# AIR-DISCOVER/TOIST

Measured on AMD Instinct MI355X. Metric: train images/sec/node (640x640, bs=8/GPU) + matcher index bit-match, higher is better.
Workload: dtype bf16; 1 GPU; configs[1]: ResNet-101 + RoBERTa-base + 6+6 transformer, 100 queries, batch 8/GPU 640x640, 16-token captions, detection loss (labels+boxes+cardinality+contrastive_align, 5 aux layers), dropout 0.1, clip 0.1 + AdamW + EMA (fused HIP tail); random-init weights; every step a different batch (4 resident batches, 0..10 targets per image) through fixed-address inputs; global_batch=8, parallelism=dp1, launch=hipGraph replay, decoder=2 XCD-resident launches (toist_xdec_fwd / toist_xdec_bwd, one image per XCD)

## Files before the change

include/toist_hip.h:

```cpp
#ifndef TOIST_HIP_H
#define TOIST_HIP_H

#include <stddef.h>
#include <stdint.h>

#ifdef __cplusplus
extern "C" {
#endif

#define TOIST_OK 0
#define TOIST_EINVAL (-1)
#define TOIST_EHIP (-2)

#define TOIST_ABI_VERSION 1

#if defined(__GNUC__)
#define TOIST_API __attribute__((visibility("default")))
#else
#define TOIST_API
#endif

TOIST_API int toist_version(void);
TOIST_API int toist_last_error(char* buf, size_t cap);

TOIST_API int toist_matcher(const float* logits, const float* boxes, const float* tgt_boxes, const float* pos_map,
                  const int32_t* tgt_off, const int32_t* match_off, int L, int B, int Q, int K, int max_T,
                  float w_class, float w_bbox, float w_giou, int64_t* src_idx, int64_t* tgt_idx,
                  int32_t* status, float* cost_out, void* stream);

enum {
    TOIST_A_ROWK = 0,
    TOIST_A_KROW = 1,
    TOIST_A_CONV = 2,
    TOIST_A_CONVT = 3
};
enum {
    TOIST_B_ROWK = 0,
    TOIST_B_KROW = 1,
    TOIST_B_CONVX = 2
};
enum {
    TOIST_ACT_NONE = 0,
    TOIST_ACT_RELU = 1,
    TOIST_ACT_GELU = 2,
    TOIST_ACT_SIGMOID = 3,
    TOIST_ACT_MASK_POS = 4,
    TOIST_ACT_GELU_BWD = 5,
    TOIST_ACT_SIGMOID_BWD = 6
};

typedef struct toist_operand {
    const void* ptr;
    int64_t bs_outer;
    int64_t bs_inner;
    int32_t ld;
    int32_t kin;
    int64_t tap_stride;
    int32_t SH, SW, SC;
    int32_t PH, PW;
    int32_t R, S, stride, pad, dil;
} toist_operand;

typedef struct toist_epilogue {
    float alpha;
    const float* scale;
    const float* shift;
    const float* rscale;
    const void* res;
    int32_t ldr;
    const void* aux;
    int32_t ldaux;
    int32_t act;
    void* pre_out;
    int32_t out_f32;
    int32_t accumulate;
    int32_t cmap, cH, cW, cOH, cOW, cst;
    int32_t res_div, res_mod;
    int32_t drop_where;
    float drop_p;
    uint64_t drop_seed;
    const uint64_t* drop_seed_dev;
} toist_epilogue;

typedef struct toist_group {
    const void* a;
    const void* b;
    int64_t c_off;
    int64_t rscale_off;
    int64_t colsum_off;
    int64_t shift_off;
} toist_group;

typedef struct toist_gemm {
    int32_t M, N, K;
    int32_t a_kind, b_kind;
    toist_operand a, b;
    void* c;
    int32_t ldc;
    int64_t cs_outer, cs_inner;
    int32_t batch, batch_inner;
    int32_t split_k;
    int32_t tile;
    int32_t flags;
    toist_epilogue epi;
    float* workspace;
    float* a_colsum;
    const toist_group* group;
    const void* a2;
    int32_t a2_from;
} toist_gemm;

TOIST_API int toist_gemm_bf16(const toist_gemm* desc, void* stream);
TOIST_API int toist_group_fill(const toist_group* rows, int n, toist_group* table, void* stream);

TOIST_API int toist_layernorm_fwd(const void* x, const float* gamma, const float* beta, float eps, int rows, int D,
                        void* y, float* mean, float* rstd, const void* add, void* y2, void* stream);
TOIST_API int toist_layernorm_bwd(const void* dy, const void* x, const float* mean, const float* rstd, const float* gamma,
                        int rows, int D, void* dx, float* dgamma, float* dbeta, void* dx_drop, float drop_p,
                        uint64_t seed, const uint64_t* seed_dev, float* partials, int partial_blocks, void* stream);
TOIST_API int toist_layernorm_bwd_blocks(int rows);
TOIST_API int toist_softmax_fwd(const void* scores, const uint8_t* key_pad, int nbatch, int H, int Sq, int Sk, int ld,
                      void* p, void* p_drop, float drop_p, uint64_t seed, const uint64_t* seed_dev, void* stream);
TOIST_API int toist_softmax_bwd(const void* p, const void* dp, int rows, int Sk, int ld, void* ds, float drop_p,
                      uint64_t seed, const uint64_t* seed_dev, void* stream);
TOIST_API int toist_colsum(const void* g, int M, int N, int ld, float* out, void* stream);
TOIST_API int toist_add_bf16(const void* a, const void* b, int64_t n, int64_t b_period, void* out, void* stream);
TOIST_API int toist_dropout_bf16(const void* x, int64_t n, float p, uint64_t seed, const uint64_t* seed_dev, void* out, void* stream);

TOIST_API int toist_pack_image(const float* nchw, int N, int C, int H, int W, void* nhwc8, void* stream);
TOIST_API int toist_maxpool3x3s2(const void* in, int N, int H, int W, int C, void* out, void* stream);
TOIST_API int toist_unpack_nhwc(const void* nhwc, int N, int HW, int C, float* nchw, void* stream);
TOIST_API int toist_text_prep(const int64_t* ids, const int64_t* attention_mask, int B, int L, int64_t pad_id, int64_t* pos_ids, uint8_t* key_pad, void* stream);
TOIST_API int toist_stamp(uint64_t* slots, int idx, void* stream);

TOIST_API int toist_stem_fwd(const float* image, const void* weight, const float* shift, int N, int C, int H, int W, void* out, void* stream);

TOIST_API int toist_sine_position(const uint8_t* mask, int B, int H, int W, int num_pos_feats, float temperature, void* out_tok,
                        float* out_nchw, void* stream);
TOIST_API int toist_sine_position_seq(const uint8_t* mask, int B, int H, int W, int num_pos_feats, float temperature, void* out_tok, int rows_per_image,
                                      void* stream);

TOIST_API int toist_embed_fwd(const int64_t* ids, const int64_t* pos_ids, const float* word, const float* pos, const float* type0,
                    int n, int D, void* out, void* stream);
TOIST_API int toist_embed_bwd(const void* g, const int64_t* ids, const int64_t* pos_ids, int n, int D, int64_t pad_id, float* dword,
                    float* dpos, float* dtype0, void* stream);

TOIST_API int toist_criterion_fwd(const float* logits, const float* boxes, const float* tgt_boxes, const float* pos_map,
                        const int32_t* tgt_off, const int32_t* match_off, const int64_t* src_idx, const int64_t* tgt_idx,
                        const float* num_boxes, int L, int B, int Q, int K, float eos_coef, float* losses,
                        const int32_t* match_status, void* stream);
TOIST_API int toist_criterion_bwd(const float* logits, const float* boxes, const float* tgt_boxes, const float* pos_map,
                        const int32_t* tgt_off, const int32_t* match_off, const int64_t* src_idx, const int64_t* tgt_idx,
                        const float* num_boxes, int L, int B, int Q, int K, float eos_coef, const float* upstream,
                        float* dlogits, float* dboxes, void* stream);

TOIST_API int toist_contrastive_fwd(const float* proj_queries, const float* proj_tokens, const uint64_t* tok_mask, const int32_t* tgt_off,
                          const int32_t* match_off, const int64_t* src_idx, const int64_t* tgt_idx, const float* num_boxes, int L,
                          int B, int Q, int T, int D, float temperature, float* losses, void* stream);
TOIST_API int toist_contrastive_bwd(const float* proj_queries, const float* proj_tokens, const uint64_t* tok_mask, const int32_t* tgt_off,
                          const int32_t* match_off, const int64_t* src_idx, const int64_t* tgt_idx, const float* num_boxes, int L,
                          int B, int Q, int T, int D, float temperature, const float* upstream, float* dproj_queries,
                          float* dproj_tokens, void* stream);
TOIST_API int toist_contrastive_bwd_ws(const float* proj_queries, const float* proj_tokens, const uint64_t* tok_mask, const int32_t* tgt_off,
                          const int32_t* match_off, const int64_t* src_idx, const int64_t* tgt_idx, const float* num_boxes, int L,
                          int B, int Q, int T, int D, float temperature, const float* upstream, float* dproj_queries,
                          float* dproj_tokens, float* workspace, void* stream);
TOIST_API int toist_contrastive_fwd_live(const float* proj_queries, const float* proj_tokens, const uint64_t* tok_mask, const int32_t* tgt_off,
                          const int32_t* match_off, const int64_t* src_idx, const int64_t* tgt_idx, const float* num_boxes, int L,
                          int B, int Q, int T, int D, float temperature, const int32_t* live_tokens, float* losses, void* stream);
TOIST_API int toist_contrastive_bwd_ws_live(const float* proj_queries, const float* proj_tokens, const uint64_t* tok_mask, const int32_t* tgt_off,
                          const int32_t* match_off, const int64_t* src_idx, const int64_t* tgt_idx, const float* num_boxes, int L,
                          int B, int Q, int T, int D, float temperature, const int32_t* live_tokens, const float* upstream,
                          float* dproj_queries, float* dproj_tokens, float* workspace, void* stream);
TOIST_API int toist_l2norm_fwd(const float* x, int rows, int D, float* y, void* stream);
TOIST_API int toist_l2norm_bwd(const float* x, const float* dy, int rows, int D, float* dx, void* stream);

TOIST_API int toist_attnmap_softmax_fwd(const void* scores, const uint8_t* key_pad, int B, int Q, int H, int HW, int ld, void* out, void* stream);
TOIST_API int toist_attnmap_softmax_bwd(const void* prob, const void* dprob, int BQ, int H, int HW, int ld, void* dscores, void* stream);
TOIST_API int toist_groupnorm_fwd(const void* x, const float* gamma, const float* beta, int N, int HW, int C, int G, float eps, int relu,
                        void* y, float* stats, void* stream);
TOIST_API int toist_groupnorm_apply(const void* x, const float* stats, const float* gamma, const float* beta, int N, int HW, int C, int G, float eps, int relu,
                        void* y, void* stream);
TOIST_API int toist_groupnorm_bwd(const void* dy, const void* y, const void* x, const float* stats, const float* gamma, const float* beta, int N, int HW,
                        int C, int G, float eps, int relu, void* dx, float* dgamma, float* dbeta, float* bstats, void* stream);
TOIST_API int toist_upsample_add(const void* in, const void* fpn, int BQ, int Q, int H, int W, int C, void* out, void* stream);
TOIST_API int toist_upsample_add_rows(const void* in, const void* fpn, const int64_t* rows, int n, int Q, int H, int W, int C, void* out, void* stream);
TOIST_API int toist_upsample_add_bwd(const void* dout, int BQ, int H, int W, int C, void* din, void* stream);
TOIST_API int toist_resize_add(const void* in, const void* fpn, const int64_t* rows, int n, int Q, int H, int W, int OH, int OW, int C, void* out, void* stream);
TOIST_API int toist_resize_add_bwd(const void* dout, int BQ, int H, int W, int OH, int OW, int C, void* din, void* stream);
TOIST_API int toist_sum_queries(const void* in, int B, int Q, int64_t per, void* out, void* stream);
TOIST_API int toist_mask_stage_fwd(const void* src, const float* src_stats, const float* gamma, const float* beta, const void* fpn_conv, const void* w,
                        const float* bias, void* out, float* out_stats, int N, int Q, int H, int W, int c_in, int c_out, int w_rows, int gn_in, int up,
                        float eps, void* stream);
TOIST_API int toist_mask_stage_fwd_pairs(const void* src, const float* src_stats, const float* gamma, const float* beta, const void* fpn_conv, const void* w,
                        const float* bias, void* out, float* out_stats, int N, int Q, int H, int W, int c_in, int c_out, int w_rows, int gn_in, int up,
                        float eps, const int32_t* pair_image, int n_images, int32_t* status, void* stream);
TOIST_API int toist_resize_add_pairs(const void* in, const void* fpn, const int32_t* pair_image, int n_images, int n, int Q, int H, int W, int OH, int OW,
                        int C, void* out, int32_t* status, void* stream);
TOIST_API int toist_sum_segments(const void* in, const int32_t* seg, int B, int rows, int64_t per, void* out, void* stream);
TOIST_API int toist_resize_add_rows_pairs(const void* in, const void* fpn, const int64_t* rows, const int32_t* pair_image, int n_images, int P, int n, int Q,
                        int H, int W, int OH, int OW, int C, void* out, int32_t* status, void* stream);
TOIST_API int toist_sum_maps_by_image(const void* in, const int32_t* seg, const int32_t* pair_image, int P, int Q, int n_images, int rows, int64_t per,
                        void* out, int32_t* status, void* stream);
TOIST_API int toist_mask_loss_fwd(const float* pred, const int32_t* pred_row, const uint8_t* gt, const int32_t* gt_row, int T, int h, int w,
                        int TH, int TW, float alpha, float* sums, const int32_t* valid_hw, void* stream);
TOIST_API int toist_mask_loss_bwd(const float* pred, const int32_t* pred_row, const uint8_t* gt, const int32_t* gt_row, int T, int h, int w,
                        int TH, int TW, float alpha, const float* sums, const float* coef, float* dpred, const int32_t* valid_hw, void* stream);
TOIST_API int toist_mask_loss_bwd_compact(const float* pred, const int32_t* pred_row, const uint8_t* gt, const int32_t* gt_row, int T, int h, int w,
                        int TH, int TW, float alpha, const float* sums, const float* coef, float* dpred_rows, const int32_t* valid_hw, void* stream);

typedef struct toist_opt_tensor {
    float* p;
    float* m;
    float* v;
    float* ema;
    uint16_t* w;
    const float* row_scale;
    int64_t numel;
    int32_t row_len;
    int32_t group;
} toist_opt_tensor;

typedef struct toist_opt_group {
    float lr;
    float weight_decay;
} toist_opt_group;

typedef struct toist_opt_state {
    float clip_coef;
    float grad_norm;
    float bias1;
    float bias2_sqrt;
    int32_t step;
    int32_t skipped;
    int32_t skipped_total;
    int32_t veto_mask;
} toist_opt_state;
#define TOIST_OPT_MAX_VETO 8

TOIST_API int toist_attn2_splits(int Sk);
TOIST_API int toist_attn2_fwd(const void* q, int ldq, const void* kmat, int ldk, const void* v, int ldv, const uint8_t* key_pad, int B, int H, int Sq,
                    int Sk, int dh, float scale, float drop_p, uint64_t seed, const uint64_t* seed_dev, void* ctx, int ldo, float* lse,
                    void* stream);
TOIST_API int toist_attn2_bwd(const void* q, int ldq, const void* kmat, int ldk, const void* v, int ldv, const void* ctx, int ldo, const void* dctx, int lddo,
                    const float* lse, const uint8_t* key_pad, int B, int H, int Sq, int Sk, int dh, float scale, float drop_p, uint64_t seed,
                    const uint64_t* seed_dev, void* dq, int lddq, void* dk, int lddk, void* dv, int lddv, void* dq_part, void* stream);

enum { TOIST_ROW_PLAIN = 0, TOIST_ROW_LN_FWD = 1, TOIST_ROW_LN_BWD = 2 };

typedef struct toist_rowgemm_desc {
    int32_t M, K;
    int32_t b_kind;
    int32_t epi;
    const void* a;
    const void* w;
    int32_t lda, ldw;
    const void* fold;
    int64_t fold_stride;
    int32_t fold_parts, fold_cols;
    const float* bias;
    const void* res;
    const void* res2;
    int32_t ldr, ldr2;
    float drop_p;
    float eps;
    uint64_t drop_seed;
    const uint64_t* drop_seed_dev;
    const float* gamma;
    const float* beta;
    void* z;
    float* mean;
    float* rstd;
    void* out;
    int32_t ldo, reserved;
    const void* add;
    void* out2;
    float* partials;
} toist_rowgemm_desc;

TOIST_API int toist_rowgemm_blocks(int M);
TOIST_API int toist_rowgemm(const toist_rowgemm_desc* d, void* stream);

enum { TOIST_XDEC_MAX_LAYERS = 8, TOIST_XDEC_CTL_WORDS = 1024 };

typedef struct toist_xdec_layer {
    const void* w_in;  const float* b_in;
    const void* w_os;  const float* b_os;
    const float* g1;   const float* be1;
    const void* w_q;   const float* b_q;
    const void* w_oc;  const float* b_oc;
    const float* g3;   const float* be3;
    const void* w1;    const float* b1;
    const void* w2;    const float* b2;
    const float* g4;   const float* be4;
    uint64_t seed[6];
} toist_xdec_layer;

typedef struct toist_xdec_desc {
// ... 4 lines not shown
    const void* kv;
    int32_t ldkv;
    int32_t ff;
    int32_t test_absent;
    int32_t reserved;
    const uint8_t* key_pad;
    float drop_p, eps;
    const uint64_t* seed_dev;
    void* qkv;
    void* ctx_s;
    float* lse_s;
    void* z1; void* y1; void* y1e; float* mean1; float* rstd1;
    void* qc;
    void* ctx_c;
    float* lse_c;
    void* z3; void* y3; float* mean3; float* rstd3;
    void* h;
    void* z4; void* y4; void* y4e; float* mean4; float* rstd4;
    void* part;
    uint32_t* ctl;
    uint64_t* prof;
    toist_xdec_layer layer[TOIST_XDEC_MAX_LAYERS];
} toist_xdec_desc;

TOIST_API int toist_xdec_supported(int B, int Q, int S, int L);
TOIST_API int toist_xdec_fwd(const toist_xdec_desc* d, void* stream);

typedef struct toist_xdec_bwd_layer {
    const void* w_in;
    const void* w_os;
    const void* w_q;
    const void* w_oc;
    const void* w1;
    const void* w2;
    const float* g1;
    const float* g3;
    const float* g4;
    uint64_t seed[6];
} toist_xdec_bwd_layer;

typedef struct toist_xdec_bwd_desc {
    int32_t B, Q, S, L;
    const void* kv;
    int32_t ldkv, ldsink, lddkv;
    int32_t ff;
    int32_t test_absent;
    int32_t reserved;
    const uint8_t* key_pad;
    float drop_p, reserved2;
    const uint64_t* seed_dev;
    const void* qkv; const void* ctx_s; const float* lse_s; const void* z1; const float* mean1; const float* rstd1;
    const void* qc; const void* ctx_c; const float* lse_c; const void* z3; const float* mean3; const float* rstd3;
    const void* h; const void* z4; const float* mean4; const float* rstd4;
    const void* g_out;
    void* gb4;
    void* dh;
    void* go3;
    void* go1;
    void* sink;
    void* dkv;
    float* ln_part;
    void* dctx;
    void* part;
    void* dq_part;
    uint32_t* ctl;
    uint64_t* prof;
    toist_xdec_bwd_layer layer[TOIST_XDEC_MAX_LAYERS];
} toist_xdec_bwd_desc;

TOIST_API int toist_xdec_bwd(const toist_xdec_bwd_desc* d, void* stream);

TOIST_API int toist_scatter_rows_f32(const float* src, const int64_t* src_row, float* dst, const int64_t* dst_row, int m, int d, void* stream);

TOIST_API int toist_kmeans(const float* banks, int64_t bank_stride, float* centers, int64_t centers_stride, const int32_t* group_task,
                 const int32_t* group_off, const int32_t* members, int n_groups, const float* features, int N, int D, int K, float tol,
                 int max_iter, int32_t* pick, float* chosen_center, int32_t* iters, void* stream);

TOIST_API int toist_kmeans_init(const float* banks, int64_t bank_stride, float* centers, int64_t centers_stride, const int32_t* group_task,
                 const int32_t* group_off, const int32_t* members, int n_groups, const float* features, int N, int D, int K, float tol,
                 int max_iter, int32_t* pick, float* chosen_center, int32_t* iters, const float* full_label, const int32_t* init_rows,
                 int32_t* status, void* stream);

TOIST_API int toist_sweep_prototypes(const void* memory, void* memory_mod, const int32_t* pair_caption, const int32_t* live, const float* W_sth,
                 const uint8_t* sub_sth, const int32_t* cap_task, const int32_t* group_task, const float* banks, int64_t bank_stride,
                 float* centers, int64_t centers_stride, int P, int HW, int L, int T, int n_tasks, int N, int D, int K, float tol, int max_iter,
                 int32_t* status, int32_t* pick, float* features, int32_t* iters, void* stream);

TOIST_API int toist_bank_fifo(float* banks, int64_t bank_stride, float* update_count, float* full_label, const int32_t* group_task,
                 const int32_t* group_off, const int32_t* members, int n_groups, const float* rows, int T, int B, int N, int D,
                 int fifo_when_full, int32_t* lsap_rows, void* stream);

TOIST_API int toist_attn_small_fwd(const void* q, int ldq, const void* kmat, int ldk, const void* v, int ldv, const uint8_t* key_pad, int B, int H, int S,
                         int dh, float scale, float drop_p, uint64_t seed, const uint64_t* seed_dev, void* ctx, int ldo, float* stats,
                         const float* bq, const float* bk, const float* bv, void* stream);
TOIST_API int toist_attn_small_bwd(const void* q, int ldq, const void* kmat, int ldk, const void* v, int ldv, const uint8_t* key_pad, int B, int H, int S,
                         int dh, float scale, float drop_p, uint64_t seed, const uint64_t* seed_dev, const float* stats, const void* dctx,
                         int lddo, void* dq, int lddq, void* dk, int lddk, void* dv, int lddv, const float* bq, const float* bk,
                         const float* bv, void* stream);

TOIST_API int toist_conv3x3_small(int dgrad, const void* src, const void* w, const float* shift, const void* res, void* out, int n_img, int H, int W,
                        int c_src, int c_out, int w_co, int w_ci, void* stream);

TOIST_API int toist_wgrad3x3_small_blocks(void);
TOIST_API int toist_wgrad3x3_small(const void* dy, const void* x, float* ws, int n_img, int H, int W, int c_in, int c_out, void* stream);

TOIST_API int toist_lsap(const float* cost, const int64_t* offset, const int32_t* rows, const int32_t* cols, int ld ,
               int n, int max_rows, int max_cols,
               int64_t max_cells , const int64_t* out_off, int64_t* row_idx, int64_t* col_idx, int32_t* status, void* stream);

#define TOIST_GEMM_DEFER_REDUCE 2
#define TOIST_GEMM_SPLIT_EPILOGUE 4
#define TOIST_GEMM_COLSUM_SLICES 32768
TOIST_API int toist_gemm_pick_tile(const toist_gemm* desc);
typedef struct toist_reduce_desc {
    const float* ws;
    float* out;
    const float* rscale;
    int32_t splits, M, N, ldc;
    float alpha;
    int32_t accumulate;
} toist_reduce_desc;
TOIST_API int toist_gemm_effective_split(const toist_gemm* desc);
TOIST_API int toist_splitk_reduce_batch(const toist_reduce_desc* descs, int n, void* stream);

typedef struct toist_conv_pair {
    int32_t M, C;
    int32_t dgrad;
    int32_t lda;
    const void* a;
    const void* w_first;
    const void* w_second;
    const float* shift_mid;
    const float* shift_out;
    const void* res;
    const void* aux_mid;
    const void* aux_out;
    void* mid;
    void* out;
    int32_t ldr, ldaux_mid, ldaux_out, ldmid, ldout, reserved;
} toist_conv_pair;
TOIST_API int toist_conv_pair_bf16(const toist_conv_pair* desc, void* stream);

TOIST_API int toist_opt_chunk_elems(void);
TOIST_API int toist_opt_sqnorm(const toist_opt_tensor* table, const int64_t* grads, const int32_t* chunks, int n_chunks, float* partial, void* stream);
TOIST_API int toist_opt_finish_norm(const float* partial, int n_chunks, float max_norm, float beta1, float beta2, toist_opt_state* state, void* stream);
TOIST_API int toist_opt_finish_norm_guarded(const float* partial, int n_chunks, float max_norm, float beta1, float beta2, toist_opt_state* state,
                        const int32_t* const* veto_i32, int n_veto_i32, const float* const* veto_f32, int n_veto_f32, void* stream);
TOIST_API int toist_opt_adamw_ema(const toist_opt_tensor* table, const int64_t* grads, const int32_t* chunks, int n_chunks,
                        const toist_opt_group* groups, const toist_opt_state* state, float beta1, float beta2, float eps,
                        float ema_decay, void* stream);
TOIST_API int toist_opt_adamw_ema_blocks(const toist_opt_tensor* table, const int64_t* grads, const int32_t* chunks, int n_chunks,
                               const toist_opt_group* groups, const toist_opt_state* state, float beta1, float beta2, float eps,
                               float ema_decay, int max_blocks, void* stream);

TOIST_API int toist_mask_resize_pack(const float* src, int n, int h0, int w0, int max_h, int max_w, int crop_h, int crop_w, int h, int w,
                           float threshold, uint64_t* bits, void* stream);
TOIST_API int toist_mask_resize_pack_batch(const float* src, int batch, int queries, int h0, int w0, int max_h, int max_w, const int64_t* table,
                                 int cap_h, int cap_w, long long capacity_words, float threshold, uint64_t* bits, void* stream);
TOIST_API int toist_mask_pack(const uint8_t* dense, int n, int h, int w, uint64_t* bits, void* stream);
TOIST_API int toist_mask_unpack(const uint64_t* bits, int n, int h, int w, uint8_t* dense, void* stream);
TOIST_API int toist_mask_area(const uint64_t* bits, int n, int h, int w, uint32_t* area, void* stream);
TOIST_API int toist_mask_iou(const uint64_t* dt, int n_dt, const uint64_t* gt, int n_gt, const uint8_t* iscrowd, const uint32_t* area_dt,
                   const uint32_t* area_gt, int h, int w, double* iou, void* stream);
TOIST_API int toist_mask_rle_count(const uint64_t* bits, int n, int h, int w, int32_t* column_transitions, void* stream);
TOIST_API int toist_mask_rle_emit(const uint64_t* bits, int n, int h, int w, const int64_t* column_offset, uint32_t* positions, void* stream);
TOIST_API int toist_mask_rle_counts(const uint32_t* positions, const int64_t* first_position, const int64_t* first_run, int n, int h, int w,
                          uint32_t* counts, void* stream);

TOIST_API int toist_postprocess(const void* pred_logits, int logits_bf16, const void* pred_boxes, int boxes_bf16, const void* pred_isfinal, int isfinal_bf16,
                      const int64_t* orig_sizes, int B, int Q, int C, float* scores, float* boxes, float* scores_refexp, void* stream);

TOIST_API int toist_coco_match(const double* iou, const int64_t* iou_offset, const double* dt_area, const int64_t* dt_offset, const double* gt_area,
                     const uint8_t* gt_ignore, const uint8_t* gt_crowd, const int64_t* gt_offset, int n_images, const double* area_ranges,
                     int n_ranges, const double* iou_thresholds, int n_thresholds, int32_t* dt_match, uint8_t* dt_ignore,
                     uint8_t* gt_range_ignore, uint8_t* gt_taken, void* stream);

#define TOIST_COCO_BOXES_MAX_Q 1024
TOIST_API int toist_coco_boxes(const float* scores, const float* boxes, int R, int Q, int max_det, const int32_t* row_slot, const int64_t* slot_off,
                     int n_slots, const double* gt_xywh, const double* gt_area, const uint8_t* gt_crowd, long long n_gt, const int64_t* iou_off,
                     const int64_t* gt_off, long long iou_cap, long long gt_cap, int32_t* order, double* dt_score, double* dt_area, double* iou,
                     double* out_gt_area, uint8_t* out_gt_crowd, void* stream);

#define TOIST_COCO_MASKS_CHUNK_WORDS 4096
TOIST_API int toist_coco_masks(const uint64_t* bits, long long capacity_words, const int64_t* row_hw, int R, int Q, int D, const int32_t* order,
                     const int32_t* row_slot, const int64_t* slot_off, int n_slots, const uint64_t* gt_bits, long long gt_words,
                     const int64_t* gt_plane_off, const int32_t* slot_hw, const uint32_t* gt_parea, const uint8_t* gt_crowd, long long n_gt,
                     const int64_t* iou_off, long long iou_cap, double* dt_area, double* iou, void* stream);

#define TOIST_PREP_DESC_WORDS 20
TOIST_API int toist_image_prep(const uint8_t* src, long long src_bytes, const int32_t* desc, const int32_t* arena, long long arena_words, const float* lut,
                     int batch_cap, int cap_h, int cap_w, float* out, uint8_t* mask, uint8_t* dst_u8, long long dst_bytes, void* stream);

#define TOIST_TMASK_DESC_WORDS 8
TOIST_API int toist_target_masks(const uint8_t* src, long long src_bytes, const int32_t* desc, const int32_t* arena, long long arena_words, int slots,
                     int cap_h, int cap_w, uint8_t* dst, void* stream);

#define TOIST_POLY_DESC_WORDS 8
#define TOIST_POLY_REC_WORDS 2
#define TOIST_POLY_STRIP 64
#define TOIST_POLY_MAX_ROWS 2048
#define TOIST_POLY_PACKED 0
#define TOIST_POLY_DENSE 1
TOIST_API int toist_polygon_masks(const int32_t* desc, int slots, const int32_t* polys, int poly_cap, const int32_t* verts, int vert_cap, int cap_h,
                     int cap_w, uint8_t* dst, long long dst_bytes, int mode, void* stream);

TOIST_API int toist_sweep_assemble(const void* img_tok, const void* img_pos, const uint8_t* img_pad, int B, int HW, const void* txt_tok,
                     const uint8_t* txt_pad, int T, int L, const int32_t* pair_image, const int32_t* pair_caption, int P, int D, void* tokens,
                     void* pos, uint8_t* key_pad, int32_t* status, void* stream);

TOIST_API int toist_sweep_assemble_bwd(const void* d_seq, const int32_t* pair_image, const int32_t* pair_caption, int P, int B, int HW, int T, int L,
                     int D, void* d_img, void* d_txt, void* stream);

TOIST_API int toist_sweep_gather(const void* src, const int32_t* pair_image, int n_images, int P, long long row_bytes, void* dst, int32_t* status,
                     void* stream);

#ifdef __cplusplus
}
#endif
#endif
```

toist_amd/csrc/optim.hip:

```cpp
#include "common.h"

namespace toist {

constexpr int OPT_CHUNK = 8192;

__device__ __forceinline__ float block_sum_256(float v, float* red) {
    v = wave_sum(v);
    const int lane = threadIdx.x & 63, wave = threadIdx.x >> 6;
    if (lane == 0) red[wave] = v;
    __syncthreads();
    return red[0] + red[1] + red[2] + red[3];
}

__global__ __launch_bounds__(256) void sqnorm_kernel(const toist_opt_tensor* __restrict__ T, const int64_t* __restrict__ G,
                                                     const int2* __restrict__ chunks, float* __restrict__ partial) {
    __shared__ float red[4];
    const int2 ch = chunks[blockIdx.x];
    const float* g = reinterpret_cast<const float*>(G[ch.x]);
    float acc = 0.f;
    if (g != nullptr) {
        const long long beg = (long long)ch.y * OPT_CHUNK;
        long long end = beg + OPT_CHUNK;
        if (end > T[ch.x].numel) end = T[ch.x].numel;
        const float* gp = g + beg;
        const int n = (int)(end - beg);
        if (((size_t)gp & 15) == 0) {
            const int n4 = n >> 2;
            for (int i = threadIdx.x; i < n4; i += 256) {
                const float4 x = reinterpret_cast<const float4*>(gp)[i];
                acc += x.x * x.x + x.y * x.y + x.z * x.z + x.w * x.w;
            }
            for (int i = (n4 << 2) + threadIdx.x; i < n; i += 256) acc += gp[i] * gp[i];
        } else {
            for (int i = threadIdx.x; i < n; i += 256) acc += gp[i] * gp[i];
        }
    }
    const float s = block_sum_256(acc, red);
    if (threadIdx.x == 0) partial[blockIdx.x] = s;
}

__device__ __forceinline__ double sum_partials_1024(const float* __restrict__ partial, int n, double* red) {
    double acc = 0.0;
    int i = threadIdx.x;
    for (; i + 3 * 1024 < n; i += 4 * 1024) {
        const float a = partial[i], b = partial[i + 1024], c = partial[i + 2 * 1024], d = partial[i + 3 * 1024];
        acc += ((double)a + (double)b) + ((double)c + (double)d);
    }
    for (; i < n; i += 1024) acc += (double)partial[i];
    red[threadIdx.x] = acc;
    __syncthreads();
    for (int s = 512; s > 0; s >>= 1) {
        if (threadIdx.x < s) red[threadIdx.x] += red[threadIdx.x + s];
        __syncthreads();
    }
    return red[0];
}

__device__ __forceinline__ void take_step(toist_opt_state* __restrict__ st, float norm, float max_norm, float beta1, float beta2) {
    float coef = 1.f;
    if (max_norm > 0.f) {
        coef = max_norm / (norm + 1e-6f);
        if (coef > 1.f) coef = 1.f;
    }
    const int step = st->step + 1;
    st->step = step;
    st->grad_norm = norm;
    st->clip_coef = coef;
    st->bias1 = 1.f - powf(beta1, (float)step);
    st->bias2_sqrt = sqrtf(1.f - powf(beta2, (float)step));
    st->skipped = 0;
}

__device__ __forceinline__ bool nonfinite(float x) { return (__float_as_uint(x) & 0x7f800000u) == 0x7f800000u; }

__global__ __launch_bounds__(1024) void finish_norm_kernel(const float* __restrict__ partial, int n, float max_norm, float beta1,
                                                           float beta2, toist_opt_state* __restrict__ st) {
    __shared__ double red[1024];
    const double sq = sum_partials_1024(partial, n, red);
    if (threadIdx.x == 0) take_step(st, (float)sqrt(sq), max_norm, beta1, beta2);
}

__global__ __launch_bounds__(1024) void finish_norm_guarded_kernel(const float* __restrict__ partial, int n, float max_norm, float beta1,
                                                                   float beta2, toist_opt_state* __restrict__ st,
                                                                   const int32_t* const* __restrict__ veto_i32, int n_i32,
                                                                   const float* const* __restrict__ veto_f32, int n_f32) {
    __shared__ double red[1024];
    __shared__ int veto[2 * TOIST_OPT_MAX_VETO];
    const int t = threadIdx.x;
    if (t < 2 * TOIST_OPT_MAX_VETO) {
        int bit = 0;
        if (t < TOIST_OPT_MAX_VETO) {
            if (t < n_i32 && *veto_i32[t] != 0) bit = 1 << (1 + t);
        } else if (t - TOIST_OPT_MAX_VETO < n_f32 && nonfinite(*veto_f32[t - TOIST_OPT_MAX_VETO])) {
            bit = 1 << (1 + t);
        }
        veto[t] = bit;
    }
    const double sq = sum_partials_1024(partial, n, red);
    if (t == 0) {
        const float norm = (float)sqrt(sq);
        int mask = nonfinite(norm) ? 1 : 0;
        for (int i = 0; i < 2 * TOIST_OPT_MAX_VETO; ++i) mask |= veto[i];
        st->veto_mask = mask;
        if (mask == 0) {
            take_step(st, norm, max_norm, beta1, beta2);
        } else {
            st->skipped = 1;
            st->skipped_total = st->skipped_total + 1;
            st->grad_norm = norm;
            st->clip_coef = 0.f;
        }
    }
}

__device__ __forceinline__ void adamw_one(float& p, float g, float& m, float& v, float lr, float wd, float b1, float b2, float eps,
                                          float step_size, float bias2_sqrt) {
    p -= lr * wd * p;
    m += (g - m) * (1.f - b1);
    v = b2 * v + (1.f - b2) * g * g;
    const float denom = sqrtf(v) / bias2_sqrt + eps;
    p -= step_size * (m / denom);
}

__global__ __launch_bounds__(256) void adamw_ema_kernel(const toist_opt_tensor* __restrict__ T, const int64_t* __restrict__ G,
                                                        const int2* __restrict__ chunks, const toist_opt_group* __restrict__ groups,
                                                        const toist_opt_state* __restrict__ st, float b1, float b2, float eps,
                                                        float decay, int n_chunks) {
  if (st->skipped != 0) return;
  for (int cb = blockIdx.x; cb < n_chunks; cb += gridDim.x) {
    const int2 ch = chunks[cb];
    const toist_opt_tensor t = T[ch.x];
    const float* g = reinterpret_cast<const float*>(G[ch.x]);
    const long long beg = (long long)ch.y * OPT_CHUNK;
    long long end = beg + OPT_CHUNK;
    if (end > t.numel) end = t.numel;
    const int n = (int)(end - beg);
    const float coef = st->clip_coef, bias2_sqrt = st->bias2_sqrt;
    const toist_opt_group gr = groups[t.group];
    const float lr = gr.lr, wd = gr.weight_decay, step_size = lr / st->bias1;
    float* p = t.p + beg;
    const bool upd = g != nullptr && t.m != nullptr;
    const bool vec = (((size_t)p | (size_t)(g ? g + beg : nullptr) | (size_t)(t.m ? t.m + beg : nullptr) | (size_t)(t.v ? t.v + beg : nullptr) |
                       (size_t)(t.ema ? t.ema + beg : nullptr)) & 15) == 0 &&
                     (t.w == nullptr || (((size_t)(t.w + beg)) & 7) == 0);
    const int n4 = vec ? (n >> 2) : 0;
    for (int i = threadIdx.x; i < n4; i += 256) {
        float4 pv = reinterpret_cast<float4*>(p)[i];
        if (upd) {
            float4 gv = reinterpret_cast<const float4*>(g + beg)[i];
            float4 mv = reinterpret_cast<float4*>(t.m + beg)[i];
            float4 vv = reinterpret_cast<float4*>(t.v + beg)[i];
            adamw_one(pv.x, gv.x * coef, mv.x, vv.x, lr, wd, b1, b2, eps, step_size, bias2_sqrt);
            adamw_one(pv.y, gv.y * coef, mv.y, vv.y, lr, wd, b1, b2, eps, step_size, bias2_sqrt);
            adamw_one(pv.z, gv.z * coef, mv.z, vv.z, lr, wd, b1, b2, eps, step_size, bias2_sqrt);
            adamw_one(pv.w, gv.w * coef, mv.w, vv.w, lr, wd, b1, b2, eps, step_size, bias2_sqrt);
            reinterpret_cast<float4*>(p)[i] = pv;
            reinterpret_cast<float4*>(t.m + beg)[i] = mv;
            reinterpret_cast<float4*>(t.v + beg)[i] = vv;
        }
        if (t.ema != nullptr) {
            float4 ev = reinterpret_cast<float4*>(t.ema + beg)[i];
            ev.x = ev.x * decay + (1.f - decay) * pv.x;
            ev.y = ev.y * decay + (1.f - decay) * pv.y;
            ev.z = ev.z * decay + (1.f - decay) * pv.z;
            ev.w = ev.w * decay + (1.f - decay) * pv.w;
            reinterpret_cast<float4*>(t.ema + beg)[i] = ev;
        }
        if (upd && t.w != nullptr) {
            float s = 1.f;
            const long long e0 = beg + ((long long)i << 2);
            if (t.row_scale != nullptr) {
                const long long r0 = e0 / t.row_len;
                if ((e0 + 3) / t.row_len == r0) s = t.row_scale[r0];
                else {
                    pv.x *= t.row_scale[e0 / t.row_len];
                    pv.y *= t.row_scale[(e0 + 1) / t.row_len];
                    pv.z *= t.row_scale[(e0 + 2) / t.row_len];
                    pv.w *= t.row_scale[(e0 + 3) / t.row_len];
                }
            }
            reinterpret_cast<uint2*>(t.w + beg)[i] = make_uint2(pack2bf(pv.x * s, pv.y * s), pack2bf(pv.z * s, pv.w * s));
        }
    }
    for (int i = (n4 << 2) + threadIdx.x; i < n; i += 256) {
        float pv = p[i];
        if (upd) {
            float mv = t.m[beg + i], vv = t.v[beg + i];
            adamw_one(pv, g[beg + i] * coef, mv, vv, lr, wd, b1, b2, eps, step_size, bias2_sqrt);
            p[i] = pv;
            t.m[beg + i] = mv;
            t.v[beg + i] = vv;
        }
        if (t.ema != nullptr) t.ema[beg + i] = t.ema[beg + i] * decay + (1.f - decay) * pv;
        if (upd && t.w != nullptr) {
            const float s = t.row_scale ? t.row_scale[(beg + i) / t.row_len] : 1.f;
            t.w[beg + i] = f2bf(pv * s);
        }
    }
  }
}

}

using namespace toist;

extern "C" int toist_opt_chunk_elems(void) { return OPT_CHUNK; }

extern "C" int toist_opt_sqnorm(const toist_opt_tensor* table, const int64_t* grads, const int32_t* chunks, int n_chunks, float* partial,
                                void* stream) {
    TOIST_REQUIRE(table && grads && chunks && partial && n_chunks > 0, "toist_opt_sqnorm: bad args");
    hipLaunchKernelGGL(sqnorm_kernel, dim3(n_chunks), dim3(256), 0, (hipStream_t)stream, table, grads, (const int2*)chunks, partial);
    return check_launch("toist_opt_sqnorm");
}

extern "C" int toist_opt_finish_norm(const float* partial, int n_chunks, float max_norm, float beta1, float beta2, toist_opt_state* state,
                                     void* stream) {
    TOIST_REQUIRE(partial && state && n_chunks > 0, "toist_opt_finish_norm: bad args");
    TOIST_REQUIRE(beta1 >= 0.f && beta1 < 1.f && beta2 >= 0.f && beta2 < 1.f, "toist_opt_finish_norm: betas must be in [0, 1)");
    hipLaunchKernelGGL(finish_norm_kernel, dim3(1), dim3(1024), 0, (hipStream_t)stream, partial, n_chunks, max_norm, beta1, beta2, state);
    return check_launch("toist_opt_finish_norm");
}

extern "C" int toist_opt_finish_norm_guarded(const float* partial, int n_chunks, float max_norm, float beta1, float beta2, toist_opt_state* state,
                                             const int32_t* const* veto_i32, int n_veto_i32, const float* const* veto_f32, int n_veto_f32,
                                             void* stream) {
    TOIST_REQUIRE(partial && state && n_chunks > 0, "toist_opt_finish_norm_guarded: bad args");
    TOIST_REQUIRE(beta1 >= 0.f && beta1 < 1.f && beta2 >= 0.f && beta2 < 1.f, "toist_opt_finish_norm_guarded: betas must be in [0, 1)");
    TOIST_REQUIRE(n_veto_i32 >= 0 && n_veto_i32 <= TOIST_OPT_MAX_VETO && n_veto_f32 >= 0 && n_veto_f32 <= TOIST_OPT_MAX_VETO,
                  "toist_opt_finish_norm_guarded: at most 8 veto words of each kind");
    TOIST_REQUIRE((veto_i32 || n_veto_i32 == 0) && (veto_f32 || n_veto_f32 == 0), "toist_opt_finish_norm_guarded: NULL veto table with a positive count");
    hipLaunchKernelGGL(finish_norm_guarded_kernel, dim3(1), dim3(1024), 0, (hipStream_t)stream, partial, n_chunks, max_norm, beta1, beta2, state,
                       veto_i32, n_veto_i32, veto_f32, n_veto_f32);
    return check_launch("toist_opt_finish_norm_guarded");
}

extern "C" int toist_opt_adamw_ema_blocks(const toist_opt_tensor* table, const int64_t* grads, const int32_t* chunks, int n_chunks,
                                          const toist_opt_group* groups, const toist_opt_state* state, float beta1, float beta2, float eps,
                                          float ema_decay, int max_blocks, void* stream) {
    TOIST_REQUIRE(table && grads && chunks && groups && state && n_chunks > 0, "toist_opt_adamw_ema: bad args");
    TOIST_REQUIRE(eps > 0.f && ema_decay >= 0.f && ema_decay <= 1.f, "toist_opt_adamw_ema: bad eps / ema_decay");
    const int blocks = (max_blocks > 0 && max_blocks < n_chunks) ? max_blocks : n_chunks;
    hipLaunchKernelGGL(adamw_ema_kernel, dim3(blocks), dim3(256), 0, (hipStream_t)stream, table, grads, (const int2*)chunks, groups, state,
                       beta1, beta2, eps, ema_decay, n_chunks);
    return check_launch("toist_opt_adamw_ema");
}

extern "C" int toist_opt_adamw_ema(const toist_opt_tensor* table, const int64_t* grads, const int32_t* chunks, int n_chunks,
                                   const toist_opt_group* groups, const toist_opt_state* state, float beta1, float beta2, float eps,
                                   float ema_decay, void* stream) {
    return toist_opt_adamw_ema_blocks(table, grads, chunks, n_chunks, groups, state, beta1, beta2, eps, ema_decay, 0, stream);
}
```

toist_amd/csrc/rows.hip:

```cpp
#include "common.h"
#include <cstdlib>

namespace toist {

constexpr int LN_MAXCH = 2;

__global__ __launch_bounds__(256) void layernorm_fwd_kernel(const bf16_t* __restrict__ x, const float* __restrict__ gamma,
                                                             const float* __restrict__ beta, float eps, int rows, int D,
                                                             bf16_t* __restrict__ y, float* __restrict__ mean_out,
                                                             float* __restrict__ rstd_out, const bf16_t* __restrict__ add,
                                                             bf16_t* __restrict__ y2) {
    const int lane = threadIdx.x & 63;
    const int row = blockIdx.x * 4 + (threadIdx.x >> 6);
    if (row >= rows) return;
    const int nch = D >> 3;
    float v[LN_MAXCH][8];
    float s = 0.f;
#pragma unroll
    for (int i = 0; i < LN_MAXCH; ++i) {
        const int ch = lane + 64 * i;
        if (ch < nch) {
            unpack8(*reinterpret_cast<const uint4*>(x + (size_t)row * D + ch * 8), v[i]);
#pragma unroll
            for (int j = 0; j < 8; ++j) s += v[i][j];
// ... 214 lines not shown
                }
                *reinterpret_cast<uint4*>(p_drop + (size_t)row * ld + ch * 8) = pack8(o);
            }
        }
    }
}

__global__ __launch_bounds__(256) void softmax_bwd_kernel(const bf16_t* __restrict__ p, const bf16_t* __restrict__ dp, int rows,
                                                           int Sk, int ld, bf16_t* __restrict__ ds, float drop_p,
                                                           unsigned long long seed, const unsigned long long* __restrict__ seed_dev) {
    if (seed_dev) seed += *seed_dev;
    const int lane = threadIdx.x & 63;
    const int row = blockIdx.x * 4 + (threadIdx.x >> 6);
    if (row >= rows) return;
    const int nch = ld >> 3;
    const bool drop = drop_p > 0.f;
    const unsigned thresh = drop ? (unsigned)(drop_p * 4294967296.0) : 0u;
    const float dscale = drop ? 1.f / (1.f - drop_p) : 1.f;
    float pv[SM_MAXCH][8], gv[SM_MAXCH][8];
    float dot = 0.f;
#pragma unroll
    for (int i = 0; i < SM_MAXCH; ++i) {
        const int ch = lane + 64 * i;
        if (ch < nch) {
            unpack8(*reinterpret_cast<const uint4*>(p + (size_t)row * ld + ch * 8), pv[i]);
            unpack8(*reinterpret_cast<const uint4*>(dp + (size_t)row * ld + ch * 8), gv[i]);
#pragma unroll
            for (int j = 0; j < 8; ++j) {
                const int k = ch * 8 + j;
                if (k >= Sk) { pv[i][j] = 0.f; gv[i][j] = 0.f; }
                if (drop) {
                    const unsigned long long idx = (unsigned long long)row * ld + k;
                    gv[i][j] = dropout_keep(seed, idx, thresh) ? gv[i][j] * dscale : 0.f;
                }
                dot += pv[i][j] * gv[i][j];
            }
        }
    }
    dot = wave_sum(dot);
#pragma unroll
    for (int i = 0; i < SM_MAXCH; ++i) {
        const int ch = lane + 64 * i;
        if (ch < nch) {
            float o[8];
#pragma unroll
            for (int j = 0; j < 8; ++j) o[j] = pv[i][j] * (gv[i][j] - dot);
            *reinterpret_cast<uint4*>(ds + (size_t)row * ld + ch * 8) = pack8(o);
        }
    }
}

constexpr int CS_ROWS = 8192;
__global__ __launch_bounds__(256) void colsum_narrow_kernel(const bf16_t* __restrict__ g, long long M, int N, float* __restrict__ out) {
    __shared__ float red[256][9];
    const int cpr = N >> 3;
    const int rpp = 256 / cpr;
    const int cx = threadIdx.x % cpr, ry = threadIdx.x / cpr;
    const long long m_beg = (long long)blockIdx.x * CS_ROWS;
    const long long m_end = (m_beg + CS_ROWS < M) ? m_beg + CS_ROWS : M;
    float a[8] = {0.f, 0.f, 0.f, 0.f, 0.f, 0.f, 0.f, 0.f};
    for (long long m = m_beg + ry; m < m_end; m += rpp) {
        float v[8];
        unpack8(*reinterpret_cast<const uint4*>(g + m * N + cx * 8), v);
#pragma unroll
        for (int j = 0; j < 8; ++j) a[j] += v[j];
    }
#pragma unroll
    for (int j = 0; j < 8; ++j) red[threadIdx.x][j] = a[j];
    __syncthreads();
    if ((int)threadIdx.x < N) {
        const int c = threadIdx.x, cc = c >> 3, j = c & 7;
        float t = 0.f;
        for (int r = 0; r < rpp; ++r) t += red[r * cpr + cc][j];
        atomicAdd(out + c, t);
    }
}

__global__ __launch_bounds__(256) void colsum_kernel(const bf16_t* __restrict__ g, int M, int N, int ld, float* __restrict__ out) {
    __shared__ float red[8][256];
    const int cx = threadIdx.x & 31, ry = threadIdx.x >> 5;
    const int n = blockIdx.x * 256 + cx * 8;
    const int m_beg = blockIdx.y * 256;
    const int m_end = (m_beg + 256 < M) ? m_beg + 256 : M;
    float a[8] = {0.f, 0.f, 0.f, 0.f, 0.f, 0.f, 0.f, 0.f};
    if (n < N) {
        const bool vec = (n + 8 <= N) && ((ld & 7) == 0) && ((((size_t)g) & 15) == 0);
        for (int m = m_beg + ry; m < m_end; m += 8) {
            if (vec) {
                float v[8];
                unpack8(*reinterpret_cast<const uint4*>(g + (size_t)m * ld + n), v);
#pragma unroll
                for (int j = 0; j < 8; ++j) a[j] += v[j];
            } else {
#pragma unroll
                for (int j = 0; j < 8; ++j) if (n + j < N) a[j] += bf2f(g[(size_t)m * ld + n + j]);
            }
        }
    }
#pragma unroll
    for (int j = 0; j < 8; ++j) red[ry][cx * 8 + j] = a[j];
    __syncthreads();
    const int c = threadIdx.x;
    if (blockIdx.x * 256 + c < N) {
        float t = 0.f;
#pragma unroll
        for (int r = 0; r < 8; ++r) t += red[r][c];
        atomicAdd(out + blockIdx.x * 256 + c, t);
    }
}

__global__ __launch_bounds__(256) void add_kernel(const bf16_t* __restrict__ a, const bf16_t* __restrict__ b, long long n8,
                                                   long long bperiod8, bf16_t* __restrict__ out) {
    for (long long i = (long long)blockIdx.x * 256 + threadIdx.x; i < n8; i += (long long)gridDim.x * 256) {
        float x[8], y[8];
        unpack8(reinterpret_cast<const uint4*>(a)[i], x);
        unpack8(reinterpret_cast<const uint4*>(b)[i % bperiod8], y);
#pragma unroll
        for (int j = 0; j < 8; ++j) x[j] += y[j];
        reinterpret_cast<uint4*>(out)[i] = pack8(x);
    }
}

__global__ __launch_bounds__(256) void dropout_kernel(const bf16_t* __restrict__ x, long long n8, float p, unsigned long long seed,
                                                       const unsigned long long* __restrict__ seed_dev, bf16_t* __restrict__ out) {
    if (seed_dev) seed += *seed_dev;
    const unsigned thresh = (unsigned)(p * 4294967296.0);
    const float sc = 1.f / (1.f - p);
    for (long long i = (long long)blockIdx.x * 256 + threadIdx.x; i < n8; i += (long long)gridDim.x * 256) {
        float v[8];
        unpack8(reinterpret_cast<const uint4*>(x)[i], v);
#pragma unroll
        for (int j = 0; j < 8; ++j) v[j] = dropout_keep(seed, (unsigned long long)i * 8 + j, thresh) ? v[j] * sc : 0.f;
        reinterpret_cast<uint4*>(out)[i] = pack8(v);
    }
}


__global__ __launch_bounds__(256) void embed_fwd_kernel(const long long* __restrict__ ids, const long long* __restrict__ pos_ids,
                                                         const float* __restrict__ word, const float* __restrict__ pos,
                                                         const float* __restrict__ type0, int n, int D, bf16_t* __restrict__ out) {
    const int lane = threadIdx.x & 63;
    const int t = blockIdx.x * 4 + (threadIdx.x >> 6);
    if (t >= n) return;
    const float* w = word + ids[t] * (long long)D;
    const float* p = pos + pos_ids[t] * (long long)D;
    for (int c = lane * 2; c < D; c += 128) {
        const float a = (w[c] + type0[c]) + p[c];
        const float b = (w[c + 1] + type0[c + 1]) + p[c + 1];
        *reinterpret_cast<unsigned*>(out + (size_t)t * D + c) = pack2bf(a, b);
    }
}
__global__ __launch_bounds__(256) void embed_bwd_kernel(const bf16_t* __restrict__ g, const long long* __restrict__ ids,
                                                         const long long* __restrict__ pos_ids, int n, int D, long long pad_id,
                                                         float* __restrict__ dword, float* __restrict__ dpos) {
    const int lane = threadIdx.x & 63;
    const int t = blockIdx.x * 4 + (threadIdx.x >> 6);
    if (t >= n) return;
    for (int which = 0; which < 2; ++which) {
        const long long* key = which ? pos_ids : ids;
        float* table = which ? dpos : dword;
        if (table == nullptr) continue;
        const long long id = key[t];
        if (id == pad_id) continue;
        bool dup = false;
        for (int u = lane; u < t; u += 64) dup |= (key[u] == id);
        if (__any(dup)) continue;
        float* row = table + id * (long long)D;
        for (int c0 = 0; c0 < D; c0 += 64) {
            const int c = c0 + lane;
            float s = 0.f;
            for (int base = t; base < n; base += 64) {
                const int u = base + lane;
                unsigned long long m = __ballot(u < n && key[u] == id);
                while (m) {
                    const int b = __ffsll((long long)m) - 1;
                    m &= m - 1;
                    if (c < D) s += bf2f(g[(size_t)(base + b) * D + c]);
                }
            }
            if (c < D) row[c] += s;
        }
    }
}
__global__ __launch_bounds__(256) void embed_type_bwd_kernel(const bf16_t* __restrict__ g, int n, int D, float* __restrict__ dtype0) {
    __shared__ float red[8][32];
    const int cx = threadIdx.x & 31, ry = threadIdx.x >> 5;
    const int c = blockIdx.x * 32 + cx;
    float a = 0.f;
    if (c < D)
        for (int t = ry; t < n; t += 8) a += bf2f(g[(size_t)t * D + c]);
    red[ry][cx] = a;
    __syncthreads();
    if (ry == 0 && c < D) {
        float s = 0.f;
#pragma unroll
        for (int r = 0; r < 8; ++r) s += red[r][cx];
        dtype0[c] += s;
    }
}

static inline int grid_for(long long n, int cap = 2048) {
    long long g = (n + 255) / 256;
    if (g < 1) g = 1;
    return (int)(g > cap ? cap : g);
}

}

using namespace toist;

extern "C" int toist_layernorm_fwd(const void* x, const float* gamma, const float* beta, float eps, int rows, int D,
                                   void* y, float* mean, float* rstd, const void* add, void* y2, void* stream) {
    TOIST_REQUIRE(rows > 0 && D > 0 && (D % 8) == 0 && D <= 1024, "toist_layernorm_fwd: rows=%d D=%d (D%%8==0, D<=1024)", rows, D);
    TOIST_REQUIRE((add == nullptr) == (y2 == nullptr), "toist_layernorm_fwd: add and y2 come together");
    hipLaunchKernelGGL(layernorm_fwd_kernel, dim3((rows + 3) / 4), dim3(256), 0, (hipStream_t)stream, (const bf16_t*)x, gamma,
                       beta, eps, rows, D, (bf16_t*)y, mean, rstd, (const bf16_t*)add, (bf16_t*)y2);
    return check_launch("toist_layernorm_fwd");
}

extern "C" int toist_layernorm_bwd_blocks(int rows) {
    int blocks = (rows + 7) / 8;
    if (blocks > 512) blocks = 512;
    return blocks < 1 ? 1 : blocks;
}

extern "C" int toist_layernorm_bwd(const void* dy, const void* x, const float* mean, const float* rstd, const float* gamma,
                                   int rows, int D, void* dx, float* dgamma, float* dbeta, void* dx_drop, float drop_p,
                                   uint64_t seed, const uint64_t* seed_dev, float* partials, int partial_blocks, void* stream) {
    TOIST_REQUIRE(rows > 0 && D > 0 && (D % 8) == 0 && D <= 1024, "toist_layernorm_bwd: rows=%d D=%d", rows, D);
    TOIST_REQUIRE((dgamma == nullptr) == (dbeta == nullptr), "toist_layernorm_bwd: dgamma/dbeta must both be set or null");
    TOIST_REQUIRE(partials == nullptr || (dgamma == nullptr && partial_blocks > 0), "toist_layernorm_bwd: partials replace dgamma / dbeta and need a block count");
    int blocks = (rows + 15) / 16;
    if (blocks > 128) blocks = 128;
    if (blocks < 1) blocks = 1;
    if (partials) blocks = partial_blocks;
    hipLaunchKernelGGL(layernorm_bwd_kernel, dim3(blocks), dim3(256), 0, (hipStream_t)stream, (const bf16_t*)dy,
                       (const bf16_t*)x, mean, rstd, gamma, rows, D, (bf16_t*)dx, dgamma, dbeta, (bf16_t*)dx_drop, drop_p,
                       (unsigned long long)seed, (const unsigned long long*)seed_dev, partials);
    return check_launch("toist_layernorm_bwd");
}

extern "C" int toist_softmax_fwd(const void* scores, const uint8_t* key_pad, int nbatch, int H, int Sq, int Sk, int ld,
                                 void* p, void* p_drop, float drop_p, uint64_t seed, const uint64_t* seed_dev, void* stream) {
    TOIST_REQUIRE(nbatch > 0 && H > 0 && Sq > 0 && Sk > 0, "toist_softmax_fwd: bad shape");
    TOIST_REQUIRE((ld % 8) == 0 && ld >= Sk && ld <= 2048, "toist_softmax_fwd: ld=%d Sk=%d (ld%%8==0, Sk<=ld<=2048)", ld, Sk);
    const int rows = nbatch * H * Sq;
    hipLaunchKernelGGL(softmax_fwd_kernel, dim3((rows + 3) / 4), dim3(256), 0, (hipStream_t)stream, (const bf16_t*)scores, key_pad,
                       rows, H, Sq, Sk, ld, (bf16_t*)p, (bf16_t*)p_drop, drop_p, (unsigned long long)seed, (const unsigned long long*)seed_dev);
    return check_launch("toist_softmax_fwd");
}

extern "C" int toist_softmax_bwd(const void* p, const void* dp, int rows, int Sk, int ld, void* ds, float drop_p, uint64_t seed,
                                 const uint64_t* seed_dev, void* stream) {
    TOIST_REQUIRE(rows > 0 && Sk > 0 && (ld % 8) == 0 && ld >= Sk && ld <= 2048, "toist_softmax_bwd: bad shape");
    hipLaunchKernelGGL(softmax_bwd_kernel, dim3((rows + 3) / 4), dim3(256), 0, (hipStream_t)stream, (const bf16_t*)p,
                       (const bf16_t*)dp, rows, Sk, ld, (bf16_t*)ds, drop_p, (unsigned long long)seed, (const unsigned long long*)seed_dev);
    return check_launch("toist_softmax_bwd");
}

extern "C" int toist_colsum(const void* g, int M, int N, int ld, float* out, void* stream) {
    TOIST_REQUIRE(M > 0 && N > 0 && ld >= N, "toist_colsum: bad shape");
    if (ld == N && N <= 128 && (N & 7) == 0 && (256 % (N >> 3)) == 0 && M >= 4 * CS_ROWS && ((((size_t)g) & 15) == 0)) {
        hipLaunchKernelGGL(colsum_narrow_kernel, dim3((unsigned)((M + CS_ROWS - 1) / CS_ROWS)), dim3(256), 0, (hipStream_t)stream, (const bf16_t*)g,
                           (long long)M, N, out);
        return check_launch("toist_colsum(narrow)");
    }
    hipLaunchKernelGGL(colsum_kernel, dim3((N + 255) / 256, (M + 255) / 256), dim3(256), 0, (hipStream_t)stream, (const bf16_t*)g, M,
                       N, ld, out);
    return check_launch("toist_colsum");
}

extern "C" int toist_add_bf16(const void* a, const void* b, int64_t n, int64_t b_period, void* out, void* stream) {
    TOIST_REQUIRE(n > 0 && (n % 8) == 0 && b_period > 0 && (b_period % 8) == 0 && (n % b_period) == 0,
                  "toist_add_bf16: n and b_period must be multiples of 8 and n %% b_period == 0");
    hipLaunchKernelGGL(add_kernel, dim3(grid_for(n / 8)), dim3(256), 0, (hipStream_t)stream, (const bf16_t*)a, (const bf16_t*)b,
                       (long long)(n / 8), (long long)(b_period / 8), (bf16_t*)out);
    return check_launch("toist_add_bf16");
}

extern "C" int toist_dropout_bf16(const void* x, int64_t n, float p, uint64_t seed, const uint64_t* seed_dev, void* out, void* stream) {
    TOIST_REQUIRE(n > 0 && (n % 8) == 0 && p >= 0.f && p < 1.f, "toist_dropout_bf16: bad args");
    hipLaunchKernelGGL(dropout_kernel, dim3(grid_for(n / 8)), dim3(256), 0, (hipStream_t)stream, (const bf16_t*)x, (long long)(n / 8),
                       p, (unsigned long long)seed, (const unsigned long long*)seed_dev, (bf16_t*)out);
    return check_launch("toist_dropout_bf16");
}

extern "C" int toist_embed_fwd(const int64_t* ids, const int64_t* pos_ids, const float* word, const float* pos, const float* type0,
                               int n, int D, void* out, void* stream) {
    TOIST_REQUIRE(n > 0 && D > 0 && (D % 2) == 0, "toist_embed_fwd: bad shape");
    hipLaunchKernelGGL(embed_fwd_kernel, dim3((n + 3) / 4), dim3(256), 0, (hipStream_t)stream, (const long long*)ids,
                       (const long long*)pos_ids, word, pos, type0, n, D, (bf16_t*)out);
    return check_launch("toist_embed_fwd");
}

extern "C" int toist_embed_bwd(const void* g, const int64_t* ids, const int64_t* pos_ids, int n, int D, int64_t pad_id, float* dword,
                               float* dpos, float* dtype0, void* stream) {
    TOIST_REQUIRE(n > 0 && D > 0, "toist_embed_bwd: bad shape");
    if (dword != nullptr || dpos != nullptr)
        hipLaunchKernelGGL(embed_bwd_kernel, dim3((n + 3) / 4), dim3(256), 0, (hipStream_t)stream, (const bf16_t*)g, (const long long*)ids,
                           (const long long*)pos_ids, n, D, (long long)pad_id, dword, dpos);
    if (dtype0 != nullptr)
        hipLaunchKernelGGL(embed_type_bwd_kernel, dim3((D + 31) / 32), dim3(256), 0, (hipStream_t)stream, (const bf16_t*)g, n, D, dtype0);
    return check_launch("toist_embed_bwd");
}
```

toist_amd/engine.py:

```python
import math

import weakref

import torch

from . import kernels as k
from . import ops
from .knobs import knob

BF16 = torch.bfloat16


class Var:

    __slots__ = ("data", "grad", "needs_grad", "drop", "gdrop", "raw_grad")

    def __init__(self, data, needs_grad=True):
        self.data = data
        self.grad = None
        self.needs_grad = needs_grad
        self.raw_grad = False
        self.drop = None
        self.gdrop = None

    def take_branch_grad(self, g):
        gd, self.gdrop = self.gdrop, None
        if gd is None:
            gd = torch.empty_like(g)
            k.dropout(g, self.drop[0], self.drop[1], gd)
        return gd

    def take_grad(self):
        g, self.grad = self.grad, None
        return g


OVERLAP = knob("TOIST_OVERLAP", "capture")
FUSED_ATTENTION = True
FUSED_BLOCKS = True
_SIDE = {}
SIDE_PRIORITY = knob("TOIST_SIDE_PRIORITY", 0)


_TEXT_PRELUDE = []


def register_text_prelude(opt, late_params):
    _TEXT_PRELUDE[:] = [(r, ids) for r, ids in _TEXT_PRELUDE if r() is not None]
    _TEXT_PRELUDE.append((weakref.ref(opt), frozenset(id(p) for p in late_params)))


def run_text_prelude(param):
    for r, ids in _TEXT_PRELUDE:
        opt = r()
        if opt is not None and id(param) in ids:
            opt.flush_late()


def side_stream(device, name):
    key = (device.index, name)
    s = _SIDE.get(key)
    if s is None:
        s = _SIDE[key] = torch.cuda.Stream(device=device, priority=SIDE_PRIORITY)
    return s


def overlap_enabled():
    if OVERLAP == "on":
        return True
    return OVERLAP == "capture" and torch.cuda.is_current_stream_capturing()


GROUP_WGRADS = knob("TOIST_GROUP_WGRADS", True)


class Tape:
    def __init__(self, training, drop_p=0.0, seed=0, group_wgrads=False):
        self.groups = {} if (group_wgrads and GROUP_WGRADS) else None
        self.steps = []
        self.training = training
        self.drop_p = drop_p if training else 0.0
        self._seed = seed * 1000003 + 12345
        self.keep = []
        self.fresh_views = []

    def next_seed(self):
        self._seed += 7919
        return self._seed & 0x7FFFFFFFFFFF

    def record(self, fn):
        self.steps.append(fn)

    def conv_wgrad(self, dy, x, w_shape, out, rscale, stride=1, pad=0, view=None):
        store = view is not None and view.fresh and not view.written
        if view is not None:
            view.mark_written()
        if self.groups is None:
            ops.conv2d_wgrad(dy, x, w_shape, stride=stride, pad=pad, out=out, rscale=rscale, defer=True, accumulate=not store)
        else:
            self.groups.setdefault((tuple(dy.shape), tuple(x.shape), tuple(w_shape), stride, pad, store), []).append((dy, x, out, rscale))

    def linear_wgrad(self, dy, x, W, b, owned=True):
        bias_out = b.g if b is not None else None
        store = W.fresh and not W.written
        W.mark_written()
        if self.groups is None or not owned:
            ops.linear_wgrad(dy, x, out=W.g, bias_out=bias_out, defer=True, accumulate=not store)
        else:
            key = ("linear", tuple(dy.shape), dy.stride(0), tuple(x.shape), x.stride(0), W.g.stride(0), bias_out is None, store)
            self.groups.setdefault(key, []).append((dy, x, W.g, bias_out))

    def backward(self):
        for fn in reversed(self.steps):
            fn()
        self.steps = []
        if self.groups:
            for key, items in self.groups.items():
                if key[0] == "linear":
                    ops.linear_wgrad_group(items, accumulate=not key[-1])
                else:
                    ops.conv2d_wgrad_group(items, key[2], stride=key[3], pad=key[4], accumulate=not key[5])
            self.groups = {}
        k.flush_reductions()
        for v in self.fresh_views:
            for a, b in v.unwritten_rows():
                if v.g.dim() == 0:
                    v.g.zero_()
                else:
                    v.g[a:b].zero_()


WEIGHT_EPOCH = 0
COPY_GEN = 0
COPIES = {}


def bump_weight_epoch():
    global WEIGHT_EPOCH
    WEIGHT_EPOCH += 1


try:
    from torch.optim.optimizer import register_optimizer_step_post_hook as _reg_post_hook
    _reg_post_hook(lambda *a, **k: bump_weight_epoch())
except Exception:
    _reg_post_hook = None


class ComputeCopy:
    __slots__ = ("version", "ptr", "epoch", "w", "row_scale", "elementwise", "master")


def prune_copies():
    for ptr in [ptr for ptr, ent in COPIES.items() if ent.master() is None]:
        del COPIES[ptr]


def copy_of(t):
    ent = COPIES.get(t.data_ptr())
    return ent if ent is not None and ent.master() is t and ent.ptr == t.data_ptr() else None


def _cast_bf16(m):
    return m.detach().to(BF16)


_cast_bf16.elementwise = True


def compute_copy(t, make, cache, name):
    global COPY_GEN
    ent = cache.get(name) if cache is not None else None
    if ent is not None and ent.version == t._version and ent.ptr == t.data_ptr() and (ent.epoch == WEIGHT_EPOCH or not t.requires_grad) \
            and _reg_post_hook is not None:
        return ent.w
    w = make(t)
    pinned = bool(getattr(make, "pinned", False))
    if ent is not None and pinned and ent.w.data_ptr() != w.data_ptr():
        ent = None
    if ent is not None and pinned:
        pass
    elif ent is not None and ent.w.shape == w.shape and ent.w.stride() == w.stride():
        ent.w.copy_(w)
    else:
        ent = ComputeCopy()
        ent.w = w
        ent.elementwise = bool(getattr(make, "elementwise", False)) and w.shape == t.shape and w.stride() == t.stride()
        ent.row_scale = getattr(make, "row_scale", None)
        COPY_GEN += 1
        if cache is not None:
            cache[name] = ent
    ent.version, ent.ptr, ent.epoch, ent.master = t._version, t.data_ptr(), WEIGHT_EPOCH, weakref.ref(t)
    if cache is not None:
        COPIES[t.data_ptr()] = ent
    return ent.w


def named_cache(owner, key, build):
    memo = owner.__dict__.setdefault("_named_memo", {})
    ent = memo.get(key)
    if ent is None:
        ent = memo[key] = build()
    return ent


class ParamView:

    __slots__ = ("w", "g", "f32", "fresh", "parent", "_lo", "_hi", "_ranges")

    def __init__(self, w_bf16, grad_f32, f32=None, fresh=False, parent=None, lo=None, hi=None):
        self.w = w_bf16
        self.g = grad_f32
        self.f32 = f32
        self.fresh = fresh
        self.parent = parent
        self._lo, self._hi = lo, hi
        self._ranges = []

    def _root(self):
        v = self
        while v.parent is not None:
            v = v.parent
        return v

    def _span(self):
        lo, hi, v = 0, None, self
        chain = []
        while v is not None:
            chain.append(v)
            v = v.parent
        for v in reversed(chain):
            if v._lo is not None:
                lo, hi = lo + v._lo, lo + v._hi
        return lo, hi

    @property
    def written(self):
        root = self._root()
        if any(a is None for a, _ in root._ranges):
            return True
        lo, hi = self._span()
        if hi is None:
            n = root.g.shape[0] if root.g is not None and root.g.dim() > 0 else 1
            lo, hi = 0, n
        pos = lo
        for a, b in sorted(root._ranges):
            if a > pos:
                break
            pos = max(pos, b)
        return pos >= hi

    @written.setter
    def written(self, value):
        if value:
            self.mark_written()
        else:
            self._root()._ranges = []

    def rows(self, a, b):
        return ParamView(None if self.w is None else self.w[a:b], None if self.g is None else self.g[a:b],
                         None if self.f32 is None else self.f32[a:b], fresh=self.fresh, parent=self, lo=a, hi=b)

    def mark_written(self):
        root = self._root()
        lo, hi = self._span()
        root._ranges.append((None, None) if hi is None else (lo, hi))

    def unwritten_rows(self):
        if any(a is None for a, _ in self._ranges):
            return []
        n = self.g.shape[0] if self.g.dim() > 0 else 1
        gaps, pos = [], 0
        for a, b in sorted(self._ranges):
            if a > pos:
                gaps.append((pos, a))
            pos = max(pos, b)
        if pos < n:
            gaps.append((pos, n))
        return gaps


REUSE_GRAD_BUFFERS = False
STORE_ONCE = knob("TOIST_STORE_ONCE", True)
POISON_FRESH = False


class ParamSet:

    def __init__(self, named, trainable, need_grads, bf16_cache=None, transforms=None, store_once=None):
        self.names = list(named.keys())
        self.views = {}
        self.zero_elems = 0
        memo = bf16_cache.get("__layout__") if bf16_cache is not None else None
        params = list(named.values())
        sig = (need_grads, len(params), tuple(trainable.get(n, False) for n in self.names), id(params[0]) if params else 0,
               params[0].data_ptr() if params else 0, id(params[-1]) if params else 0, params[-1].data_ptr() if params else 0,
               STORE_ONCE and store_once is not None)
        if REUSE_GRAD_BUFFERS and memo is not None and memo["sig"] == sig and need_grads and memo["flat"] is not None:
            lo, hi = memo["flat"].data_ptr(), memo["flat"].data_ptr() + memo["flat"].numel() * 4
            if not any(p.grad is not None and lo <= p.grad.data_ptr() < hi for p in params):
                self.flat = memo["flat"]
                self.zero_elems = memo["zero_elems"]
                self._clear()
                for n, t in named.items():
                    pv = memo["views"][n]
                    pv.written = False
                    if t.dim() >= 2:
                        pv.w = compute_copy(t, (transforms or {}).get(n) or _cast_bf16, bf16_cache, n)
                    self.views[n] = pv
                return
        fresh_names = set()
        if need_grads and STORE_ONCE and store_once is not None:
            fresh_names = {n for n in self.names if trainable.get(n, False) and store_once(n, named[n])}
        pad = lambda t: (t.numel() + 63) // 64 * 64
        total = 0
        if need_grads:
            self.zero_elems = sum(pad(named[n]) for n in self.names if trainable.get(n, False) and n not in fresh_names)
            total = self.zero_elems + sum(pad(named[n]) for n in fresh_names)
        dev = next(iter(named.values())).device if named else None
        self.flat = torch.empty(total, dtype=torch.float32, device=dev) if total else None
        self._clear()
        off_zero, off_fresh = 0, self.zero_elems
        for n in self.names:
            t = named[n]
            g = None
            if need_grads and trainable.get(n, False):
                off = off_fresh if n in fresh_names else off_zero
                g = self.flat[off:off + t.numel()].view(t.shape)
                if t.dim() == 4 and not t.is_contiguous() and t.is_contiguous(memory_format=torch.channels_last):
                    O, I, R, S = t.shape
                    g = self.flat[off:off + t.numel()].view(O, R, S, I).permute(0, 3, 1, 2)
                if n in fresh_names:
                    off_fresh += pad(t)
                else:
                    off_zero += pad(t)
            wb = None
            if t.dim() >= 2:
                make = (transforms or {}).get(n) or _cast_bf16
                wb = compute_copy(t, make, bf16_cache, n)
            self.views[n] = ParamView(wb, g, t.detach(), fresh=n in fresh_names)
        if REUSE_GRAD_BUFFERS and bf16_cache is not None and need_grads and (memo is None or memo["sig"] != sig):
            bf16_cache["__layout__"] = {"sig": sig, "flat": self.flat, "views": dict(self.views), "zero_elems": self.zero_elems}

    def _clear(self):
        if self.flat is None:
            return
        if self.zero_elems:
            self.flat[:self.zero_elems].zero_()
        if POISON_FRESH and self.zero_elems < self.flat.numel():
            self.flat[self.zero_elems:].fill_(float("nan"))

    def fresh_views(self):
        return [v for v in self.views.values() if v.fresh and v.g is not None]

    def __getitem__(self, name):
        return self.views[name]

    def grads(self):
        return [self.views[n].g for n in self.names]


def krsc(w):
    v = w.permute(0, 2, 3, 1)
    assert v.is_contiguous(), "conv weights must be channels_last"
    return v


def accumulate(var, g):
    if var.grad is None:
        var.grad = g
    else:
        k.add(var.grad, g, var.grad)


def linear_chain(tape, x, layers, res=None, final_drop=False, out_dtype=BF16, last_act_external=False, in_relu_mask=False):
    acts = []
    cur = x.data
    p = tape.drop_p
    seeds = []
    n = len(layers)
    for i, (W, b, act, drop_after) in enumerate(layers):
        last = i == n - 1
        kw = {}
        seed = 0
        if drop_after and p > 0:
            seed = tape.next_seed()
            kw = dict(drop_where=2, drop_p=p, drop_seed=seed)
        if last and final_drop and p > 0:
            seed = tape.next_seed()
            kw = dict(drop_where=1, drop_p=p, drop_seed=seed)
        pre = None
        if act == k.ACT_GELU:
            pre = torch.empty(cur.shape[0], W.w.shape[0], dtype=BF16, device=cur.device)
        y = ops.linear(cur, W.w, b.f32 if b is not None else None, act=act, res=res.data if (last and res is not None) else None,
                       pre_out=pre, out_dtype=out_dtype if last else BF16, **kw)
        acts.append((cur, y, pre))
        seeds.append(seed)
        cur = y
    out = Var(cur)
    if final_drop and p > 0:
        out.drop = (p, seeds[-1])

    def bwd():
        g = out.take_grad()
        if g is None:
            return
        if res is not None and res.needs_grad:
            accumulate(res, g)
        for i in range(n - 1, -1, -1):
            W, b, act, drop_after = layers[i]
            xin, y, pre = acts[i]
            last = i == n - 1
            if last:
                if final_drop and p > 0:
                    g = out.take_branch_grad(g)
                if act != k.ACT_NONE and not last_act_external:
                    raise NotImplementedError("activation on the last layer of a chain needs last_act_external")
            if W.g is not None:
                tape.linear_wgrad(g, xin, W, b, owned=not (last and res is not None and res.needs_grad and not (final_drop and p > 0)))
            if i == 0:
                if x.needs_grad:
                    if in_relu_mask:
                        x.grad = ops.linear_dgrad(g, W.w, res=x.grad, act=k.ACT_MASK_POS, aux=x.data)
                    else:
                        x.grad = ops.linear_dgrad(g, W.w, res=x.grad)
            else:
                pW, pb, pact, pdrop = layers[i - 1]
                _, py, ppre = acts[i - 1]
                alpha = 1.0 / (1.0 - p) if (pdrop and p > 0) else 1.0
                if pact == k.ACT_RELU:
                    g = ops.linear_dgrad(g, W.w, act=k.ACT_MASK_POS, aux=py, alpha=alpha)
                elif pact == k.ACT_GELU:
                    if pdrop and p > 0:
                        raise NotImplementedError("dropout after GELU")
                    g = ops.linear_dgrad(g, W.w, act=k.ACT_GELU_BWD, aux=ppre)
                elif pact == k.ACT_NONE:
                    g = ops.linear_dgrad(g, W.w)
                else:
                    raise NotImplementedError

    tape.record(bwd)
    return out


def layernorm(tape, x, gamma, beta, eps, y=None):
    rows, D = x.data.shape
    if y is None:
        y = torch.empty_like(x.data)
    mean = torch.empty(rows, dtype=torch.float32, device=y.device)
    rstd = torch.empty(rows, dtype=torch.float32, device=y.device)
    k.layernorm_fwd(x.data, gamma.f32, beta.f32, eps, y, mean, rstd)
    out = Var(y)

    def bwd():
        g = out.take_grad()
        if g is None:
            return
        dx = torch.empty_like(g)
        if x.drop is not None and x.grad is None and x.needs_grad:
            x.gdrop = torch.empty_like(g)
            k.layernorm_bwd(g, x.data, mean, rstd, gamma.f32, dx, gamma.g, beta.g if gamma.g is not None else None, dx_drop=x.gdrop,
                            drop_p=x.drop[0], seed=x.drop[1], defer=True)
        else:
            k.layernorm_bwd(g, x.data, mean, rstd, gamma.f32, dx, gamma.g, beta.g if gamma.g is not None else None, defer=True)
        if x.needs_grad:
            accumulate(x, dx)

    tape.record(bwd)
    return out


def add_const(tape, x, c):
    y = torch.empty_like(x.data)
    k.add(x.data, c, y, b_period=c.numel())
    out = Var(y)

    def bwd():
        g = out.take_grad()
        if g is not None and x.needs_grad:
            accumulate(x, g)

    tape.record(bwd)
    return out


def add_vars(tape, a, b):
    y = torch.empty_like(a.data)
    k.add(a.data, b.data, y, b_period=b.data.numel())
    out = Var(y)
    rep = a.data.numel() // b.data.numel()

    def bwd():
        g = out.take_grad()
        if g is None:
            return
        if b.needs_grad:
            if rep == 1:
                accumulate(b, g)
            else:
                gb = g.view(rep, -1).float().sum(0).to(BF16).view(b.data.shape)
                accumulate(b, gb)
        if a.needs_grad:
            accumulate(a, g)
# ... 317 lines not shown
```

toist_amd/functions.py:

```python
import torch

from . import engine, kernels

GRAD_SYNC = None

AFTER_BACKWARD = []

REJOIN = None

PARAM_GRADS = "auto"


def _via_autograd():
    if PARAM_GRADS != "auto":
        return PARAM_GRADS == "autograd"
    try:
        from torch.nn.parallel import DistributedDataParallel as _DDP
        return getattr(_DDP, "_active_ddp_module", None) is not None
    except Exception:
        return False


class _TapeFn(torch.autograd.Function):
    @staticmethod
    def forward(ctx, body, names, cache, n_in, tape_kw, *tensors):
        inputs = tensors[:n_in]
        params = tensors[n_in:]
        tape_kw = dict(tape_kw)
        ctx.rejoin = tape_kw.pop('rejoin')
        ctx.via_autograd = tape_kw.pop('via_autograd')
        need = tape_kw.pop('need_grads')
        transforms = tape_kw.pop('transforms')
        store_once = tape_kw.pop('store_once')
        named = dict(zip(names, params))
        trainable = {n: p.requires_grad for n, p in named.items()}
        ps = engine.ParamSet(named, trainable, need_grads=need, bf16_cache=cache, transforms=transforms, store_once=store_once)
        tape = engine.Tape(**tape_kw)
        tape.fresh_views = ps.fresh_views() if need else []
        in_vars = [None if t is None else engine.Var(t, needs_grad=(need and t.requires_grad and t.is_floating_point()))
                   for t in inputs]
        out_vars, extra = body(tape, ps, *in_vars)
        if need:
            ctx.tape, ctx.ps, ctx.in_vars, ctx.out_vars = tape, ps, in_vars, out_vars
            ctx.params = params
        else:
            tape.steps = []
        ctx.n_in = n_in
        ctx.label = names[0].split(".")[0] if names else "program"
        ctx.n_par = len(params)
        ctx.extra = extra
        non_diff = [v.data for v in out_vars if not v.needs_grad]
        if non_diff:
            ctx.mark_non_differentiable(*non_diff)
        return tuple(v.data for v in out_vars)

    @staticmethod
    def backward(ctx, *grads):
        tape, ps = ctx.tape, ctx.ps
        if kernels.STAMPS is not None:
            kernels.stamp("bwd." + ctx.label + ".start")
        for v, g in zip(ctx.out_vars, grads):
            if g is not None and v.needs_grad:
                if v.raw_grad:
                    v.grad = g
                    continue
                if g.dtype != v.data.dtype:
                    g = g.to(v.data.dtype)
                v.grad = g.contiguous()
        tape.backward()
        if kernels.STAMPS is not None:
            kernels.stamp("bwd." + ctx.label + ".end")
        in_grads = []
        for v in ctx.in_vars:
            if v is None or not v.needs_grad:
                in_grads.append(None)
            else:
                in_grads.append(v.take_grad())
        n_par = len(ctx.params)
        if ctx.via_autograd:
            par_grads = [g if (g is not None and p.requires_grad) else None for p, g in zip(ctx.params, ps.grads())]
            if ctx.rejoin is not None:
                ctx.rejoin.wait_stream(torch.cuda.current_stream())
            ctx.tape = ctx.ps = ctx.in_vars = ctx.out_vars = ctx.params = None
            del tape, ps
            return (None, None, None, None, None, *in_grads, *par_grads)
        for p, g in zip(ctx.params, ps.grads()):
            if g is None:
                continue
            if p.grad is None:
                p.grad = g
            else:
                p.grad.add_(g)
                ps.flat = None
        if GRAD_SYNC is not None:
            GRAD_SYNC(ps.flat)
        elif AFTER_BACKWARD:
            for hook in AFTER_BACKWARD:
                hook(ctx.params)
        if ctx.rejoin is not None:
            ctx.rejoin.wait_stream(torch.cuda.current_stream())
        ctx.tape = ctx.ps = ctx.in_vars = ctx.out_vars = ctx.params = None
        return (None, None, None, None, None, *in_grads, *([None] * n_par))


def run_program(body, named_params, inputs, cache=None, training=False, drop_p=0.0, seed=0, transforms=None, group_wgrads=False, store_once=None):
    names = tuple(named_params.keys())
    params = tuple(named_params.values())
    need = torch.is_grad_enabled() and any(t is not None and t.requires_grad for t in (*inputs, *params))
    tape_kw = dict(training=training, drop_p=drop_p, seed=seed, need_grads=need, transforms=transforms, rejoin=REJOIN, group_wgrads=group_wgrads,
                   via_autograd=need and _via_autograd(), store_once=store_once)
    return _TapeFn.apply(body, names, cache, len(inputs), tape_kw, *inputs, *params)
```

toist_amd/kernels.py:

```python
import ctypes
import os

import torch

from . import _lib
from .devcache import DeviceCache, keep
from .folds import FOLDS, _raw_stream
from .knobs import knob
from ._lib import (A_CONV, A_CONVT, A_KROW, A_ROWK, ACT_GELU, ACT_GELU_BWD, ACT_MASK_POS, ACT_NONE, ACT_RELU,
                   ACT_SIGMOID, ACT_SIGMOID_BWD, B_CONVX, B_KROW, B_ROWK, Epilogue, Gemm, Operand)

__all__ = [
    "A_ROWK", "A_KROW", "A_CONV", "A_CONVT", "B_ROWK", "B_KROW", "B_CONVX", "ACT_NONE", "ACT_RELU", "ACT_GELU",
    "ACT_SIGMOID", "ACT_MASK_POS", "ACT_GELU_BWD", "ACT_SIGMOID_BWD", "ConvGeom", "operand", "gemm", "matcher",
    "layernorm_fwd", "layernorm_bwd", "softmax_fwd", "softmax_bwd", "colsum", "add", "dropout", "pack_image", "maxpool3x3s2", "stem_fwd",
    "unpack_nhwc", "sine_position", "embed_fwd", "embed_bwd", "criterion_fwd", "criterion_bwd", "attnmap_softmax_fwd", "attnmap_softmax_bwd",
    "groupnorm_fwd", "groupnorm_apply", "groupnorm_bwd", "upsample_add", "upsample_add_bwd", "sum_queries", "sum_segments", "upsample_add_rows", "mask_stage_fwd", "mask_loss_fwd", "mask_loss_bwd",
]


PROFILE = None
SEED_DEV = None
FORCE_TILE = 0
FORCE_SPLIT = 0
# ... 249 lines not shown
    d.aux_mid, d.ldaux_mid = _p(aux_mid, torch.bfloat16), aux_mid.stride(0) if aux_mid is not None else 0
    d.aux_out, d.ldaux_out = _p(aux_out, torch.bfloat16), aux_out.stride(0) if aux_out is not None else 0
    d.mid, d.ldmid, d.out, d.ldout = _p(mid, torch.bfloat16), mid.stride(0), _p(out, torch.bfloat16), out.stride(0)
    CONV_PAIR_CALLS[1 if dgrad else 0] += 1
    _lib.check(_lib.lib().toist_conv_pair_bf16(ctypes.cast(ctypes.pointer(d), ctypes.c_void_p), _stream()), "toist_conv_pair_bf16")


def matcher(logits, boxes, tgt_boxes, pos_map, tgt_off, match_off, max_T, w_class, w_bbox, w_giou, src_idx, tgt_idx,
            status, cost_out=None):
    L, B, Q, K = logits.shape
    _lib.check(
        _lib.lib().toist_matcher(_p(logits, torch.float32), _p(boxes, torch.float32), _p(tgt_boxes, torch.float32),
                                 _p(pos_map, torch.float32), _p(tgt_off, torch.int32), _p(match_off, torch.int32), L, B, Q,
                                 K, max_T, w_class, w_bbox, w_giou, _p(src_idx, torch.int64), _p(tgt_idx, torch.int64),
                                 _p(status, torch.int32), _p(cost_out, torch.float32), _stream()), "toist_matcher")


def layernorm_fwd(x, gamma, beta, eps, y, mean=None, rstd=None, add=None, y2=None):
    rows, D = x.shape
    _lib.check(
        _lib.lib().toist_layernorm_fwd(_p(x, torch.bfloat16), _p(gamma, torch.float32), _p(beta, torch.float32), eps, rows, D,
                                       _p(y, torch.bfloat16), _p(mean, torch.float32), _p(rstd, torch.float32), _p(add, torch.bfloat16),
                                       _p(y2, torch.bfloat16), _stream()),
        "toist_layernorm_fwd")


LN_DEFER = knob("TOIST_LN_DEFER", True)


def _queue_ln_param_grads(blocks, D, dgamma, dbeta):
    partials = FOLDS.acquire(2 * blocks * D, dgamma.device, (dgamma, dbeta))
    for i, out in enumerate((dgamma, dbeta)):
        FOLDS.queue(partials.data_ptr() + 4 * i * blocks * D, out, blocks, 1, D, D)
    return partials


def layernorm_bwd(dy, x, mean, rstd, gamma, dx, dgamma=None, dbeta=None, dx_drop=None, drop_p=0.0, seed=0, defer=False):
    rows, D = x.shape
    partials, blocks = None, 0
    if defer and LN_DEFER and dgamma is not None:
        blocks = int(_lib.lib().toist_layernorm_bwd_blocks(rows))
        partials = _queue_ln_param_grads(blocks, D, dgamma, dbeta)
    _lib.check(
        _lib.lib().toist_layernorm_bwd(_p(dy, torch.bfloat16), _p(x, torch.bfloat16), _p(mean, torch.float32),
                                       _p(rstd, torch.float32), _p(gamma, torch.float32), rows, D, _p(dx, torch.bfloat16),
                                       None if partials is not None else _p(dgamma, torch.float32),
                                       None if partials is not None else _p(dbeta, torch.float32), _p(dx_drop, torch.bfloat16),
                                       drop_p, seed, _p(SEED_DEV), _p(partials, torch.float32), blocks, _stream()), "toist_layernorm_bwd")


def softmax_fwd(scores, key_pad, nbatch, H, Sq, Sk, ld, p, p_drop=None, drop_p=0.0, seed=0):
    _lib.check(
        _lib.lib().toist_softmax_fwd(_p(scores, torch.bfloat16), _p(key_pad, torch.uint8), nbatch, H, Sq, Sk, ld,
                                     _p(p, torch.bfloat16), _p(p_drop, torch.bfloat16), drop_p, seed, _p(SEED_DEV), _stream()),
        "toist_softmax_fwd")


def softmax_bwd(p, dp, rows, Sk, ld, ds, drop_p=0.0, seed=0):
    _lib.check(
        _lib.lib().toist_softmax_bwd(_p(p, torch.bfloat16), _p(dp, torch.bfloat16), rows, Sk, ld, _p(ds, torch.bfloat16),
                                     drop_p, seed, _p(SEED_DEV), _stream()), "toist_softmax_bwd")


def colsum(g, M, N, ld, out):
    _lib.check(_lib.lib().toist_colsum(_p(g, torch.bfloat16), M, N, ld, _p(out, torch.float32), _stream()), "toist_colsum")


def add(a, b, out, b_period=None):
    n = a.numel()
    _lib.check(
        _lib.lib().toist_add_bf16(_p(a, torch.bfloat16), _p(b, torch.bfloat16), n, n if b_period is None else b_period,
                                  _p(out, torch.bfloat16), _stream()), "toist_add_bf16")


STAMPS = None


def stamp(name):
    st = STAMPS
    if st is None:
        return
    names = st["names"]
    if name in names:
        idx = names.index(name)
    else:
        idx = len(names)
        if idx >= st["buf"].numel():
            return
        names.append(name)
    _lib.check(_lib.lib().toist_stamp(_p(st["buf"], torch.int64), idx, _stream()), "toist_stamp")


def dropout(x, p, seed, out):
    _lib.check(_lib.lib().toist_dropout_bf16(_p(x, torch.bfloat16), x.numel(), p, seed, _p(SEED_DEV), _p(out, torch.bfloat16), _stream()),
               "toist_dropout_bf16")


def pack_image(nchw, out):
    N, C, H, W = nchw.shape
    _lib.check(_lib.lib().toist_pack_image(_p(nchw, torch.float32), N, C, H, W, _p(out, torch.bfloat16), _stream()), "toist_pack_image")


def stem_fwd(images, w, shift, out):
    N, C, H, W = images.shape
    assert tuple(w.shape) == (64, 7, 7, 8) and w.is_contiguous() and images.is_contiguous() and out.is_contiguous()
    _lib.check(_lib.lib().toist_stem_fwd(_p(images, torch.float32), _p(w, torch.bfloat16), _p(shift, torch.float32), N, C, H, W,
                                         _p(out, torch.bfloat16), _stream()), "toist_stem_fwd")


def maxpool3x3s2(x, out):
    N, H, W, C = x.shape
    _lib.check(_lib.lib().toist_maxpool3x3s2(_p(x, torch.bfloat16), N, H, W, C, _p(out, torch.bfloat16), _stream()), "toist_maxpool3x3s2")


def unpack_nhwc(x, out):
    N, HW, C = x.shape
    _lib.check(_lib.lib().toist_unpack_nhwc(_p(x, torch.bfloat16), N, HW, C, _p(out, torch.float32), _stream()), "toist_unpack_nhwc")


def sine_position(mask_u8, num_pos_feats, temperature, out_tok=None, out_nchw=None):
    B, H, W = mask_u8.shape
    _lib.check(_lib.lib().toist_sine_position(_p(mask_u8, torch.uint8), B, H, W, num_pos_feats, temperature, _p(out_tok, torch.bfloat16),
                                              _p(out_nchw, torch.float32), _stream()), "toist_sine_position")


def text_prep(ids, attention_mask, pad_id):
    B, L = ids.shape
    pos_ids = torch.empty(B, L, dtype=torch.int64, device=ids.device)
    key_pad = torch.empty(B, L, dtype=torch.uint8, device=ids.device)
    _lib.check(_lib.lib().toist_text_prep(_p(ids, torch.int64), _p(attention_mask, torch.int64), B, L, pad_id, _p(pos_ids), _p(key_pad), _stream()),
               "toist_text_prep")
    return pos_ids, key_pad


def sine_position_seq(mask_u8, num_pos_feats, temperature, out_tok):
    B, H, W = mask_u8.shape
    _lib.check(_lib.lib().toist_sine_position_seq(_p(mask_u8, torch.uint8), B, H, W, num_pos_feats, temperature, _p(out_tok, torch.bfloat16),
                                                  out_tok.shape[1], _stream()), "toist_sine_position_seq")


def embed_fwd(ids, pos_ids, word, pos, type0, out):
    n, D = out.shape
    _lib.check(_lib.lib().toist_embed_fwd(_p(ids, torch.int64), _p(pos_ids, torch.int64), _p(word, torch.float32), _p(pos, torch.float32),
                                          _p(type0, torch.float32), n, D, _p(out, torch.bfloat16), _stream()), "toist_embed_fwd")


def embed_bwd(g, ids, pos_ids, pad_id, dword, dpos, dtype0):
    n, D = g.shape
    _lib.check(_lib.lib().toist_embed_bwd(_p(g, torch.bfloat16), _p(ids, torch.int64), _p(pos_ids, torch.int64), n, D, pad_id,
                                          _p(dword, torch.float32), _p(dpos, torch.float32), _p(dtype0, torch.float32), _stream()),
               "toist_embed_bwd")


def criterion_fwd(logits, boxes, tgt_boxes, pos_map, tgt_off, match_off, src_idx, tgt_idx, num_boxes, eos_coef, losses, status=None):
    L, B, Q, K = logits.shape
    _lib.check(_lib.lib().toist_criterion_fwd(_p(logits, torch.float32), _p(boxes, torch.float32), _p(tgt_boxes, torch.float32),
                                              _p(pos_map, torch.float32), _p(tgt_off, torch.int32), _p(match_off, torch.int32),
                                              _p(src_idx, torch.int64), _p(tgt_idx, torch.int64), _p(num_boxes, torch.float32), L, B, Q, K,
                                              eos_coef, _p(losses, torch.float32), _p(status, torch.int32), _stream()), "toist_criterion_fwd")


def criterion_bwd(logits, boxes, tgt_boxes, pos_map, tgt_off, match_off, src_idx, tgt_idx, num_boxes, eos_coef, upstream, dlogits, dboxes):
    L, B, Q, K = logits.shape
    _lib.check(_lib.lib().toist_criterion_bwd(_p(logits, torch.float32), _p(boxes, torch.float32), _p(tgt_boxes, torch.float32),
                                              _p(pos_map, torch.float32), _p(tgt_off, torch.int32), _p(match_off, torch.int32),
                                              _p(src_idx, torch.int64), _p(tgt_idx, torch.int64), _p(num_boxes, torch.float32), L, B, Q, K,
                                              eos_coef, _p(upstream, torch.float32), _p(dlogits, torch.float32), _p(dboxes, torch.float32),
                                              _stream()), "toist_criterion_bwd")


def contrastive_fwd(pq, pt, tok_mask, tgt_off, match_off, src_idx, tgt_idx, num_boxes, temperature, losses, live_tokens=None):
    L, B, Q, D = pq.shape
    if live_tokens is None:
        _lib.check(_lib.lib().toist_contrastive_fwd(_p(pq, torch.float32), _p(pt, torch.float32), _p(tok_mask, torch.int64), _p(tgt_off, torch.int32),
                                                    _p(match_off, torch.int32), _p(src_idx, torch.int64), _p(tgt_idx, torch.int64),
                                                    _p(num_boxes, torch.float32), L, B, Q, pt.shape[1], D, temperature, _p(losses, torch.float32),
                                                    _stream()), "toist_contrastive_fwd")
        return
    _lib.check(_lib.lib().toist_contrastive_fwd_live(_p(pq, torch.float32), _p(pt, torch.float32), _p(tok_mask, torch.int64), _p(tgt_off, torch.int32),
                                                     _p(match_off, torch.int32), _p(src_idx, torch.int64), _p(tgt_idx, torch.int64),
                                                     _p(num_boxes, torch.float32), L, B, Q, pt.shape[1], D, temperature, _p(live_tokens, torch.int32),
                                                     _p(losses, torch.float32), _stream()), "toist_contrastive_fwd_live")


def contrastive_bwd(pq, pt, tok_mask, tgt_off, match_off, src_idx, tgt_idx, num_boxes, temperature, upstream, dpq, dpt, live_tokens=None, workspace=None):
    L, B, Q, D = pq.shape
    ws = workspace if workspace is not None else \
        torch.empty(L * B * pt.shape[1] * D, dtype=torch.float32, device=pq.device)
    if ws.numel() < L * B * pt.shape[1] * D:
        raise ValueError(f"contrastive_bwd: the workspace holds {ws.numel()} floats, L * B * T * D = {L * B * pt.shape[1] * D}")
    if live_tokens is None:
        _lib.check(_lib.lib().toist_contrastive_bwd_ws(_p(pq, torch.float32), _p(pt, torch.float32), _p(tok_mask, torch.int64), _p(tgt_off, torch.int32),
                                                       _p(match_off, torch.int32), _p(src_idx, torch.int64), _p(tgt_idx, torch.int64),
                                                       _p(num_boxes, torch.float32), L, B, Q, pt.shape[1], D, temperature, _p(upstream, torch.float32),
                                                       _p(dpq, torch.float32), _p(dpt, torch.float32), _p(ws, torch.float32), _stream()), "toist_contrastive_bwd_ws")
        return
    _lib.check(_lib.lib().toist_contrastive_bwd_ws_live(_p(pq, torch.float32), _p(pt, torch.float32), _p(tok_mask, torch.int64), _p(tgt_off, torch.int32),
                                                        _p(match_off, torch.int32), _p(src_idx, torch.int64), _p(tgt_idx, torch.int64),
                                                        _p(num_boxes, torch.float32), L, B, Q, pt.shape[1], D, temperature,
                                                        _p(live_tokens, torch.int32), _p(upstream, torch.float32), _p(dpq, torch.float32),
                                                        _p(dpt, torch.float32), _p(ws, torch.float32), _stream()), "toist_contrastive_bwd_ws_live")


def l2norm_fwd(x, y):
    rows, D = x.numel() // x.shape[-1], x.shape[-1]
    _lib.check(_lib.lib().toist_l2norm_fwd(_p(x, torch.float32), rows, D, _p(y, torch.float32), _stream()), "toist_l2norm_fwd")


def l2norm_bwd(x, dy, dx):
    rows, D = x.numel() // x.shape[-1], x.shape[-1]
    _lib.check(_lib.lib().toist_l2norm_bwd(_p(x, torch.float32), _p(dy, torch.float32), rows, D, _p(dx, torch.float32), _stream()), "toist_l2norm_bwd")


BF16, F32 = torch.bfloat16, torch.float32


def attnmap_softmax_fwd(scores, key_pad, B, Q, H, HW, ld, out):
    _lib.check(_lib.lib().toist_attnmap_softmax_fwd(_p(scores, BF16), _p(key_pad, torch.uint8), B, Q, H, HW, ld, _p(out, BF16), _stream()),
               "toist_attnmap_softmax_fwd")


def attnmap_softmax_bwd(prob, dprob, BQ, H, HW, ld, dscores):
    _lib.check(_lib.lib().toist_attnmap_softmax_bwd(_p(prob, BF16), _p(dprob, BF16), BQ, H, HW, ld, _p(dscores, BF16), _stream()),
               "toist_attnmap_softmax_bwd")


def groupnorm_fwd(x, gamma, beta, N, HW, C, G, eps, relu, y, stats):
    _lib.check(_lib.lib().toist_groupnorm_fwd(_p(x, BF16), _p(gamma, F32), _p(beta, F32), N, HW, C, G, eps, 1 if relu else 0, _p(y, BF16),
                                              _p(stats, F32), _stream()), "toist_groupnorm_fwd")


def groupnorm_apply(x, stats, gamma, beta, N, HW, C, G, eps, relu, y):
    _lib.check(_lib.lib().toist_groupnorm_apply(_p(x, BF16), _p(stats, F32), _p(gamma, F32), _p(beta, F32), N, HW, C, G, eps, 1 if relu else 0, _p(y, BF16),
                                                _stream()), "toist_groupnorm_apply")


def groupnorm_bwd(dy, y, x, stats, gamma, N, HW, C, G, eps, relu, dx, dgamma, dbeta, bstats, beta=None):
    _lib.check(_lib.lib().toist_groupnorm_bwd(_p(dy, BF16), _p(y, BF16), _p(x, BF16), _p(stats, F32), _p(gamma, F32), _p(beta, F32), N, HW, C, G, eps,
                                              1 if relu else 0, _p(dx, BF16), _p(dgamma, F32), _p(dbeta, F32), _p(bstats, F32), _stream()),
               "toist_groupnorm_bwd")


def upsample_add(inp, fpn, BQ, Q, H, W, C, out):
    _lib.check(_lib.lib().toist_upsample_add(_p(inp, BF16), _p(fpn, BF16), BQ, Q, H, W, C, _p(out, BF16), _stream()), "toist_upsample_add")


def resize_add(inp, fpn, rows, n, Q, H, W, OH, OW, C, out):
    _lib.check(_lib.lib().toist_resize_add(_p(inp, BF16), _p(fpn, BF16), _p(rows, torch.int64), n, Q, H, W, OH, OW, C, _p(out, BF16), _stream()), "toist_resize_add")


def resize_add_bwd(dout, BQ, H, W, OH, OW, C, din):
    _lib.check(_lib.lib().toist_resize_add_bwd(_p(dout, BF16), BQ, H, W, OH, OW, C, _p(din, BF16), _stream()), "toist_resize_add_bwd")


def upsample_add_rows(inp, fpn, rows, n, Q, H, W, C, out):
    _lib.check(_lib.lib().toist_upsample_add_rows(_p(inp, BF16), _p(fpn, BF16), _p(rows, torch.int64), n, Q, H, W, C, _p(out, BF16), _stream()),
               "toist_upsample_add_rows")


def mask_stage_fwd(src, src_stats, gamma, beta, fpn_conv, w, bias, out, out_stats, N, Q, H, W, c_in, c_out, w_rows, gn_in, up, eps=1e-5):
    _lib.check(_lib.lib().toist_mask_stage_fwd(_p(src, BF16), _p(src_stats, F32), _p(gamma, F32), _p(beta, F32), _p(fpn_conv, BF16), _p(w, BF16), _p(bias, F32),
                                               _p(out, F32 if c_out == 1 else BF16), _p(out_stats, F32), N, Q, H, W, c_in, c_out, w_rows,
                                               1 if gn_in else 0, 1 if up else 0, eps, _stream()), "toist_mask_stage_fwd")


def upsample_add_bwd(dout, BQ, H, W, C, din):
    _lib.check(_lib.lib().toist_upsample_add_bwd(_p(dout, BF16), BQ, H, W, C, _p(din, BF16), _stream()), "toist_upsample_add_bwd")


def sum_queries(inp, B, Q, per, out):
    _lib.check(_lib.lib().toist_sum_queries(_p(inp, BF16), B, Q, per, _p(out, BF16), _stream()), "toist_sum_queries")


def mask_loss_fwd(pred, pred_row, gt, gt_row, T, h, w, TH, TW, alpha, sums, valid_hw=None):
    _lib.check(_lib.lib().toist_mask_loss_fwd(_p(pred, F32), _p(pred_row, torch.int32), _p(gt, torch.uint8), _p(gt_row, torch.int32), T, h, w, TH,
                                              TW, alpha, _p(sums, F32), _p(valid_hw, torch.int32), _stream()), "toist_mask_loss_fwd")


def sum_segments(inp, seg, B, rows, per, out):
    _lib.check(_lib.lib().toist_sum_segments(_p(inp, BF16), _p(seg, torch.int32), B, rows, per, _p(out, BF16), _stream()), "toist_sum_segments")


def mask_loss_bwd(pred, pred_row, gt, gt_row, T, h, w, TH, TW, alpha, sums, coef, dpred, compact=False, valid_hw=None):
    if compact:
        _lib.check(_lib.lib().toist_mask_loss_bwd_compact(_p(pred, F32), _p(pred_row, torch.int32), _p(gt, torch.uint8), _p(gt_row, torch.int32), T, h, w,
                                                          TH, TW, alpha, _p(sums, F32), _p(coef, F32), _p(dpred, F32), _p(valid_hw, torch.int32), _stream()), "toist_mask_loss_bwd_compact")
        return
    _lib.check(_lib.lib().toist_mask_loss_bwd(_p(pred, F32), _p(pred_row, torch.int32), _p(gt, torch.uint8), _p(gt_row, torch.int32), T, h, w, TH,
                                              TW, alpha, _p(sums, F32), _p(coef, F32), _p(dpred, F32), _p(valid_hw, torch.int32), _stream()), "toist_mask_loss_bwd")


def opt_chunk_elems():
    return int(_lib.lib().toist_opt_chunk_elems())


def opt_sqnorm(table, grads, chunks, n_chunks, partial):
    _lib.check(_lib.lib().toist_opt_sqnorm(_p(table, torch.uint8), _p(grads, torch.int64), _p(chunks, torch.int32), n_chunks,
                                           _p(partial, torch.float32), _stream()), "toist_opt_sqnorm")


def opt_finish_norm(partial, n_chunks, max_norm, beta1, beta2, state):
    _lib.check(_lib.lib().toist_opt_finish_norm(_p(partial, torch.float32), n_chunks, max_norm, beta1, beta2, _p(state, torch.uint8),
                                                _stream()), "toist_opt_finish_norm")


def opt_finish_norm_guarded(partial, n_chunks, max_norm, beta1, beta2, state, veto_i32, n_veto_i32, veto_f32, n_veto_f32):
    _lib.check(_lib.lib().toist_opt_finish_norm_guarded(_p(partial, torch.float32), n_chunks, max_norm, beta1, beta2, _p(state, torch.uint8),
                                                        _p(veto_i32, torch.int64), n_veto_i32, _p(veto_f32, torch.int64), n_veto_f32, _stream()),
               "toist_opt_finish_norm_guarded")


def opt_adamw_ema(table, grads, chunks, n_chunks, groups, state, beta1, beta2, eps, ema_decay, max_blocks=0):
    _lib.check(_lib.lib().toist_opt_adamw_ema_blocks(_p(table, torch.uint8), _p(grads, torch.int64), _p(chunks, torch.int32), n_chunks,
                                                     _p(groups, torch.float32), _p(state, torch.uint8), beta1, beta2, eps, ema_decay, max_blocks, _stream()),
               "toist_opt_adamw_ema")


def lsap(cost, offset, rows, cols, n, max_rows, max_cols, max_cells, out_off, row_idx, col_idx, status, ld=0):
    _lib.check(_lib.lib().toist_lsap(_p(cost, torch.float32), _p(offset, torch.int64), _p(rows, torch.int32), _p(cols, torch.int32), ld, n, max_rows,
                                     max_cols, max_cells, _p(out_off, torch.int64), _p(row_idx, torch.int64), _p(col_idx, torch.int64),
                                     _p(status, torch.int32), _stream()), "toist_lsap")


def conv3x3_small(dgrad, src, w, shift, res, out, n_img, H, W, c_src, c_out):
    w_co, w_ci = int(w.shape[0]), int(w.shape[3])
    _lib.check(_lib.lib().toist_conv3x3_small(1 if dgrad else 0, _p(src, torch.bfloat16), _p(w, torch.bfloat16), _p(shift, torch.float32),
                                              _p(res, torch.bfloat16), _p(out, torch.bfloat16), n_img, H, W, c_src, c_out, w_co, w_ci, _stream()),
               "toist_conv3x3_small")


def wgrad3x3_small(dy, x, out, defer=False, accumulate=True):
    n_img, H, W, C = x.shape
    Co = dy.shape[-1]
    blocks = int(_lib.lib().toist_wgrad3x3_small_blocks())
    ws = FOLDS.acquire(blocks * Co * 9 * C, x.device, (out,))
    _lib.check(_lib.lib().toist_wgrad3x3_small(_p(dy, torch.bfloat16), _p(x, torch.bfloat16), _p(ws, torch.float32), n_img, H, W, C, Co, _stream()),
               "toist_wgrad3x3_small")
    FOLDS.queue(ws.data_ptr(), out, blocks, Co, 9 * C, 9 * C, accumulate=accumulate)
    if not defer:
        flush_reductions()


def attn2_splits(Sk):
    return int(_lib.lib().toist_attn2_splits(Sk))


def attn2_fwd(q, kmat, v, key_pad, B, H, Sq, Sk, dh, scale, drop_p, seed, ctx, lse):
    _lib.check(_lib.lib().toist_attn2_fwd(_p(q, torch.bfloat16), q.stride(0), _p(kmat, torch.bfloat16), kmat.stride(0), _p(v, torch.bfloat16), v.stride(0),
                                          _p(key_pad, torch.uint8), B, H, Sq, Sk, dh, scale, drop_p, seed, _p(SEED_DEV) if drop_p > 0 else None,
                                          _p(ctx, torch.bfloat16), ctx.stride(0), _p(lse, torch.float32), _stream()), "toist_attn2_fwd")


def attn2_bwd(q, kmat, v, ctx, dctx, lse, key_pad, B, H, Sq, Sk, dh, scale, drop_p, seed, dq, dk, dv, dq_part=None):
    _lib.check(_lib.lib().toist_attn2_bwd(_p(q, torch.bfloat16), q.stride(0), _p(kmat, torch.bfloat16), kmat.stride(0), _p(v, torch.bfloat16), v.stride(0),
                                          _p(ctx, torch.bfloat16), ctx.stride(0), _p(dctx, torch.bfloat16), dctx.stride(0), _p(lse, torch.float32),
                                          _p(key_pad, torch.uint8), B, H, Sq, Sk, dh, scale, drop_p, seed, _p(SEED_DEV) if drop_p > 0 else None,
                                          _p(dq, torch.bfloat16), dq.stride(0) if dq is not None else 0, _p(dk, torch.bfloat16), dk.stride(0),
                                          _p(dv, torch.bfloat16), dv.stride(0), _p(dq_part, torch.bfloat16), _stream()), "toist_attn2_bwd")


def rowgemm(a, w, out, *, b_kind, epi, K=None, bias=None, res=None, res2=None, drop_p=0.0, drop_seed=0, gamma=None, beta=None, eps=1e-5,
            z=None, mean=None, rstd=None, add=None, out2=None, fold=None, fold_cols=0, dgamma=None, dbeta=None):
    M = a.shape[0]
    d = _lib.RowGemm()
    d.M, d.K, d.b_kind, d.epi = M, (a.shape[1] if K is None else K), b_kind, epi
    d.a, d.lda, d.w, d.ldw = _p(a, torch.bfloat16), a.stride(0), _p(w, torch.bfloat16), w.stride(0)
    if fold is not None:
        d.fold, d.fold_parts, d.fold_cols, d.fold_stride = _p(fold, torch.bfloat16), fold.shape[0], fold_cols, fold.stride(0)
        assert fold.shape[1] == M and fold.shape[2] == fold_cols and fold.stride(1) == fold_cols
    d.bias = _p(bias, torch.float32)
    if res is not None:
        d.res, d.ldr = _p(res, torch.bfloat16), res.stride(0)
    if res2 is not None:
        d.res2, d.ldr2 = _p(res2, torch.bfloat16), res2.stride(0)
    d.drop_p, d.eps, d.drop_seed = drop_p, eps, drop_seed
    d.drop_seed_dev = _p(SEED_DEV) if drop_p > 0 else None
    d.gamma, d.beta = _p(gamma, torch.float32), _p(beta, torch.float32)
    for name, t in (("z", z), ("add", add), ("out2", out2)):
        if t is not None:
            assert t.is_contiguous() and t.shape[-1] == 256
            setattr(d, name, _p(t, torch.bfloat16))
    d.mean, d.rstd = _p(mean, torch.float32), _p(rstd, torch.float32)
    d.out, d.ldo = _p(out, torch.bfloat16), out.stride(0)
    keep = None
    if epi == _lib.ROW_LN_BWD and dgamma is not None:
        keep = _queue_ln_param_grads(int(_lib.lib().toist_rowgemm_blocks(M)), 256, dgamma, dbeta)
        d.partials = _p(keep, torch.float32)
    _lib.check(_lib.lib().toist_rowgemm(ctypes.byref(d), _stream()), "toist_rowgemm")
    return keep


ROW_PLAIN, ROW_LN_FWD, ROW_LN_BWD = _lib.ROW_PLAIN, _lib.ROW_LN_FWD, _lib.ROW_LN_BWD


XDEC_PROF = None
XDEC_TEST_ABSENT = 0
XDEC_LAUNCHES = 0
XDEC_FAILED = False
_XDEC_CTL = {}


def _xdec_ctl(device, create=True):
    ctl = _XDEC_CTL.get(device)
    if ctl is None and create:
        if torch.cuda.is_current_stream_capturing():
            return None
        ctl = _XDEC_CTL[device] = torch.zeros(_lib.XDEC_CTL_WORDS, dtype=torch.int32, device=device)
    return ctl


def _ranks_share_a_device():
    import torch.distributed as dist
    if not (dist.is_available() and dist.is_initialized()):
        return False
    local = os.environ.get("LOCAL_WORLD_SIZE")
    local = int(local) if local and local.isdigit() else dist.get_world_size()
    return local > torch.cuda.device_count()


def xdec_supported(B, Q, S, L, ff=2048):
    if XDEC_FAILED or ff != 2048 or _ranks_share_a_device():
        return False
    if not _lib.lib().toist_xdec_supported(B, Q, S, L):
        return False
    return _xdec_ctl(torch.device("cuda", torch.cuda.current_device())) is not None


def xdec_fwd(B, Q, S, x0, qpos, kv, key_pad, drop_p, eps, out, layers, part, *, xe0):
    d = _lib.Xdec()
    d.B, d.Q, d.S, d.L = B, Q, S, len(layers)
    d.ff, d.test_absent = int(layers[0]["w1"].shape[0]), XDEC_TEST_ABSENT
    assert all(tuple(ly["w1"].shape) == (d.ff, 256) and tuple(ly["w2"].shape) == (256, d.ff) for ly in layers)
    d.x0, d.qpos, d.kv, d.ldkv = _p(x0, torch.bfloat16), _p(qpos, torch.bfloat16), _p(kv, torch.bfloat16), kv.stride(0)
    assert xe0.is_contiguous() and xe0.shape == qpos.shape
    d.xe0 = _p(xe0, torch.bfloat16)
    d.key_pad = _p(key_pad, torch.uint8) if key_pad is not None else None
    d.drop_p, d.eps = drop_p, eps
    d.seed_dev = _p(SEED_DEV) if drop_p > 0 else None
    for name in ("qkv", "ctx_s", "z1", "y1", "y1e", "qc", "ctx_c", "z3", "y3", "h", "z4", "y4", "y4e"):
        t = out[name]
        assert t.is_contiguous()
        setattr(d, name, _p(t, torch.bfloat16))
    for name in ("lse_s", "mean1", "rstd1", "lse_c", "mean3", "rstd3", "mean4", "rstd4"):
        t = out[name]
        assert t.is_contiguous()
        setattr(d, name, _p(t, torch.float32))
    assert part.is_contiguous() and part.numel() >= B * 32 * 128 * 256
    d.part = _p(part, torch.bfloat16)
    d.ctl = _xdec_ctl(x0.device).data_ptr()
    d.prof = XDEC_PROF.data_ptr() if XDEC_PROF is not None else None
    for i, ly in enumerate(layers):
        e = d.layer[i]
        for name in ("w_in", "w_os", "w_q", "w_oc", "w1", "w2"):
            t = ly[name]
            assert t.is_contiguous()
            setattr(e, name, _p(t, torch.bfloat16))
        for name in ("b_in", "b_os", "g1", "be1", "b_q", "b_oc", "g3", "be3", "b1", "b2", "g4", "be4"):
            t = ly[name]
            assert t.is_contiguous()
            setattr(e, name, _p(t, torch.float32))
        for j in range(6):
            e.seed[j] = ly["seed"][j]
    global XDEC_LAUNCHES
    XDEC_LAUNCHES += 1
    _lib.check(_lib.lib().toist_xdec_fwd(ctypes.byref(d), _stream()), "toist_xdec_fwd")
# ... 598 lines not shown
```

toist_amd/optim.py:

```python
import numpy as np
import torch

from . import _lib, engine
from . import kernels as k
from .knobs import knob

LATE_BLOCKS = knob("TOIST_LATE_BLOCKS", 0)

_TENSOR_DT = np.dtype([("p", "<i8"), ("m", "<i8"), ("v", "<i8"), ("ema", "<i8"), ("w", "<i8"), ("row_scale", "<i8"),
                       ("numel", "<i8"), ("row_len", "<i4"), ("group", "<i4")])
assert _TENSOR_DT.itemsize == 64
_GROUP_DT = np.dtype([("lr", "<f4"), ("weight_decay", "<f4")])
_STATE_DT = np.dtype([("clip_coef", "<f4"), ("grad_norm", "<f4"), ("bias1", "<f4"), ("bias2_sqrt", "<f4"),
                      ("step", "<i4"), ("skipped", "<i4"), ("skipped_total", "<i4"), ("veto_mask", "<i4")])


def ema_pairs(model, model_ema):
    if hasattr(model, "module"):
        model = model.module
    msd = model.state_dict()
    return [(msd[name], ev) for name, ev in model_ema.state_dict().items() if ev.is_floating_point()]


def _dense(t):
    return t.is_contiguous() or (t.dim() == 4 and t.is_contiguous(memory_format=torch.channels_last))


import weakref as _weakref

_LIVE_TAILS = _weakref.WeakSet()
CARRY_OTHER_TAILS = True


class FusedClipAdamWEMA:

    MAX_VETO = _lib.CONSTANTS["TOIST_OPT_MAX_VETO"]

    def __init__(self, param_groups, lr=1e-4, betas=(0.9, 0.999), eps=1e-8, weight_decay=1e-4, max_norm=0.1, ema=None, ema_decay=0.9998,
                 defer_ema=False, skip_nonfinite=False):
        if isinstance(param_groups, (list, tuple)) and param_groups and torch.is_tensor(param_groups[0]):
            param_groups = [{"params": list(param_groups)}]
        self.param_groups = []
        for g in param_groups:
            g = dict(g)
            g["params"] = [p for p in g["params"]]
            g.setdefault("lr", lr)
            g.setdefault("weight_decay", weight_decay)
            self.param_groups.append(g)
        self.betas, self.eps, self.max_norm, self.ema_decay = (float(betas[0]), float(betas[1])), float(eps), float(max_norm), float(ema_decay)
        params = [p for g in self.param_groups for p in g["params"]]
        if not params:
            raise ValueError("FusedClipAdamWEMA: no parameters")
        self.device = params[0].device
        if self.device.type != "cuda":
            raise RuntimeError("FusedClipAdamWEMA needs GPU tensors: toist_amd has no CPU fallback")
        self.params = params
        self.exp_avg = [torch.zeros_like(p) for p in params]
        self.exp_avg_sq = [torch.zeros_like(p) for p in params]
        ema = list(ema or [])
        by_ptr = {src.data_ptr(): e for src, e in ema}
        self._ema_of = [by_ptr.pop(p.data_ptr(), None) for p in params]
        self._ema_only = [(src, e) for src, e in ema if src.data_ptr() in by_ptr]
        self._group_of = [gi for gi, g in enumerate(self.param_groups) for _ in g["params"]]
        self._late = [bool(g.get("late", False)) for g in self.param_groups for _ in g["params"]]
        self._early = [bool(g.get("early_norm", False)) and not bool(g.get("late", False)) for g in self.param_groups for _ in g["params"]]
        self._param_ids = frozenset(id(p) for p in params)
        _LIVE_TAILS.add(self)
        self._early_ids = frozenset(id(p) for p, e in zip(params, self._early) if e)
        self._early_idx = [i for i, e in enumerate(self._early) if e]
        self._early_done = False
        self._e_lo = self._e_hi = 0
        if self._early_ids:
            import weakref
            from . import functions
            ref = weakref.ref(self)

            def hook(prog_params, _ref=ref):
                o = _ref()
                if o is not None:
                    o._maybe_norm_early(prog_params)

            functions.AFTER_BACKWARD[:] = [h for h in functions.AFTER_BACKWARD if getattr(h, "_owner", lambda: None)() is not None]
            hook._owner = ref
            functions.AFTER_BACKWARD.append(hook)
        self._late_pending = False
        self._late_captured = False
        self._late_grads = None
        self._n_now = self._n_late = 0
        if any(self._late):
            if defer_ema:
                raise ValueError("FusedClipAdamWEMA: late groups and defer_ema are alternatives")
            engine.register_text_prelude(self, [p for p, l in zip(params, self._late) if l])
        for t in params + self.exp_avg + [e for e in self._ema_of if e is not None] + [x for pr in self._ema_only for x in pr]:
            if t.dtype != torch.float32 or not _dense(t) or t.device != self.device:
                raise TypeError("FusedClipAdamWEMA: tensors must be dense fp32 tensors on one GPU")
        for p, e in zip(params, self._ema_of):
            if e is not None and (e.shape != p.shape or e.stride() != p.stride()):
                raise ValueError("FusedClipAdamWEMA: an EMA tensor must share its source's shape and strides")
        self.state = torch.zeros(_STATE_DT.itemsize, dtype=torch.uint8, device=self.device)
        self.skip_nonfinite = bool(skip_nonfinite)
        self._veto_words = ([], [])
        self._veto_dev = tuple(torch.zeros(self.MAX_VETO, dtype=torch.int64, device=self.device) for _ in range(2)) if self.skip_nonfinite else None
        self._groups_host = None
        self._groups_dev = torch.zeros(len(self.param_groups), len(_GROUP_DT.names), dtype=torch.float32, device=self.device)
        self._chunk = k.opt_chunk_elems()
        n_t = len(params) + len(self._ema_only)
        self._grads_host = [torch.zeros(n_t, dtype=torch.int64).pin_memory() for _ in range(2)]
        self._grads_event = [None, None]
        self._grads_turn = 0
        self._grads_last = None
        self._grads_dev = torch.zeros(n_t, dtype=torch.int64, device=self.device)
        self._table = None
        self._chunks = self._partial = self._ema_table = self._ema_chunks = self._ema_grads = None
        self._retired = []
        self.defer_ema = bool(defer_ema) and (any(e is not None for e in self._ema_of) or bool(self._ema_only))
        self._ema_pending = False
        self._copy_gen = -1
        self._copies = []
        self.sync_hyperparams()

    def sync_hyperparams(self):
        cur = [(float(g["lr"]), float(g["weight_decay"])) for g in self.param_groups]
        if cur != self._groups_host:
            self._groups_host = cur
            rows = np.array(cur, dtype=_GROUP_DT)
            self._groups_dev.copy_(torch.from_numpy(rows.view(np.float32).reshape(len(rows), -1)), non_blocking=False)

    def _build_table(self):
        rows = np.zeros(len(self.params) + len(self._ema_only), dtype=_TENSOR_DT)
        engine.prune_copies()
        self._copies = []
        for i, p in enumerate(self.params):
            r = rows[i]
            r["p"], r["m"], r["v"] = p.data_ptr(), self.exp_avg[i].data_ptr(), self.exp_avg_sq[i].data_ptr()
            r["ema"] = self._ema_of[i].data_ptr() if self._ema_of[i] is not None else 0
            r["numel"], r["group"], r["row_len"] = p.numel(), self._group_of[i], 1
            ent = engine.copy_of(p)
            if ent is not None and ent.elementwise and ent.w.numel() == p.numel():
                r["w"] = ent.w.data_ptr()
                if ent.row_scale is not None:
                    r["row_scale"] = ent.row_scale.data_ptr()
                    r["row_len"] = p.numel() // p.shape[0]
                self._copies.append((ent, p))
        for j, (src, e) in enumerate(self._ema_only):
            r = rows[len(self.params) + j]
            r["p"], r["ema"], r["numel"], r["row_len"] = src.data_ptr(), e.data_ptr(), src.numel(), 1

        def chunked(rr):
            numels = rr["numel"]
            nch = (numels + self._chunk - 1) // self._chunk
            tens = np.repeat(np.arange(len(rr), dtype=np.int32), nch)
            first = np.repeat(np.cumsum(nch) - nch, nch)
            idx = (np.arange(int(nch.sum()), dtype=np.int64) - first).astype(np.int32)
            ch = np.ascontiguousarray(np.stack([tens, idx], axis=1).astype(np.int32))
            return torch.from_numpy(rr.view(np.uint8).copy()).to(self.device), torch.from_numpy(ch).to(self.device), int(ch.shape[0])

        def keep(name, new):
            cur = getattr(self, name, None)
            if cur is not None and cur.shape == new.shape and cur.dtype == new.dtype:
                cur.copy_(new)
                return
            if cur is not None:
                self._retired.append(cur)
            setattr(self, name, new)

        if self.defer_ema:
            erows = rows[rows["ema"] != 0].copy()
            erows["m"], erows["v"], erows["w"], erows["row_scale"] = 0, 0, 0, 0
            et, ec, self._n_ema_chunks = chunked(erows)
            keep("_ema_table", et)
            keep("_ema_chunks", ec)
            keep("_ema_grads", torch.zeros(len(erows), dtype=torch.int64, device=self.device))
            rows = rows[:len(self.params)].copy()
            rows["ema"] = 0
        table, chunks, self._n_chunks = chunked(rows)
        keep("_table", table)
        late_rows = torch.tensor(self._late + [False] * len(self._ema_only), dtype=torch.bool, device=self.device)
        early_rows = torch.tensor(self._early + [False] * len(self._ema_only), dtype=torch.bool, device=self.device)
        is_late = late_rows[chunks[:, 0].long()]
        is_early = early_rows[chunks[:, 0].long()]
        keep("_chunks", torch.cat([chunks[~is_late & ~is_early], chunks[is_early], chunks[is_late]], dim=0).contiguous())
        self._n_late = int(is_late.sum())
        self._n_now = self._n_chunks - self._n_late
        self._e_hi = self._n_now
        self._e_lo = self._n_now - int(is_early.sum())
        self._late_copies = [(ent, p_) for ent, p_ in self._copies if any(p_ is q for q, l in zip(self.params, self._late) if l)]
        keep("_partial", torch.empty(self._n_chunks, dtype=torch.float32, device=self.device))
        self._copy_gen = engine.COPY_GEN

    def add_veto(self, word):
        if not self.skip_nonfinite:
            raise ValueError("FusedClipAdamWEMA.add_veto needs skip_nonfinite=True")
        if not torch.is_tensor(word) or word.numel() != 1 or word.device != self.device or word.dtype not in (torch.int32, torch.float32):
            raise TypeError("FusedClipAdamWEMA.add_veto: a one-element int32 or fp32 tensor on the optimizer's device")
        kind = 0 if word.dtype == torch.int32 else 1
        words = self._veto_words[kind]
        for j, w in enumerate(words):
            if w.data_ptr() == word.data_ptr():
                return 1 << (1 + self.MAX_VETO * kind + j)
        if len(words) >= self.MAX_VETO:
            raise ValueError(f"FusedClipAdamWEMA.add_veto: at most {self.MAX_VETO} {'fp32' if kind else 'int32'} veto words")
        words.append(word)
        self._veto_dev[kind].copy_(torch.tensor([w.data_ptr() for w in words] + [0] * (self.MAX_VETO - len(words)), dtype=torch.int64))
        return 1 << (1 + self.MAX_VETO * kind + len(words) - 1)

    def zero_grad(self, set_to_none=True):
        if not set_to_none:
            self.flush_late()
        self._early_done = False
        for p in self.params:
            if set_to_none:
                p.grad = None
            elif p.grad is not None:
                p.grad.zero_()

    @torch.no_grad()
    def step(self):
        capturing = torch.cuda.is_current_stream_capturing()
        if self._late_pending and not self._late_captured:
            self.flush_late()
        self._late_captured = False
        if self._table is None or (self._copy_gen != engine.COPY_GEN and not capturing):
            self._build_table()
        if not capturing:
            self.sync_hyperparams()
        if self._ema_pending:
            self.ema_update()
        turn = self._grads_turn
        if self._grads_event[turn] is not None and not capturing:
            self._grads_event[turn].synchronize()
        gh = self._grads_host[turn].numpy()
        for i, p in enumerate(self.params):
            g = p.grad
            if g is None:
                gh[i] = 0
                continue
            if g.dtype != torch.float32 or g.shape != p.shape or g.stride() != p.stride():
                raise TypeError("FusedClipAdamWEMA: every gradient must be fp32 with its parameter's shape and strides")
            gh[i] = g.data_ptr()
        if self._grads_last is None or capturing or not np.array_equal(gh, self._grads_last):
            self._grads_dev.copy_(self._grads_host[turn], non_blocking=True)
            if not capturing:
                ev = self._grads_event[turn] or torch.cuda.Event()
                ev.record()
                self._grads_event[turn] = ev
            self._grads_last = gh.copy()
            self._grads_turn = turn ^ 1
        if self._early_done and self._e_hi > self._e_lo:
            if self._e_lo:
                k.opt_sqnorm(self._table, self._grads_dev, self._chunks, self._e_lo, self._partial)
            if self._n_chunks > self._e_hi:
                k.opt_sqnorm(self._table, self._grads_dev, self._chunks[self._e_hi:], self._n_chunks - self._e_hi, self._partial[self._e_hi:])
        else:
            k.opt_sqnorm(self._table, self._grads_dev, self._chunks, self._n_chunks, self._partial)
        self._early_done = False
        if self.skip_nonfinite:
            k.opt_finish_norm_guarded(self._partial, self._n_chunks, self.max_norm, self.betas[0], self.betas[1], self.state,
                                      self._veto_dev[0], len(self._veto_words[0]), self._veto_dev[1], len(self._veto_words[1]))
        else:
            k.opt_finish_norm(self._partial, self._n_chunks, self.max_norm, self.betas[0], self.betas[1], self.state)
        if self._n_now:
            k.opt_adamw_ema(self._table, self._grads_dev, self._chunks, self._n_now, self._groups_dev, self.state, self.betas[0],
                            self.betas[1], self.eps, self.ema_decay)
        self._ema_pending = self.defer_ema
        self._bump_epoch()
        if self._n_late:
            self._late_pending = True
            self._late_grads = [p.grad for p, l in zip(self.params, self._late) if l]

    def note_replayed_step(self):
        self._bump_epoch()

    def _bump_epoch(self):
        old = engine.WEIGHT_EPOCH
        engine.bump_weight_epoch()
        late_ids = {id(p_) for _, p_ in self._late_copies} if self._n_late else ()
        for ent, p in self._copies:
            if p.grad is not None and id(p) not in late_ids:
                ent.epoch = engine.WEIGHT_EPOCH
        for other in list(_LIVE_TAILS) if CARRY_OTHER_TAILS else ():
            if other is self:
                continue
            for ent, p in getattr(other, "_copies", ()):
                if ent.epoch == old and id(p) not in self._param_ids:
                    ent.epoch = engine.WEIGHT_EPOCH

    @torch.no_grad()
    def _maybe_norm_early(self, prog_params):
        if not self._early_ids or self._table is None or self._grads_last is None or self._e_hi <= self._e_lo:
            return
        if not any(id(p) in self._early_ids for p in prog_params):
            return
        self._early_done = False
        if self._copy_gen != engine.COPY_GEN and not torch.cuda.is_current_stream_capturing():
            return
        last = self._grads_last
        for i in self._early_idx:
            g = self.params[i].grad
            if (0 if g is None else g.data_ptr()) != int(last[i]):
                return
        k.opt_sqnorm(self._table, self._grads_dev, self._chunks[self._e_lo:], self._e_hi - self._e_lo, self._partial[self._e_lo:])
        self._early_done = True

    @torch.no_grad()
    def flush_late(self):
        capturing = torch.cuda.is_current_stream_capturing()
        if not self._n_late or not (self._late_pending or capturing) or (capturing and self._late_captured):
            return
        k.opt_adamw_ema(self._table, self._grads_dev, self._chunks[self._n_now:], self._n_late, self._groups_dev, self.state, self.betas[0],
                        self.betas[1], self.eps, self.ema_decay, max_blocks=LATE_BLOCKS)
        for ent, p in self._late_copies:
            ent.epoch = engine.WEIGHT_EPOCH
        if not capturing:
            self._late_pending = False
            self._late_grads = None
        else:
            self._late_captured = True

    def finish(self):
        self.flush_late()
        if self._ema_pending:
            self.ema_update()

    @torch.no_grad()
    def ema_update(self):
        if not self._ema_pending:
            return
        if self._table is None:
            self._build_table()
        k.opt_adamw_ema(self._ema_table, self._ema_grads, self._ema_chunks, self._n_ema_chunks, self._groups_dev, self.state, self.betas[0],
                        self.betas[1], self.eps, self.ema_decay)
        self._ema_pending = False

    def device_state(self):
        s = self.state.cpu().numpy().view(_STATE_DT)[0]
        return {n: bool(s[n]) if n == "skipped" else s[n].item() for n in _STATE_DT.names}

    def state_dict(self):
        self.finish()
        step = self.device_state()["step"]
        state = {i: {"step": torch.tensor(float(step)), "exp_avg": self.exp_avg[i].clone(), "exp_avg_sq": self.exp_avg_sq[i].clone()}
                 for i in range(len(self.params))} if step > 0 else {}
        groups, base = [], 0
        for g in self.param_groups:
            d = {kk: vv for kk, vv in g.items() if kk != "params"}
            d.update(betas=self.betas, eps=self.eps, amsgrad=False, maximize=False)
            d["params"] = list(range(base, base + len(g["params"])))
            base += len(g["params"])
            groups.append(d)
        return {"state": state, "param_groups": groups}

    def load_state_dict(self, sd):
        self.finish()
        if "state" not in sd and "exp_avg" in sd:
            sd = {"state": {i: {"step": sd["step"], "exp_avg": a, "exp_avg_sq": b} for i, (a, b) in enumerate(zip(sd["exp_avg"], sd["exp_avg_sq"]))},
                  "param_groups": sd.get("param_groups", [])}
        steps = []
        for i, st in sd["state"].items():
            i = int(i)
            self.exp_avg[i].copy_(st["exp_avg"].reshape(self.exp_avg[i].shape) if st["exp_avg"].shape != self.exp_avg[i].shape else st["exp_avg"])
            self.exp_avg_sq[i].copy_(st["exp_avg_sq"].reshape(self.exp_avg_sq[i].shape) if st["exp_avg_sq"].shape != self.exp_avg_sq[i].shape else st["exp_avg_sq"])
            steps.append(int(float(st["step"])))
        if steps and min(steps) != max(steps):
            raise ValueError("FusedClipAdamWEMA.load_state_dict: parameters with different step counts (the fused tail keeps one counter)")
        raw = np.zeros(1, dtype=_STATE_DT)
        raw["step"] = steps[0] if steps else 0
        self.state.copy_(torch.from_numpy(raw.view(np.uint8)))
        for g, src in zip(self.param_groups, sd.get("param_groups", [])):
            g.update({kk: vv for kk, vv in src.items() if kk in ("lr", "weight_decay", "initial_lr")})
        self.sync_hyperparams()
```

toist_amd/parallel.py:

```python
import torch
import torch.distributed as dist

from . import functions


class GradSync:

    def __init__(self, model=None, process_group=None, static_set=False):
        if model is not None and not isinstance(model, (torch.nn.Module, list, tuple)):
            model, process_group = None, model
        self.models = [] if model is None else (list(model) if isinstance(model, (list, tuple)) else [model])
        self.group = process_group
        self.pending = []
        self.ranges = []
        self.world = dist.get_world_size(process_group) if dist.is_available() and dist.is_initialized() else 1
        self.static_set = static_set
        self._agreed = None

    def __enter__(self):
        if self.world > 1:
            functions.GRAD_SYNC = self._launch
        return self

    def __exit__(self, *exc):
        functions.GRAD_SYNC = None
        return False

    def _launch(self, flat):
        if flat is None:
            return
        op = _mean_op(self.group)
        work = dist.all_reduce(flat, op=op, group=self.group, async_op=True)
        self.pending.append((work, flat, op))
        self.ranges.append((flat.data_ptr(), flat.data_ptr() + flat.numel() * flat.element_size()))

    def _local_states(self, params):
        state = []
        for p in params:
            g = p.grad
            if g is None:
                state.append(0)
            else:
                a = g.data_ptr()
                state.append(1 if any(lo <= a < hi for lo, hi in self.ranges) else 2)
        return state

    def _agree(self, params, state):
        if self.static_set and self._agreed is not None:
            if self._agreed[0] != state:
                raise RuntimeError("GradSync(static_set=True): this rank's gradient states changed since the first step; use the default (agreement every step)")
            return self._agreed[1]
        dev = next((p.grad.device for p in params if p.grad is not None), params[0].device)
        onehot = torch.zeros(len(params), 3, dtype=torch.int32)
        onehot[torch.arange(len(params)), torch.tensor(state, dtype=torch.int64)] = 1
        counts = onehot.to(dev)
        dist.all_reduce(counts, op=dist.ReduceOp.SUM, group=self.group)
        counts = counts.cpu()
        conflict = ((counts[:, 1] > 0) & (counts[:, 2] > 0)).nonzero().flatten().tolist()
        if conflict:
            raise RuntimeError("GradSync: %d parameter gradient(s) travelled in a flat program buffer on some ranks and stand-alone on others "
                               "(first index %d): the ranks ran different backward schedules; zero the gradients on every rank before the step "
                               "or accumulate on all of them" % (len(conflict), conflict[0]))
        alone = (counts[:, 2] > 0).nonzero().flatten().tolist()
        if self.static_set:
            self._agreed = (list(state), alone)
        return alone

    def finish(self):
        for work, flat, op in self.pending:
            work.wait()
            if op == dist.ReduceOp.SUM:
                flat.div_(self.world)
        rest = []
        if self.world > 1 and self.models:
            params = [q for m in self.models for q in m.parameters() if q.requires_grad]
            if params:
                try:
                    for i in self._agree(params, self._local_states(params)):
                        p = params[i]
                        if p.grad is None:
                            p.grad = torch.zeros_like(p)
                        rest.append(p.grad)
                finally:
                    self.pending, self.ranges = [], []
        if rest:
            all_reduce_mean(rest, self.group)
        self.pending, self.ranges = [], []


def _mean_op(group=None):
    return dist.ReduceOp.AVG if dist.get_backend(group) == "nccl" else dist.ReduceOp.SUM


class _MeanHandle:
    def __init__(self, works, flats, op, world, wire=None):
        self.works, self.flats, self.op, self.world, self.wire = works, flats, op, world, wire

    def wait(self):
        for w in self.works:
            w.wait()
        if self.wire is not None:
            for f, t in zip(self.flats, self.wire):
                f.copy_(t)
        if self.op == dist.ReduceOp.SUM:
            for f in self.flats:
                f.div_(self.world)


def all_reduce_mean_async(flats, group=None, bf16=False):
    op = _mean_op(group)
    wire = [f.to(torch.bfloat16) for f in flats] if bf16 else None
    works = [dist.all_reduce(t, op=op, group=group, async_op=True) for t in (wire if bf16 else flats)]
    return _MeanHandle(works, list(flats), op, dist.get_world_size(group), wire)


def measure_all_reduce(flats, group=None, iters=5, bf16=False):
    import time
    world = dist.get_world_size(group)
    nbytes = sum(f.numel() * (2 if bf16 else f.element_size()) for f in flats)
    scratch = [torch.zeros_like(f) for f in flats]
    all_reduce_mean_async(scratch, group, bf16).wait()
    torch.cuda.synchronize()
    dist.barrier(group)
    t0 = time.perf_counter()
    for _ in range(iters):
        all_reduce_mean_async(scratch, group, bf16).wait()
    torch.cuda.synchronize()
    dt = (time.perf_counter() - t0) / iters
    alg = nbytes / dt / 1e9
    return {"bytes": nbytes, "ms": round(1000 * dt, 3), "algbw_GBps": round(alg, 1), "busbw_GBps": round(alg * 2 * (world - 1) / world, 1)}


def all_reduce_mean(flats, group=None):
    all_reduce_mean_async(flats, group).wait()


def enable_backward_cuts(model, on=True):
    getattr(model, "detr", model).split_backward = bool(on)


BACKWARD_CUTS = ("text", "backbone", "backbone.layer3", "backbone.layer2")


def backward_cut(memory_cache, name):
    cut = memory_cache.get("_native", {}).get("cuts", {}).get(name)
    if not cut:
        return
    pairs = [(src, leaf.grad) for src, leaf in zip(*cut) if leaf.grad is not None and src.requires_grad]
    if pairs:
        torch.autograd.backward([s for s, _ in pairs], [g for _, g in pairs])


def broadcast_parameters(module, src=0, group=None):
    if not (dist.is_available() and dist.is_initialized()) or dist.get_world_size(group) < 2:
        return
    with torch.no_grad():
        for t in list(module.parameters()) + list(module.buffers()):
            dist.broadcast(t.data, src=src, group=group)


class DistributedDataParallel(torch.nn.Module):

    def __init__(self, module, device_ids=None, output_device=None, find_unused_parameters=False, process_group=None, broadcast_buffers=True,
                 **unused):
        super().__init__()
        self.module = module
        self.process_group = process_group
        self.require_backward_grad_sync = True
        self._sync = GradSync(module, process_group)
        self._queued = False
        broadcast_parameters(module, 0, process_group)

    def forward(self, *args, **kwargs):
        functions.GRAD_SYNC = None
        if self.require_backward_grad_sync and self._sync.world > 1 and torch.is_grad_enabled():
            functions.GRAD_SYNC = self._on_flat
        return self.module(*args, **kwargs)

    def _on_flat(self, flat):
        if not self._queued:
            self._queued = True
            torch.autograd.Variable._execution_engine.queue_callback(self._finish)
        self._sync._launch(flat)

    def _finish(self):
        functions.GRAD_SYNC = None
        self._queued = False
        self._sync.finish()

    class _NoSync:
        def __init__(self, ddp):
            self.ddp = ddp

        def __enter__(self):
            self.old, self.ddp.require_backward_grad_sync = self.ddp.require_backward_grad_sync, False

        def __exit__(self, *exc):
            self.ddp.require_backward_grad_sync = self.old
            return False

    def no_sync(self):
        return DistributedDataParallel._NoSync(self)
```

toist_amd/transformer.py:

```python
from collections import OrderedDict
from types import SimpleNamespace

import torch
from torch import nn

from . import engine, functions, tlayer
from . import kernels as k

BF16 = torch.bfloat16


class MHAParams(nn.Module):

    def __init__(self, d_model, nhead, dropout=0.0):
        super().__init__()
        self.embed_dim, self.num_heads, self.dropout = d_model, nhead, dropout
        self.in_proj_weight = nn.Parameter(torch.empty(3 * d_model, d_model))
        self.in_proj_bias = nn.Parameter(torch.zeros(3 * d_model))
        self.out_proj = nn.Linear(d_model, d_model)
        nn.init.xavier_uniform_(self.in_proj_weight)
        nn.init.zeros_(self.out_proj.bias)


class TransformerEncoderLayer(nn.Module):
# ... 218 lines not shown
    tgt = engine.Var(torch.zeros(B * Q, d, dtype=BF16, device=dev), needs_grad=False)
    stack = torch.empty(n_layers, B * Q, d, dtype=BF16, device=dev)
    inter = []
    for i in range(n_layers):
        lp = f"layers.{i}."
        Ws, bs = ps[lp + "self_attn.in_proj_weight"], ps[lp + "self_attn.in_proj_bias"]
        Wc, bc = ps[lp + "cross_attn_image.in_proj_weight"], ps[lp + "cross_attn_image.in_proj_bias"]
        qk = engine.add_vars(tape, tgt, qpos)
        z1 = engine.attention(tape, qk, qk, tgt, None, None, (Ws.rows(2 * d, 3 * d), bs.rows(2 * d, 3 * d)),
                              ps[lp + "self_attn.out_proj.weight"], ps[lp + "self_attn.out_proj.bias"], tgt, None, B, Q, Q, H,
                              packed_qk=(Ws.rows(0, 2 * d), bs.rows(0, 2 * d)))
        t1 = engine.layernorm(tape, z1, ps[lp + "norm1.weight"], ps[lp + "norm1.bias"], 1e-5)
        q2 = engine.add_vars(tape, t1, qpos)
        z3 = engine.attention(tape, q2, mem_pos, mem, (Wc.rows(0, d), bc.rows(0, d)), (Wc.rows(d, 2 * d), bc.rows(d, 2 * d)),
                              (Wc.rows(2 * d, 3 * d), bc.rows(2 * d, 3 * d)), ps[lp + "cross_attn_image.out_proj.weight"],
                              ps[lp + "cross_attn_image.out_proj.bias"], t1, key_pad, B, Q, S, H)
        t3 = engine.layernorm(tape, z3, ps[lp + "norm3.weight"], ps[lp + "norm3.bias"], 1e-5)
        z4 = engine.linear_chain(tape, t3, [(ps[lp + "linear1.weight"], ps[lp + "linear1.bias"], k.ACT_RELU, True),
                                            (ps[lp + "linear2.weight"], ps[lp + "linear2.bias"], k.ACT_NONE, False)],
                                 res=t3, final_drop=True)
        tgt = engine.layernorm(tape, z4, ps[lp + "norm4.weight"], ps[lp + "norm4.bias"], 1e-5)
        inter.append(engine.layernorm(tape, tgt, ps["norm.weight"], ps["norm.bias"], 1e-5, y=stack[i]))
    hs = engine.Var(stack)

    def split_bwd():
        g = hs.take_grad()
        if g is None:
            return
        for i, v in enumerate(inter):
            v.grad = g[i]

    tape.record(split_bwd)
    return [hs], None


class Transformer(nn.Module):
    def __init__(self, args=None, d_model=512, nhead=8, num_encoder_layers=6, num_decoder_layers=6, dim_feedforward=2048,
                 dropout=0.1, activation="relu", normalize_before=False, return_intermediate_dec=False, pass_pos_and_query=True,
                 text_encoder_type="roberta-base", freeze_text_encoder=False, contrastive_loss=False):
        super().__init__()
        if normalize_before:
            raise NotImplementedError("pre-norm is not on the hot path (the reference decoder asserts False)")
        if activation != "relu":
            raise NotImplementedError("only relu FFNs are on the hot path")
        if not pass_pos_and_query:
            raise NotImplementedError("pass_pos_and_query=False is not on the hot path")
        self.args = args
        self.pass_pos_and_query = True
        self.encoder = TransformerEncoder([TransformerEncoderLayer(d_model, nhead, dim_feedforward, dropout) for _ in range(num_encoder_layers)])
        self.decoder = TransformerDecoder([TransformerDecoderLayer(d_model, nhead, dim_feedforward, dropout) for _ in range(num_decoder_layers)], d_model)
        self.CLS = nn.Embedding(1, d_model) if contrastive_loss else None
        if contrastive_loss:
            raise NotImplementedError("--contrastive_loss (CLS token) is off in every TOIST recipe; not on the hot path")
        for p in self.parameters():
            if p.dim() > 1:
                nn.init.xavier_uniform_(p)
        self._tokenizer = None
        self.text_encoder_type = text_encoder_type
        without_pretrain = bool(getattr(args, "without_pretrain", False)) if args is not None else True
        if without_pretrain:
            self.text_encoder = RobertaTextEncoder(roberta_config())
        else:
            self.text_encoder = self._from_pretrained(text_encoder_type)
        if freeze_text_encoder:
            for p in self.text_encoder.parameters():
                p.requires_grad_(False)
        self.expander_dropout = 0.1
        self.resizer = FeatureResizer(self.text_encoder.config.hidden_size, d_model, self.expander_dropout)
        self.d_model, self.nhead, self.dropout = d_model, nhead, dropout
        self._cache_text, self._cache_enc, self._cache_dec = {}, {}, {}
        self._step = 0

    @staticmethod
    def _from_pretrained(name):
        try:
            from transformers import RobertaModel
            hf = RobertaModel.from_pretrained(name)
        except Exception as e:
            raise RuntimeError(f"pretrained text encoder {name!r} is unavailable offline; pass args.without_pretrain=True "
                               f"or load a TOIST checkpoint ({e})")
        c = hf.config
        enc = RobertaTextEncoder(roberta_config(vocab_size=c.vocab_size, hidden_size=c.hidden_size, num_hidden_layers=c.num_hidden_layers,
                                                num_attention_heads=c.num_attention_heads, intermediate_size=c.intermediate_size,
                                                max_position_embeddings=c.max_position_embeddings, type_vocab_size=c.type_vocab_size,
                                                layer_norm_eps=c.layer_norm_eps, pad_token_id=c.pad_token_id))
        enc.load_state_dict(hf.state_dict(), strict=False)
        return enc

    @property
    def tokenizer(self):
        if self._tokenizer is None:
            try:
                from transformers import RobertaTokenizerFast
                self._tokenizer = RobertaTokenizerFast.from_pretrained(self.text_encoder_type)
            except Exception as e:
                raise RuntimeError("RobertaTokenizerFast files are unavailable offline: pass pre-tokenised captions "
                                   f"(dict with input_ids / attention_mask) instead of strings ({e})")
        return self._tokenizer

    @tokenizer.setter
    def tokenizer(self, value):
        self._tokenizer = value

    def _next_seed(self):
        self._step += 1
        return self._step

    def encode_text(self, tokenized):
        engine.run_text_prelude(self.text_encoder.embeddings.word_embeddings.weight)
        ids = tokenized["input_ids"]
        att = tokenized["attention_mask"]
        B, L = ids.shape
        te, cfg = self.text_encoder, self.text_encoder.config
        H = cfg.num_attention_heads
        ids = ids.contiguous()
        if ids.dtype == torch.int64 and att.dtype == torch.int64:
            pos_ids, key_pad = k.text_prep(ids, att.contiguous(), cfg.pad_token_id)
        else:
            keep = ids.ne(cfg.pad_token_id).to(torch.int64)
            pos_ids = (torch.cumsum(keep, dim=1) * keep + cfg.pad_token_id).contiguous()
            key_pad = att.ne(1).to(torch.uint8).contiguous()
        ids_flat = ids.view(-1)
        def _named():
            d = OrderedDict(("text_encoder." + n, p) for n, p in te.named_parameters())
            d.update(("resizer." + n, p) for n, p in self.resizer.named_parameters())
            return d
        named = engine.named_cache(self, "text", _named)

        small = engine.FUSED_BLOCKS and L <= 64 and cfg.hidden_size // H <= 64 and (cfg.hidden_size // H) % 8 == 0
        packs = self.__dict__.setdefault("_text_packs", {})
        key_dev = str(ids.device)
        if key_dev not in packs or packs[key_dev][2] != id(self):
            Dh = cfg.hidden_size
            bufs = [torch.zeros(3 * Dh, Dh, dtype=BF16, device=ids.device) for _ in range(cfg.num_hidden_layers)]
            tr = {}
            for i, buf in enumerate(bufs):
                for j, nm in enumerate(("query", "key", "value")):
                    tr[f"text_encoder.encoder.layer.{i}.attention.self.{nm}.weight"] = engine.packed_cast(buf[j * Dh:(j + 1) * Dh])
            packs[key_dev] = (bufs, tr, id(self))
        pack_bufs, transforms = packs[key_dev][:2]

        def prog(tape, ps):
            P = lambda n: ps["text_encoder." + n]
            D = cfg.hidden_size
            x0 = torch.empty(B * L, D, dtype=BF16, device=ids.device)
            wv, pv, tv = P("embeddings.word_embeddings.weight"), P("embeddings.position_embeddings.weight"), P("embeddings.token_type_embeddings.weight")
            k.embed_fwd(ids_flat, pos_ids.view(-1), wv.f32, pv.f32, tv.f32[0], x0)
            emb = engine.Var(x0)

            def emb_bwd():
                g = emb.take_grad()
                if g is None or wv.g is None:
                    return
                k.embed_bwd(g, ids_flat, pos_ids.view(-1), cfg.pad_token_id, wv.g, pv.g, tv.g[0] if tv.g is not None else None)

            tape.record(emb_bwd)
            x = engine.layernorm(tape, emb, P("embeddings.LayerNorm.weight"), P("embeddings.LayerNorm.bias"), cfg.layer_norm_eps)
            x = engine.dropout(tape, x)
            for i in range(cfg.num_hidden_layers):
                lp = f"encoder.layer.{i}."
                if small:
                    proj = [(P(lp + f"attention.self.{nm}.weight"), P(lp + f"attention.self.{nm}.bias")) for nm in ("query", "key", "value")]
                    z = engine.text_attention_block(tape, x, proj, pack_bufs[i], P(lp + "attention.output.dense.weight"),
                                                    P(lp + "attention.output.dense.bias"), key_pad, B, L, H)
                else:
                  z = engine.attention(
                    tape, x, x, x, (P(lp + "attention.self.query.weight"), P(lp + "attention.self.query.bias")),
                    (P(lp + "attention.self.key.weight"), P(lp + "attention.self.key.bias")),
                    (P(lp + "attention.self.value.weight"), P(lp + "attention.self.value.bias")), P(lp + "attention.output.dense.weight"),
                    P(lp + "attention.output.dense.bias"), x, key_pad, B, L, L, H)
                x1 = engine.layernorm(tape, z, P(lp + "attention.output.LayerNorm.weight"), P(lp + "attention.output.LayerNorm.bias"), cfg.layer_norm_eps)
                z2 = engine.linear_chain(tape, x1, [(P(lp + "intermediate.dense.weight"), P(lp + "intermediate.dense.bias"), k.ACT_GELU, False),
                                                    (P(lp + "output.dense.weight"), P(lp + "output.dense.bias"), k.ACT_NONE, False)],
                                         res=x1, final_drop=True)
                x = engine.layernorm(tape, z2, P(lp + "output.LayerNorm.weight"), P(lp + "output.LayerNorm.bias"), cfg.layer_norm_eps)
            r = engine.linear_chain(tape, x, [(ps["resizer.fc.weight"], ps["resizer.fc.bias"], k.ACT_NONE, False)])
            r = engine.layernorm(tape, r, ps["resizer.layer_norm.weight"], ps["resizer.layer_norm.bias"], 1e-12)
            r = engine.dropout(tape, r)
            return [r], None

        (out,) = functions.run_program(prog, named, [], cache=self._cache_text, training=self.training, drop_p=cfg.hidden_dropout_prob,
                                       seed=self._next_seed(), group_wgrads=True, transforms=transforms,
                                       store_once=lambda n, t: t.dim() == 2 and "embeddings" not in n)
        return out, key_pad

    def encode_tokens(self, tokens, pos, key_pad, B, S):
        d, H = self.d_model, self.nhead
        named = engine.named_cache(self, "encoder", lambda: OrderedDict(self.encoder.named_parameters()))
        n_layers = self.encoder.num_layers

        def prog(tape, ps, x):
            program = tlayer.encoder_program if tlayer.supported(d, H, S) else per_op_encoder_program
            return program(tape, ps, x, pos, key_pad, B, S, H, n_layers)

        (out,) = functions.run_program(prog, named, [tokens], cache=self._cache_enc, training=self.training, drop_p=self.dropout,
                                       seed=self._next_seed(), group_wgrads=True, store_once=lambda n, t: t.dim() == 2)
        return out

    def decode_tokens(self, memory, pos, key_pad, query_embed, B, S):
        d, H = self.d_model, self.nhead
        Q = query_embed.shape[0]
        named = engine.named_cache(self, "decoder", lambda: OrderedDict(self.decoder.named_parameters()))
        n_layers = self.decoder.num_layers

        def prog(tape, ps, mem, qe):
            program = tlayer.decoder_program if tlayer.supported(d, H, max(S, Q)) else per_op_decoder_program
            return program(tape, ps, mem, qe, pos, key_pad, B, S, Q, H, n_layers)

        def run():
            (o,) = functions.run_program(prog, named, [memory, query_embed], cache=self._cache_dec, training=self.training,
                                         drop_p=self.dropout, seed=self._next_seed(), group_wgrads=True, store_once=lambda n, t: t.dim() == 2)
            return o

        launches = k.XDEC_LAUNCHES
        out = run()
        if (k.XDEC_LAUNCHES != launches and not self.training and not torch.is_grad_enabled() and not torch.cuda.is_current_stream_capturing()):
            torch.cuda.current_stream().synchronize()
            if k.xdec_check(raise_on_failure=False):
                import warnings
                warnings.warn("toist_xdec: the XCD-resident decoder launch found its workgroups not co-resident (is the GPU shared?); "
                              "repeating the decoder on the per-op launches and keeping them for the rest of this process")
                out = run()
        return out

    def forward(self, src=None, mask=None, query_embed=None, pos_embed=None, text=None, encode_and_save=True, text_memory=None,
                img_memory=None, text_attention_mask=None):
        if encode_and_save:
            bs, c, h, w = src.shape
            tokens_img = src.flatten(2).permute(0, 2, 1).to(BF16)
            pos_img = pos_embed.flatten(2).permute(0, 2, 1).to(BF16)
            return self.encode_native(tokens_img, pos_img, mask.flatten(1), query_embed, text)
        stack = self.decode_native(img_memory, pos_embed, mask, query_embed)
        L, B = stack.shape[0], img_memory.shape[1]
        return stack.view(L, B, -1, stack.shape[-1]).float()

    def _tokenize(self, text, device):
        if isinstance(text, (list, tuple)) and len(text) and isinstance(text[0], str):
            tok = self.tokenizer(list(text), padding="longest", return_tensors="pt").to(device)
            return tok
        if isinstance(text, dict) or hasattr(text, "input_ids"):
            keep = isinstance(text, TokenizedText) or (hasattr(text, "char_to_token") and hasattr(text, "to"))
            tok = text if keep else TokenizedText({"input_ids": text["input_ids"], "attention_mask": text["attention_mask"]})
            return tok.to(device)
        raise TypeError("captions must be list[str] or a dict with input_ids / attention_mask")

    def encode_native(self, tokens_img, pos_img, mask_img, query_embed, text):
        B, HW, d = tokens_img.shape
        dev = tokens_img.device
        pre_encoded = isinstance(text, tuple) and len(text) == 3 and torch.is_tensor(text[0])
        if pre_encoded:
            text_attention_mask, text_memory_resized, tokenized = text
            text_tok = text_memory_resized.permute(1, 0, 2).to(BF16)
            L = text_tok.shape[1]
        else:
            key_pad_text = None
            if isinstance(text, EncodedText):
                tokenized, flat, key_pad_text = text.tokenized, text.flat, text.key_pad
            else:
                tokenized = self._tokenize(text, dev)
                flat, key_pad_text = self.encode_text(tokenized)
            L = tokenized["input_ids"].shape[1]
            text_tok = flat.view(B, L, d)
            text_attention_mask = key_pad_text.view(torch.bool) if key_pad_text is not None else tokenized["attention_mask"].ne(1).bool()
            text_memory_resized = None
        S = HW + L
        tokens = torch.cat([tokens_img, text_tok], dim=1).reshape(B * S, d)
        if pos_img.shape[1] == S:
            pos = pos_img.reshape(B * S, d)
        else:
            pos = torch.cat([pos_img, torch.zeros(B, L, d, dtype=BF16, device=dev)], dim=1).reshape(B * S, d).contiguous()
        mask = torch.cat([mask_img, text_attention_mask], dim=1)
        return self.encode_sequences(tokens, pos, mask, B, S, L, query_embed, tokenized, text_attention_mask, text_tok, text_memory_resized)

    def encode_sequences(self, tokens, pos, mask, B, S, L, query_embed, tokenized, text_attention_mask, text_tok, text_memory_resized=None):
        d = tokens.shape[-1]
        key_pad = mask.view(torch.uint8)
        mem = self.encode_tokens(tokens, pos, key_pad, B, S)
        mem3 = mem.view(B, S, d)
        native = {"memory": mem, "pos": pos, "key_pad": key_pad, "B": B, "S": S, "L": L, "img_memory_ref": None, "query_embed": query_embed}

        def img_memory():
            t = mem3.permute(1, 0, 2).float()
            native["img_memory_ref"] = t
            return t

        out = MemoryCache({"text_pooled_op": None, "img_pooled_op": None, "mask": mask, "text_attention_mask": text_attention_mask, "tokenized": tokenized,
                           "_native": native},
                          lazy={"img_memory": img_memory, "pos_embed": lambda: pos.view(B, S, d).permute(1, 0, 2).float(),
                                "query_embed": lambda: query_embed.unsqueeze(1).repeat(1, B, 1)})
        out._lazy["text_memory"] = lambda: out["img_memory"][-L:]
        if text_memory_resized is not None:
            out["text_memory_resized"] = text_memory_resized
        else:
            out._lazy["text_memory_resized"] = lambda: text_tok.permute(1, 0, 2).float()
        return out

    def decode_native(self, img_memory, pos_embed, mask, query_embed, native=None):
        if native is not None and (img_memory is None or native.get("img_memory_ref") is img_memory):
            mem, pos, key_pad, B, S = native["memory"], native["pos"], native["key_pad"], native["B"], native["S"]
        else:
            S, B, d = img_memory.shape
            mem = img_memory.permute(1, 0, 2).reshape(B * S, d).to(BF16)
            pos = pos_embed.permute(1, 0, 2).reshape(B * S, d).to(BF16).contiguous()
            key_pad = mask.to(torch.uint8).contiguous()
        qe = query_embed[:, 0, :] if query_embed.dim() == 3 else query_embed
        stack = self.decode_tokens(mem, pos, key_pad, qe, B, S)
        return stack


def build_transformer(args):
    return Transformer(args=args, d_model=args.hidden_dim, dropout=args.dropout, nhead=args.nheads, dim_feedforward=args.dim_feedforward,
                       num_encoder_layers=args.enc_layers, num_decoder_layers=args.dec_layers, normalize_before=args.pre_norm,
                       return_intermediate_dec=True, pass_pos_and_query=args.pass_pos_and_query, text_encoder_type=args.text_encoder_type,
                       freeze_text_encoder=args.freeze_text_encoder, contrastive_loss=args.contrastive_loss)
```

Before: 714.3 images/s.

## Track touched embedding chunks to skip grad clear, norm and cold Adam work

```diff
diff --git a/include/toist_hip.h b/include/toist_hip.h
--- a/include/toist_hip.h
+++ b/include/toist_hip.h
@@ -144,6 +144,10 @@
                     int n, int D, void* out, void* stream);
 TOIST_API int toist_embed_bwd(const void* g, const int64_t* ids, const int64_t* pos_ids, int n, int D, int64_t pad_id, float* dword,
                     float* dpos, float* dtype0, void* stream);
+TOIST_API int toist_embed_bwd_sparse(const void* g, const int64_t* ids, const int64_t* pos_ids, int n, int D, int64_t pad_id, float* dword,
+                    float* dpos, float* dtype0, uint8_t* touched_word, uint8_t* touched_pos, int chunk, void* stream);
+TOIST_API int toist_sparse_clear(float* g0, uint8_t* touched0, int64_t numel0, float* g1, uint8_t* touched1, int64_t numel1, int chunk,
+                    void* stream);
 
 TOIST_API int toist_criterion_fwd(const float* logits, const float* boxes, const float* tgt_boxes, const float* pos_map,
                         const int32_t* tgt_off, const int32_t* match_off, const int64_t* src_idx, const int64_t* tgt_idx,
@@ -454,6 +458,11 @@
 TOIST_API int toist_opt_adamw_ema_blocks(const toist_opt_tensor* table, const int64_t* grads, const int32_t* chunks, int n_chunks,
                                const toist_opt_group* groups, const toist_opt_state* state, float beta1, float beta2, float eps,
                                float ema_decay, int max_blocks, void* stream);
+TOIST_API int toist_opt_sqnorm_sparse(const toist_opt_tensor* table, const int64_t* grads, const int64_t* touched, const int32_t* chunks,
+                               int n_chunks, float* partial, void* stream);
+TOIST_API int toist_opt_adamw_ema_sparse(const toist_opt_tensor* table, const int64_t* grads, const int64_t* touched, const int64_t* hot,
+                               const int32_t* chunks, int n_chunks, const toist_opt_group* groups, const toist_opt_state* state,
+                               float beta1, float beta2, float eps, float ema_decay, int max_blocks, void* stream);
 
 TOIST_API int toist_mask_resize_pack(const float* src, int n, int h0, int w0, int max_h, int max_w, int crop_h, int crop_w, int h, int w,
                            float threshold, uint64_t* bits, void* stream);
diff --git a/toist_amd/csrc/optim.hip b/toist_amd/csrc/optim.hip
--- a/toist_amd/csrc/optim.hip
+++ b/toist_amd/csrc/optim.hip
@@ -13,10 +13,15 @@
 }
 
 __global__ __launch_bounds__(256) void sqnorm_kernel(const toist_opt_tensor* __restrict__ T, const int64_t* __restrict__ G,
-                                                     const int2* __restrict__ chunks, float* __restrict__ partial) {
+                                                     const int64_t* __restrict__ TCH, const int2* __restrict__ chunks,
+                                                     float* __restrict__ partial) {
     __shared__ float red[4];
     const int2 ch = chunks[blockIdx.x];
     const float* g = reinterpret_cast<const float*>(G[ch.x]);
+    if (g != nullptr && TCH != nullptr) {
+        const uint8_t* touched = reinterpret_cast<const uint8_t*>(TCH[ch.x]);
+        if (touched != nullptr && touched[ch.y] == 0) g = nullptr;
+    }
     float acc = 0.f;
     if (g != nullptr) {
         const long long beg = (long long)ch.y * OPT_CHUNK;
@@ -122,7 +127,100 @@
     p -= step_size * (m / denom);
 }
 
+__device__ __forceinline__ float opaque_zero() {
+    float z = 0.f;
+    asm volatile("" : "+v"(z));
+    return z;
+}
+
+template <bool COLD>
+__device__ __forceinline__ void adamw_ema_chunk(const toist_opt_tensor& t, const float* g, long long beg, int n, const toist_opt_group gr,
+                                                const toist_opt_state* __restrict__ st, float b1, float b2, float eps, float decay,
+                                                uint8_t* hot_flag) {
+    const float coef = st->clip_coef, bias2_sqrt = st->bias2_sqrt;
+    const float lr = gr.lr, wd = gr.weight_decay, step_size = lr / st->bias1;
+    float* p = t.p + beg;
+    const bool upd = COLD || (g != nullptr && t.m != nullptr);
+    const bool vec = (((size_t)p | (size_t)(g ? g + beg : nullptr) | (size_t)(t.m ? t.m + beg : nullptr) | (size_t)(t.v ? t.v + beg : nullptr) |
+                       (size_t)(t.ema ? t.ema + beg : nullptr)) & 15) == 0 &&
+                     (t.w == nullptr || (((size_t)(t.w + beg)) & 7) == 0);
+    const int n4 = vec ? (n >> 2) : 0;
+    for (int i = threadIdx.x; i < n4; i += 256) {
+        float4 pv = reinterpret_cast<float4*>(p)[i];
+        if (upd) {
+            float4 gv, mv, vv;
+            if (COLD) {
+                gv = make_float4(opaque_zero(), opaque_zero(), opaque_zero(), opaque_zero());
+                mv = make_float4(opaque_zero(), opaque_zero(), opaque_zero(), opaque_zero());
+                vv = make_float4(opaque_zero(), opaque_zero(), opaque_zero(), opaque_zero());
+            } else {
+                gv = reinterpret_cast<const float4*>(g + beg)[i];
+                mv = reinterpret_cast<float4*>(t.m + beg)[i];
+                vv = reinterpret_cast<float4*>(t.v + beg)[i];
+            }
+            adamw_one(pv.x, gv.x * coef, mv.x, vv.x, lr, wd, b1, b2, eps, step_size, bias2_sqrt);
+            adamw_one(pv.y, gv.y * coef, mv.y, vv.y, lr, wd, b1, b2, eps, step_size, bias2_sqrt);
+            adamw_one(pv.z, gv.z * coef, mv.z, vv.z, lr, wd, b1, b2, eps, step_size, bias2_sqrt);
+            adamw_one(pv.w, gv.w * coef, mv.w, vv.w, lr, wd, b1, b2, eps, step_size, bias2_sqrt);
+            reinterpret_cast<float4*>(p)[i] = pv;
+            if (!COLD || ((__float_as_uint(mv.x) | __float_as_uint(mv.y) | __float_as_uint(mv.z) | __float_as_uint(mv.w) | __float_as_uint(vv.x) |
+                           __float_as_uint(vv.y) | __float_as_uint(vv.z) | __float_as_uint(vv.w)) != 0u)) {
+                reinterpret_cast<float4*>(t.m + beg)[i] = mv;
+                reinterpret_cast<float4*>(t.v + beg)[i] = vv;
+                if (COLD) *hot_flag = 1;
+            }
+        }
+        if (t.ema != nullptr) {
+            float4 ev = reinterpret_cast<float4*>(t.ema + beg)[i];
+            ev.x = ev.x * decay + (1.f - decay) * pv.x;
+            ev.y = ev.y * decay + (1.f - decay) * pv.y;
+            ev.z = ev.z * decay + (1.f - decay) * pv.z;
+            ev.w = ev.w * decay + (1.f - decay) * pv.w;
+            reinterpret_cast<float4*>(t.ema + beg)[i] = ev;
+        }
+        if (upd && t.w != nullptr) {
+            float s = 1.f;
+            const long long e0 = beg + ((long long)i << 2);
+            if (t.row_scale != nullptr) {
+                const long long r0 = e0 / t.row_len;
+                if ((e0 + 3) / t.row_len == r0) s = t.row_scale[r0];
+                else {
+                    pv.x *= t.row_scale[e0 / t.row_len];
+                    pv.y *= t.row_scale[(e0 + 1) / t.row_len];
+                    pv.z *= t.row_scale[(e0 + 2) / t.row_len];
+                    pv.w *= t.row_scale[(e0 + 3) / t.row_len];
+                }
+            }
+            reinterpret_cast<uint2*>(t.w + beg)[i] = make_uint2(pack2bf(pv.x * s, pv.y * s), pack2bf(pv.z * s, pv.w * s));
+        }
+    }
+    for (int i = (n4 << 2) + threadIdx.x; i < n; i += 256) {
+        float pv = p[i];
+        if (upd) {
+            float gs, mv, vv;
+            if (COLD) {
+                gs = opaque_zero(), mv = opaque_zero(), vv = opaque_zero();
+            } else {
+                gs = g[beg + i], mv = t.m[beg + i], vv = t.v[beg + i];
+            }
+            adamw_one(pv, gs * coef, mv, vv, lr, wd, b1, b2, eps, step_size, bias2_sqrt);
+            p[i] = pv;
+            if (!COLD || (__float_as_uint(mv) | __float_as_uint(vv)) != 0u) {
+                t.m[beg + i] = mv;
+                t.v[beg + i] = vv;
+                if (COLD) *hot_flag = 1;
+            }
+        }
+        if (t.ema != nullptr) t.ema[beg + i] = t.ema[beg + i] * decay + (1.f - decay) * pv;
+        if (upd && t.w != nullptr) {
+            const float s = t.row_scale ? t.row_scale[(beg + i) / t.row_len] : 1.f;
+            t.w[beg + i] = f2bf(pv * s);
+        }
+    }
+}
+
 __global__ __launch_bounds__(256) void adamw_ema_kernel(const toist_opt_tensor* __restrict__ T, const int64_t* __restrict__ G,
+                                                        const int64_t* __restrict__ TCH, const int64_t* __restrict__ HOT,
                                                         const int2* __restrict__ chunks, const toist_opt_group* __restrict__ groups,
                                                         const toist_opt_state* __restrict__ st, float b1, float b2, float eps,
                                                         float decay, int n_chunks) {
@@ -135,68 +233,23 @@
     long long end = beg + OPT_CHUNK;
     if (end > t.numel) end = t.numel;
     const int n = (int)(end - beg);
-    const float coef = st->clip_coef, bias2_sqrt = st->bias2_sqrt;
     const toist_opt_group gr = groups[t.group];
-    const float lr = gr.lr, wd = gr.weight_decay, step_size = lr / st->bias1;
-    float* p = t.p + beg;
-    const bool upd = g != nullptr && t.m != nullptr;
-    const bool vec = (((size_t)p | (size_t)(g ? g + beg : nullptr) | (size_t)(t.m ? t.m + beg : nullptr) | (size_t)(t.v ? t.v + beg : nullptr) |
-                       (size_t)(t.ema ? t.ema + beg : nullptr)) & 15) == 0 &&
-                     (t.w == nullptr || (((size_t)(t.w + beg)) & 7) == 0);
-    const int n4 = vec ? (n >> 2) : 0;
-    for (int i = threadIdx.x; i < n4; i += 256) {
-        float4 pv = reinterpret_cast<float4*>(p)[i];
-        if (upd) {
-            float4 gv = reinterpret_cast<const float4*>(g + beg)[i];
-            float4 mv = reinterpret_cast<float4*>(t.m + beg)[i];
-            float4 vv = reinterpret_cast<float4*>(t.v + beg)[i];
-            adamw_one(pv.x, gv.x * coef, mv.x, vv.x, lr, wd, b1, b2, eps, step_size, bias2_sqrt);
-            adamw_one(pv.y, gv.y * coef, mv.y, vv.y, lr, wd, b1, b2, eps, step_size, bias2_sqrt);
-            adamw_one(pv.z, gv.z * coef, mv.z, vv.z, lr, wd, b1, b2, eps, step_size, bias2_sqrt);
-            adamw_one(pv.w, gv.w * coef, mv.w, vv.w, lr, wd, b1, b2, eps, step_size, bias2_sqrt);
-            reinterpret_cast<float4*>(p)[i] = pv;
-            reinterpret_cast<float4*>(t.m + beg)[i] = mv;
-            reinterpret_cast<float4*>(t.v + beg)[i] = vv;
-        }
-        if (t.ema != nullptr) {
-            float4 ev = reinterpret_cast<float4*>(t.ema + beg)[i];
-            ev.x = ev.x * decay + (1.f - decay) * pv.x;
-            ev.y = ev.y * decay + (1.f - decay) * pv.y;
-            ev.z = ev.z * decay + (1.f - decay) * pv.z;
-            ev.w = ev.w * decay + (1.f - decay) * pv.w;
-            reinterpret_cast<float4*>(t.ema + beg)[i] = ev;
-        }
-        if (upd && t.w != nullptr) {
-            float s = 1.f;
-            const long long e0 = beg + ((long long)i << 2);
-            if (t.row_scale != nullptr) {
-                const long long r0 = e0 / t.row_len;
-                if ((e0 + 3) / t.row_len == r0) s = t.row_scale[r0];
-                else {
-                    pv.x *= t.row_scale[e0 / t.row_len];
-                    pv.y *= t.row_scale[(e0 + 1) / t.row_len];
-                    pv.z *= t.row_scale[(e0 + 2) / t.row_len];
-                    pv.w *= t.row_scale[(e0 + 3) / t.row_len];
-                }
-            }
-            reinterpret_cast<uint2*>(t.w + beg)[i] = make_uint2(pack2bf(pv.x * s, pv.y * s), pack2bf(pv.z * s, pv.w * s));
-        }
-    }
-    for (int i = (n4 << 2) + threadIdx.x; i < n; i += 256) {
-        float pv = p[i];
-        if (upd) {
-            float mv = t.m[beg + i], vv = t.v[beg + i];
-            adamw_one(pv, g[beg + i] * coef, mv, vv, lr, wd, b1, b2, eps, step_size, bias2_sqrt);
-            p[i] = pv;
-            t.m[beg + i] = mv;
-            t.v[beg + i] = vv;
-        }
-        if (t.ema != nullptr) t.ema[beg + i] = t.ema[beg + i] * decay + (1.f - decay) * pv;
-        if (upd && t.w != nullptr) {
-            const float s = t.row_scale ? t.row_scale[(beg + i) / t.row_len] : 1.f;
-            t.w[beg + i] = f2bf(pv * s);
-        }
-    }
+    bool cold = false;
+    uint8_t* hot_flag = nullptr;
+    if (HOT != nullptr && g != nullptr && t.m != nullptr) {
+        hot_flag = reinterpret_cast<uint8_t*>(HOT[ch.x]);
+        const uint8_t* touched = reinterpret_cast<const uint8_t*>(TCH[ch.x]);
+        if (hot_flag != nullptr) {
+            hot_flag += ch.y;
+            if (touched == nullptr || touched[ch.y] != 0) {
+                if (threadIdx.x == 0) *hot_flag = 1;
+            } else {
+                cold = *reinterpret_cast<volatile uint8_t*>(hot_flag) == 0;
+            }
+        }
+    }
+    if (cold) adamw_ema_chunk<true>(t, g, beg, n, gr, st, b1, b2, eps, decay, hot_flag);
+    else adamw_ema_chunk<false>(t, g, beg, n, gr, st, b1, b2, eps, decay, hot_flag);
   }
 }
 
@@ -205,12 +258,17 @@
 using namespace toist;
 
 extern "C" int toist_opt_chunk_elems(void) { return OPT_CHUNK; }
+
+extern "C" int toist_opt_sqnorm_sparse(const toist_opt_tensor* table, const int64_t* grads, const int64_t* touched, const int32_t* chunks,
+                                       int n_chunks, float* partial, void* stream) {
+    TOIST_REQUIRE(table && grads && chunks && partial && n_chunks > 0, "toist_opt_sqnorm: bad args");
+    hipLaunchKernelGGL(sqnorm_kernel, dim3(n_chunks), dim3(256), 0, (hipStream_t)stream, table, grads, touched, (const int2*)chunks, partial);
+    return check_launch("toist_opt_sqnorm");
+}
 
 extern "C" int toist_opt_sqnorm(const toist_opt_tensor* table, const int64_t* grads, const int32_t* chunks, int n_chunks, float* partial,
                                 void* stream) {
-    TOIST_REQUIRE(table && grads && chunks && partial && n_chunks > 0, "toist_opt_sqnorm: bad args");
-    hipLaunchKernelGGL(sqnorm_kernel, dim3(n_chunks), dim3(256), 0, (hipStream_t)stream, table, grads, (const int2*)chunks, partial);
-    return check_launch("toist_opt_sqnorm");
+    return toist_opt_sqnorm_sparse(table, grads, nullptr, chunks, n_chunks, partial, stream);
 }
 
 extern "C" int toist_opt_finish_norm(const float* partial, int n_chunks, float max_norm, float beta1, float beta2, toist_opt_state* state,
@@ -234,15 +292,22 @@
     return check_launch("toist_opt_finish_norm_guarded");
 }
 
+extern "C" int toist_opt_adamw_ema_sparse(const toist_opt_tensor* table, const int64_t* grads, const int64_t* touched, const int64_t* hot,
+                                          const int32_t* chunks, int n_chunks, const toist_opt_group* groups, const toist_opt_state* state,
+                                          float beta1, float beta2, float eps, float ema_decay, int max_blocks, void* stream) {
+    TOIST_REQUIRE(table && grads && chunks && groups && state && n_chunks > 0, "toist_opt_adamw_ema: bad args");
+    TOIST_REQUIRE((touched == nullptr) == (hot == nullptr), "toist_opt_adamw_ema_sparse: touched and hot tables come together");
+    TOIST_REQUIRE(eps > 0.f && ema_decay >= 0.f && ema_decay <= 1.f, "toist_opt_adamw_ema: bad eps / ema_decay");
+    const int blocks = (max_blocks > 0 && max_blocks < n_chunks) ? max_blocks : n_chunks;
+    hipLaunchKernelGGL(adamw_ema_kernel, dim3(blocks), dim3(256), 0, (hipStream_t)stream, table, grads, touched, hot, (const int2*)chunks, groups,
+                       state, beta1, beta2, eps, ema_decay, n_chunks);
+    return check_launch("toist_opt_adamw_ema");
+}
+
 extern "C" int toist_opt_adamw_ema_blocks(const toist_opt_tensor* table, const int64_t* grads, const int32_t* chunks, int n_chunks,
                                           const toist_opt_group* groups, const toist_opt_state* state, float beta1, float beta2, float eps,
                                           float ema_decay, int max_blocks, void* stream) {
-    TOIST_REQUIRE(table && grads && chunks && groups && state && n_chunks > 0, "toist_opt_adamw_ema: bad args");
-    TOIST_REQUIRE(eps > 0.f && ema_decay >= 0.f && ema_decay <= 1.f, "toist_opt_adamw_ema: bad eps / ema_decay");
-    const int blocks = (max_blocks > 0 && max_blocks < n_chunks) ? max_blocks : n_chunks;
-    hipLaunchKernelGGL(adamw_ema_kernel, dim3(blocks), dim3(256), 0, (hipStream_t)stream, table, grads, (const int2*)chunks, groups, state,
-                       beta1, beta2, eps, ema_decay, n_chunks);
-    return check_launch("toist_opt_adamw_ema");
+    return toist_opt_adamw_ema_sparse(table, grads, nullptr, nullptr, chunks, n_chunks, groups, state, beta1, beta2, eps, ema_decay, max_blocks, stream);
 }
 
 extern "C" int toist_opt_adamw_ema(const toist_opt_tensor* table, const int64_t* grads, const int32_t* chunks, int n_chunks,
diff --git a/toist_amd/csrc/rows.hip b/toist_amd/csrc/rows.hip
--- a/toist_amd/csrc/rows.hip
+++ b/toist_amd/csrc/rows.hip
@@ -390,19 +390,23 @@
 }
 __global__ __launch_bounds__(256) void embed_bwd_kernel(const bf16_t* __restrict__ g, const long long* __restrict__ ids,
                                                          const long long* __restrict__ pos_ids, int n, int D, long long pad_id,
-                                                         float* __restrict__ dword, float* __restrict__ dpos) {
+                                                         float* __restrict__ dword, float* __restrict__ dpos, uint8_t* __restrict__ tword,
+                                                         uint8_t* __restrict__ tpos, int chunk) {
     const int lane = threadIdx.x & 63;
     const int t = blockIdx.x * 4 + (threadIdx.x >> 6);
     if (t >= n) return;
     for (int which = 0; which < 2; ++which) {
         const long long* key = which ? pos_ids : ids;
         float* table = which ? dpos : dword;
+        uint8_t* touched = which ? tpos : tword;
         if (table == nullptr) continue;
         const long long id = key[t];
         if (id == pad_id) continue;
         bool dup = false;
         for (int u = lane; u < t; u += 64) dup |= (key[u] == id);
         if (__any(dup)) continue;
+        if (touched != nullptr && lane == 0)
+            for (long long c = id * (long long)D / chunk; c <= ((id + 1) * (long long)D - 1) / chunk; ++c) touched[c] = 1;
         float* row = table + id * (long long)D;
         for (int c0 = 0; c0 < D; c0 += 64) {
             const int c = c0 + lane;
@@ -435,6 +439,26 @@
         for (int r = 0; r < 8; ++r) s += red[r][cx];
         dtype0[c] += s;
     }
+}
+
+__global__ __launch_bounds__(256) void sparse_clear_kernel(float* __restrict__ g0, uint8_t* __restrict__ t0, long long n0, int chunks0,
+                                                            float* __restrict__ g1, uint8_t* __restrict__ t1, long long n1, int chunk) {
+    const bool second = (int)blockIdx.x >= chunks0;
+    const int c = second ? (int)blockIdx.x - chunks0 : (int)blockIdx.x;
+    uint8_t* flag = (second ? t1 : t0) + c;
+    const bool set = *flag != 0;
+    __syncthreads();
+    if (!set) return;
+    const long long numel = second ? n1 : n0;
+    const long long beg = (long long)c * chunk;
+    long long end = beg + chunk;
+    if (end > numel) end = numel;
+    float* p = (second ? g1 : g0) + beg;
+    const int n = (int)(end - beg);
+    const int n4 = (((size_t)p & 15) == 0) ? (n >> 2) : 0;
+    for (int i = threadIdx.x; i < n4; i += 256) reinterpret_cast<float4*>(p)[i] = make_float4(0.f, 0.f, 0.f, 0.f);
+    for (int i = (n4 << 2) + threadIdx.x; i < n; i += 256) p[i] = 0.f;
+    if (threadIdx.x == 0) *flag = 0;
 }
 
 static inline int grid_for(long long n, int cap = 2048) {
@@ -531,13 +555,29 @@
     return check_launch("toist_embed_fwd");
 }
 
-extern "C" int toist_embed_bwd(const void* g, const int64_t* ids, const int64_t* pos_ids, int n, int D, int64_t pad_id, float* dword,
-                               float* dpos, float* dtype0, void* stream) {
-    TOIST_REQUIRE(n > 0 && D > 0, "toist_embed_bwd: bad shape");
+extern "C" int toist_embed_bwd_sparse(const void* g, const int64_t* ids, const int64_t* pos_ids, int n, int D, int64_t pad_id, float* dword,
+                                      float* dpos, float* dtype0, uint8_t* touched_word, uint8_t* touched_pos, int chunk, void* stream) {
+    TOIST_REQUIRE(n > 0 && D > 0 && chunk > 0, "toist_embed_bwd: bad shape");
     if (dword != nullptr || dpos != nullptr)
         hipLaunchKernelGGL(embed_bwd_kernel, dim3((n + 3) / 4), dim3(256), 0, (hipStream_t)stream, (const bf16_t*)g, (const long long*)ids,
-                           (const long long*)pos_ids, n, D, (long long)pad_id, dword, dpos);
+                           (const long long*)pos_ids, n, D, (long long)pad_id, dword, dpos, touched_word, touched_pos, chunk);
     if (dtype0 != nullptr)
         hipLaunchKernelGGL(embed_type_bwd_kernel, dim3((D + 31) / 32), dim3(256), 0, (hipStream_t)stream, (const bf16_t*)g, n, D, dtype0);
     return check_launch("toist_embed_bwd");
 }
+
+extern "C" int toist_embed_bwd(const void* g, const int64_t* ids, const int64_t* pos_ids, int n, int D, int64_t pad_id, float* dword,
+                               float* dpos, float* dtype0, void* stream) {
+    return toist_embed_bwd_sparse(g, ids, pos_ids, n, D, pad_id, dword, dpos, dtype0, nullptr, nullptr, 1, stream);
+}
+
+extern "C" int toist_sparse_clear(float* g0, uint8_t* touched0, int64_t numel0, float* g1, uint8_t* touched1, int64_t numel1, int chunk,
+                                  void* stream) {
+    TOIST_REQUIRE(chunk > 0 && numel0 >= 0 && numel1 >= 0 && (numel0 == 0 || (g0 && touched0)) && (numel1 == 0 || (g1 && touched1)),
+                  "toist_sparse_clear: bad args");
+    const long long c0 = (numel0 + chunk - 1) / chunk, c1 = (numel1 + chunk - 1) / chunk;
+    TOIST_REQUIRE(c0 + c1 > 0 && c0 + c1 < (1ll << 31), "toist_sparse_clear: bad size");
+    hipLaunchKernelGGL(sparse_clear_kernel, dim3((unsigned)(c0 + c1)), dim3(256), 0, (hipStream_t)stream, g0, touched0, (long long)numel0, (int)c0,
+                       g1, touched1, (long long)numel1, chunk);
+    return check_launch("toist_sparse_clear");
+}
diff --git a/toist_amd/engine.py b/toist_amd/engine.py
--- a/toist_amd/engine.py
+++ b/toist_amd/engine.py
@@ -159,6 +159,40 @@
 def copy_of(t):
     ent = COPIES.get(t.data_ptr())
     return ent if ent is not None and ent.master() is t and ent.ptr == t.data_ptr() else None
+
+
+SPARSE_TAIL = knob("TOIST_SPARSE_TAIL", True)
+TOUCHED = {}
+_OPT_CHUNK = None
+
+
+def opt_chunk():
+    global _OPT_CHUNK
+    if _OPT_CHUNK is None:
+        _OPT_CHUNK = k.opt_chunk_elems()
+    return _OPT_CHUNK
+
+
+def register_touched(g, touched):
+    for ptr in [ptr for ptr, ent in TOUCHED.items() if ent[0]() is None]:
+        del TOUCHED[ptr]
+    TOUCHED[g.data_ptr()] = (weakref.ref(g), touched)
+
+
+def touched_of(g):
+    ent = TOUCHED.get(g.data_ptr()) if g is not None and TOUCHED else None
+    return ent[1] if ent is not None and ent[0]() is g else None
+
+
+def touched_in(flat):
+    lo, hi = flat.data_ptr(), flat.data_ptr() + flat.numel() * flat.element_size()
+    return [ent[1] for ptr, ent in TOUCHED.items() if lo <= ptr < hi and ent[0]() is not None]
+
+
+def mark_all_touched(g):
+    t = touched_of(g)
+    if t is not None:
+        t.fill_(1)
 
 
 def _cast_bf16(m):
@@ -206,7 +240,7 @@
 
 class ParamView:
 
-    __slots__ = ("w", "g", "f32", "fresh", "parent", "_lo", "_hi", "_ranges")
+    __slots__ = ("w", "g", "f32", "fresh", "parent", "_lo", "_hi", "_ranges", "touched")
 
     def __init__(self, w_bf16, grad_f32, f32=None, fresh=False, parent=None, lo=None, hi=None):
         self.w = w_bf16
@@ -216,6 +250,12 @@
         self.parent = parent
         self._lo, self._hi = lo, hi
         self._ranges = []
+        self.touched = None
+
+    def mark_all_touched(self):
+        t = self._root().touched
+        if t is not None:
+            t.fill_(1)
 
     def _root(self):
         v = self
@@ -287,68 +327,91 @@
 
 class ParamSet:
 
-    def __init__(self, named, trainable, need_grads, bf16_cache=None, transforms=None, store_once=None):
+    def __init__(self, named, trainable, need_grads, bf16_cache=None, transforms=None, store_once=None, row_sparse=None):
         self.names = list(named.keys())
         self.views = {}
-        self.zero_elems = 0
+        self.zero_elems = self.fresh_off = 0
+        self.sparse = []
+        fp32_only = frozenset(row_sparse or ()) if SPARSE_TAIL else frozenset()
         memo = bf16_cache.get("__layout__") if bf16_cache is not None else None
         params = list(named.values())
         sig = (need_grads, len(params), tuple(trainable.get(n, False) for n in self.names), id(params[0]) if params else 0,
                params[0].data_ptr() if params else 0, id(params[-1]) if params else 0, params[-1].data_ptr() if params else 0,
-               STORE_ONCE and store_once is not None)
+               STORE_ONCE and store_once is not None, fp32_only)
         if REUSE_GRAD_BUFFERS and memo is not None and memo["sig"] == sig and need_grads and memo["flat"] is not None:
             lo, hi = memo["flat"].data_ptr(), memo["flat"].data_ptr() + memo["flat"].numel() * 4
             if not any(p.grad is not None and lo <= p.grad.data_ptr() < hi for p in params):
                 self.flat = memo["flat"]
-                self.zero_elems = memo["zero_elems"]
-                self._clear()
+                self.zero_elems, self.fresh_off, self.sparse = memo["zero_elems"], memo["fresh_off"], memo["sparse"]
+                self._clear(reused=True)
                 for n, t in named.items():
                     pv = memo["views"][n]
                     pv.written = False
-                    if t.dim() >= 2:
+                    if t.dim() >= 2 and n not in fp32_only:
                         pv.w = compute_copy(t, (transforms or {}).get(n) or _cast_bf16, bf16_cache, n)
                     self.views[n] = pv
                 return
         fresh_names = set()
         if need_grads and STORE_ONCE and store_once is not None:
             fresh_names = {n for n in self.names if trainable.get(n, False) and store_once(n, named[n])}
+        sparse_names = set()
+        if need_grads:
+            sparse_names = {n for n in self.names if n in fp32_only and trainable.get(n, False) and n not in fresh_names and named[n].dim() == 2
+                            and named[n].is_contiguous()}
         pad = lambda t: (t.numel() + 63) // 64 * 64
         total = 0
         if need_grads:
-            self.zero_elems = sum(pad(named[n]) for n in self.names if trainable.get(n, False) and n not in fresh_names)
-            total = self.zero_elems + sum(pad(named[n]) for n in fresh_names)
+            self.zero_elems = sum(pad(named[n]) for n in self.names if trainable.get(n, False) and n not in fresh_names and n not in sparse_names)
+            self.fresh_off = self.zero_elems + sum(pad(named[n]) for n in sparse_names)
+            total = self.fresh_off + sum(pad(named[n]) for n in fresh_names)
         dev = next(iter(named.values())).device if named else None
         self.flat = torch.empty(total, dtype=torch.float32, device=dev) if total else None
         self._clear()
-        off_zero, off_fresh = 0, self.zero_elems
+        off_zero, off_sparse, off_fresh = 0, self.zero_elems, self.fresh_off
         for n in self.names:
             t = named[n]
             g = None
             if need_grads and trainable.get(n, False):
-                off = off_fresh if n in fresh_names else off_zero
+                off = off_fresh if n in fresh_names else off_sparse if n in sparse_names else off_zero
                 g = self.flat[off:off + t.numel()].view(t.shape)
                 if t.dim() == 4 and not t.is_contiguous() and t.is_contiguous(memory_format=torch.channels_last):
                     O, I, R, S = t.shape
                     g = self.flat[off:off + t.numel()].view(O, R, S, I).permute(0, 3, 1, 2)
                 if n in fresh_names:
                     off_fresh += pad(t)
+                elif n in sparse_names:
+                    off_sparse += pad(t)
                 else:
                     off_zero += pad(t)
             wb = None
-            if t.dim() >= 2:
+            if t.dim() >= 2 and n not in fp32_only:
                 make = (transforms or {}).get(n) or _cast_bf16
                 wb = compute_copy(t, make, bf16_cache, n)
-            self.views[n] = ParamView(wb, g, t.detach(), fresh=n in fresh_names)
+            pv = self.views[n] = ParamView(wb, g, t.detach(), fresh=n in fresh_names)
+            if n in sparse_names:
+                pv.touched = torch.zeros((t.numel() + opt_chunk() - 1) // opt_chunk(), dtype=torch.uint8, device=dev)
+                register_touched(g, pv.touched)
+                self.sparse.append(pv)
         if REUSE_GRAD_BUFFERS and bf16_cache is not None and need_grads and (memo is None or memo["sig"] != sig):
-            bf16_cache["__layout__"] = {"sig": sig, "flat": self.flat, "views": dict(self.views), "zero_elems": self.zero_elems}
-
-    def _clear(self):
+            bf16_cache["__layout__"] = {"sig": sig, "flat": self.flat, "views": dict(self.views), "zero_elems": self.zero_elems,
+                                        "fresh_off": self.fresh_off, "sparse": self.sparse}
+
+    def _clear(self, reused=False):
         if self.flat is None:
             return
-        if self.zero_elems:
-            self.flat[:self.zero_elems].zero_()
-        if POISON_FRESH and self.zero_elems < self.flat.numel():
-            self.flat[self.zero_elems:].fill_(float("nan"))
+        if reused and self.sparse:
+            if self.zero_elems:
+                self.flat[:self.zero_elems].zero_()
+            for i in range(0, len(self.sparse), 2):
+                k.sparse_clear([(v.g, v.touched) for v in self.sparse[i:i + 2]], opt_chunk())
+        elif self.fresh_off:
+            self.flat[:self.fresh_off].zero_()
+        if POISON_FRESH and self.fresh_off < self.flat.numel():
+            self.flat[self.fresh_off:].fill_(float("nan"))
+
+    def mark_all_touched(self):
+        for v in self.sparse:
+            v.mark_all_touched()
 
     def fresh_views(self):
         return [v for v in self.views.values() if v.fresh and v.g is not None]
diff --git a/toist_amd/functions.py b/toist_amd/functions.py
--- a/toist_amd/functions.py
+++ b/toist_amd/functions.py
@@ -32,9 +32,11 @@
         need = tape_kw.pop('need_grads')
         transforms = tape_kw.pop('transforms')
         store_once = tape_kw.pop('store_once')
+        row_sparse = tape_kw.pop('row_sparse')
         named = dict(zip(names, params))
         trainable = {n: p.requires_grad for n, p in named.items()}
-        ps = engine.ParamSet(named, trainable, need_grads=need, bf16_cache=cache, transforms=transforms, store_once=store_once)
+        ps = engine.ParamSet(named, trainable, need_grads=need, bf16_cache=cache, transforms=transforms, store_once=store_once,
+                             row_sparse=row_sparse)
         tape = engine.Tape(**tape_kw)
         tape.fresh_views = ps.fresh_views() if need else []
         in_vars = [None if t is None else engine.Var(t, needs_grad=(need and t.requires_grad and t.is_floating_point()))
@@ -79,6 +81,7 @@
         n_par = len(ctx.params)
         if ctx.via_autograd:
             par_grads = [g if (g is not None and p.requires_grad) else None for p, g in zip(ctx.params, ps.grads())]
+            ps.mark_all_touched()
             if ctx.rejoin is not None:
                 ctx.rejoin.wait_stream(torch.cuda.current_stream())
             ctx.tape = ctx.ps = ctx.in_vars = ctx.out_vars = ctx.params = None
@@ -90,6 +93,7 @@
             if p.grad is None:
                 p.grad = g
             else:
+                engine.mark_all_touched(p.grad)
                 p.grad.add_(g)
                 ps.flat = None
         if GRAD_SYNC is not None:
@@ -103,10 +107,11 @@
         return (None, None, None, None, None, *in_grads, *([None] * n_par))
 
 
-def run_program(body, named_params, inputs, cache=None, training=False, drop_p=0.0, seed=0, transforms=None, group_wgrads=False, store_once=None):
+def run_program(body, named_params, inputs, cache=None, training=False, drop_p=0.0, seed=0, transforms=None, group_wgrads=False, store_once=None,
+                row_sparse=None):
     names = tuple(named_params.keys())
     params = tuple(named_params.values())
     need = torch.is_grad_enabled() and any(t is not None and t.requires_grad for t in (*inputs, *params))
     tape_kw = dict(training=training, drop_p=drop_p, seed=seed, need_grads=need, transforms=transforms, rejoin=REJOIN, group_wgrads=group_wgrads,
-                   via_autograd=need and _via_autograd(), store_once=store_once)
+                   via_autograd=need and _via_autograd(), store_once=store_once, row_sparse=row_sparse)
     return _TapeFn.apply(body, names, cache, len(inputs), tape_kw, *inputs, *params)
diff --git a/toist_amd/kernels.py b/toist_amd/kernels.py
--- a/toist_amd/kernels.py
+++ b/toist_amd/kernels.py
@@ -425,6 +425,28 @@
                "toist_embed_bwd")
 
 
+def embed_bwd_sparse(g, ids, pos_ids, pad_id, dword, dpos, dtype0, touched_word, touched_pos, chunk):
+    n, D = g.shape
+    for grad, t in ((dword, touched_word), (dpos, touched_pos)):
+        if t is not None and (grad is None or t.numel() * chunk < grad.numel()):
+            raise ValueError("embed_bwd_sparse: a touched array needs one byte per chunk of its gradient")
+    _lib.check(_lib.lib().toist_embed_bwd_sparse(_p(g, torch.bfloat16), _p(ids, torch.int64), _p(pos_ids, torch.int64), n, D, pad_id,
+                                                 _p(dword, torch.float32), _p(dpos, torch.float32), _p(dtype0, torch.float32),
+                                                 _p(touched_word, torch.uint8), _p(touched_pos, torch.uint8), chunk, _stream()),
+               "toist_embed_bwd_sparse")
+
+
+def sparse_clear(slots, chunk):
+    if not 1 <= len(slots) <= 2:
+        raise ValueError("sparse_clear: one or two slots per launch")
+    for grad, t in slots:
+        if not grad.is_contiguous() or t.numel() * chunk < grad.numel():
+            raise ValueError("sparse_clear: a contiguous gradient and one byte per chunk of it")
+    (g0, t0), (g1, t1) = slots[0], (slots[1] if len(slots) > 1 else (None, None))
+    _lib.check(_lib.lib().toist_sparse_clear(_p(g0, torch.float32), _p(t0, torch.uint8), g0.numel(), _p(g1, torch.float32), _p(t1, torch.uint8),
+                                             0 if g1 is None else g1.numel(), chunk, _stream()), "toist_sparse_clear")
+
+
 def criterion_fwd(logits, boxes, tgt_boxes, pos_map, tgt_off, match_off, src_idx, tgt_idx, num_boxes, eos_coef, losses, status=None):
     L, B, Q, K = logits.shape
     _lib.check(_lib.lib().toist_criterion_fwd(_p(logits, torch.float32), _p(boxes, torch.float32), _p(tgt_boxes, torch.float32),
@@ -567,7 +589,11 @@
     return int(_lib.lib().toist_opt_chunk_elems())
 
 
-def opt_sqnorm(table, grads, chunks, n_chunks, partial):
+def opt_sqnorm(table, grads, chunks, n_chunks, partial, touched=None):
+    if touched is not None:
+        _lib.check(_lib.lib().toist_opt_sqnorm_sparse(_p(table, torch.uint8), _p(grads, torch.int64), _p(touched, torch.int64), _p(chunks, torch.int32),
+                                                      n_chunks, _p(partial, torch.float32), _stream()), "toist_opt_sqnorm_sparse")
+        return
     _lib.check(_lib.lib().toist_opt_sqnorm(_p(table, torch.uint8), _p(grads, torch.int64), _p(chunks, torch.int32), n_chunks,
                                            _p(partial, torch.float32), _stream()), "toist_opt_sqnorm")
 
@@ -583,7 +609,12 @@
                "toist_opt_finish_norm_guarded")
 
 
-def opt_adamw_ema(table, grads, chunks, n_chunks, groups, state, beta1, beta2, eps, ema_decay, max_blocks=0):
+def opt_adamw_ema(table, grads, chunks, n_chunks, groups, state, beta1, beta2, eps, ema_decay, max_blocks=0, touched=None, hot=None):
+    if touched is not None or hot is not None:
+        _lib.check(_lib.lib().toist_opt_adamw_ema_sparse(_p(table, torch.uint8), _p(grads, torch.int64), _p(touched, torch.int64), _p(hot, torch.int64),
+                                                         _p(chunks, torch.int32), n_chunks, _p(groups, torch.float32), _p(state, torch.uint8), beta1,
+                                                         beta2, eps, ema_decay, max_blocks, _stream()), "toist_opt_adamw_ema_sparse")
+        return
     _lib.check(_lib.lib().toist_opt_adamw_ema_blocks(_p(table, torch.uint8), _p(grads, torch.int64), _p(chunks, torch.int32), n_chunks,
                                                      _p(groups, torch.float32), _p(state, torch.uint8), beta1, beta2, eps, ema_decay, max_blocks, _stream()),
                "toist_opt_adamw_ema")
diff --git a/toist_amd/optim.py b/toist_amd/optim.py
--- a/toist_amd/optim.py
+++ b/toist_amd/optim.py
@@ -1,7 +1,7 @@
 import numpy as np
 import torch
 
-from . import _lib, engine
+from . import _lib, devcache, engine
 from . import kernels as k
 from .knobs import knob
 
@@ -105,11 +105,20 @@
         self._groups_dev = torch.zeros(len(self.param_groups), len(_GROUP_DT.names), dtype=torch.float32, device=self.device)
         self._chunk = k.opt_chunk_elems()
         n_t = len(params) + len(self._ema_only)
-        self._grads_host = [torch.zeros(n_t, dtype=torch.int64).pin_memory() for _ in range(2)]
+        self._n_t = n_t
+        self._sparse = bool(engine.SPARSE_TAIL)
+        nch = [(p.numel() + self._chunk - 1) // self._chunk for p in params]
+        self._hot = torch.zeros(sum(nch), dtype=torch.uint8, device=self.device)
+        self._hot_off = np.concatenate([[0], np.cumsum(nch)]).astype(np.int64)
+        hot_rows = np.zeros(n_t, dtype=np.int64)
+        hot_rows[:len(params)] = self._hot.data_ptr() + self._hot_off[:-1]
+        self._hot_dev = torch.from_numpy(hot_rows).to(self.device)
+        self._touched_held = []
+        self._grads_host = [torch.zeros(2 * n_t, dtype=torch.int64).pin_memory() for _ in range(2)]
         self._grads_event = [None, None]
         self._grads_turn = 0
         self._grads_last = None
-        self._grads_dev = torch.zeros(n_t, dtype=torch.int64, device=self.device)
+        self._grads_dev = torch.zeros(2 * n_t, dtype=torch.int64, device=self.device)
         self._table = None
         self._chunks = self._partial = self._ema_table = self._ema_chunks = self._ema_grads = None
         self._retired = []
@@ -230,14 +239,24 @@
         if self._grads_event[turn] is not None and not capturing:
             self._grads_event[turn].synchronize()
         gh = self._grads_host[turn].numpy()
+        n_t, held = self._n_t, []
+        sparse = self._sparse and bool(engine.TOUCHED)
         for i, p in enumerate(self.params):
             g = p.grad
+            gh[n_t + i] = 0
             if g is None:
                 gh[i] = 0
                 continue
             if g.dtype != torch.float32 or g.shape != p.shape or g.stride() != p.stride():
                 raise TypeError("FusedClipAdamWEMA: every gradient must be fp32 with its parameter's shape and strides")
             gh[i] = g.data_ptr()
+            if sparse:
+                tb = engine.touched_of(g)
+                if tb is not None:
+                    gh[n_t + i] = tb.data_ptr()
+                    held.append(tb)
+        self._touched_held = held
+        devcache.keep(self._hot_dev)
         if self._grads_last is None or capturing or not np.array_equal(gh, self._grads_last):
             self._grads_dev.copy_(self._grads_host[turn], non_blocking=True)
             if not capturing:
@@ -248,11 +267,12 @@
             self._grads_turn = turn ^ 1
         if self._early_done and self._e_hi > self._e_lo:
             if self._e_lo:
-                k.opt_sqnorm(self._table, self._grads_dev, self._chunks, self._e_lo, self._partial)
+                k.opt_sqnorm(self._table, self._grads_dev, self._chunks, self._e_lo, self._partial, touched=self._touched_dev())
             if self._n_chunks > self._e_hi:
-                k.opt_sqnorm(self._table, self._grads_dev, self._chunks[self._e_hi:], self._n_chunks - self._e_hi, self._partial[self._e_hi:])
+                k.opt_sqnorm(self._table, self._grads_dev, self._chunks[self._e_hi:], self._n_chunks - self._e_hi, self._partial[self._e_hi:],
+                             touched=self._touched_dev())
         else:
-            k.opt_sqnorm(self._table, self._grads_dev, self._chunks, self._n_chunks, self._partial)
+            k.opt_sqnorm(self._table, self._grads_dev, self._chunks, self._n_chunks, self._partial, touched=self._touched_dev())
         self._early_done = False
         if self.skip_nonfinite:
             k.opt_finish_norm_guarded(self._partial, self._n_chunks, self.max_norm, self.betas[0], self.betas[1], self.state,
@@ -261,12 +281,27 @@
             k.opt_finish_norm(self._partial, self._n_chunks, self.max_norm, self.betas[0], self.betas[1], self.state)
         if self._n_now:
             k.opt_adamw_ema(self._table, self._grads_dev, self._chunks, self._n_now, self._groups_dev, self.state, self.betas[0],
-                            self.betas[1], self.eps, self.ema_decay)
+                            self.betas[1], self.eps, self.ema_decay, touched=self._touched_dev(), hot=self._hot_dev if self._sparse else None)
         self._ema_pending = self.defer_ema
         self._bump_epoch()
         if self._n_late:
             self._late_pending = True
             self._late_grads = [p.grad for p, l in zip(self.params, self._late) if l]
+
+    def _touched_dev(self):
+        return self._grads_dev[self._n_t:] if self._sparse else None
+
+    def hot_chunks(self, i):
+        return self._hot[int(self._hot_off[i]):int(self._hot_off[i + 1])]
+
+    def _recompute_hot(self):
+        for i, (m, v) in enumerate(zip(self.exp_avg, self.exp_avg_sq)):
+            n = m.numel()
+            nz = (m.as_strided((n,), (1,)).view(torch.int32) != 0) | (v.as_strided((n,), (1,)).view(torch.int32) != 0)
+            pad = (-n) % self._chunk
+            if pad:
+                nz = torch.cat([nz, nz.new_zeros(pad)])
+            self.hot_chunks(i).copy_(nz.view(-1, self._chunk).any(dim=1))
 
     def note_replayed_step(self):
         self._bump_epoch()
@@ -299,7 +334,11 @@
             g = self.params[i].grad
             if (0 if g is None else g.data_ptr()) != int(last[i]):
                 return
-        k.opt_sqnorm(self._table, self._grads_dev, self._chunks[self._e_lo:], self._e_hi - self._e_lo, self._partial[self._e_lo:])
+            tb = engine.touched_of(g) if self._sparse else None
+            if (0 if tb is None else tb.data_ptr()) != int(last[self._n_t + i]):
+                return
+        k.opt_sqnorm(self._table, self._grads_dev, self._chunks[self._e_lo:], self._e_hi - self._e_lo, self._partial[self._e_lo:],
+                     touched=self._touched_dev())
         self._early_done = True
 
     @torch.no_grad()
@@ -308,7 +347,8 @@
         if not self._n_late or not (self._late_pending or capturing) or (capturing and self._late_captured):
             return
         k.opt_adamw_ema(self._table, self._grads_dev, self._chunks[self._n_now:], self._n_late, self._groups_dev, self.state, self.betas[0],
-                        self.betas[1], self.eps, self.ema_decay, max_blocks=LATE_BLOCKS)
+                        self.betas[1], self.eps, self.ema_decay, max_blocks=LATE_BLOCKS, touched=self._touched_dev(),
+                        hot=self._hot_dev if self._sparse else None)
         for ent, p in self._late_copies:
             ent.epoch = engine.WEIGHT_EPOCH
         if not capturing:
@@ -361,6 +401,7 @@
             self.exp_avg[i].copy_(st["exp_avg"].reshape(self.exp_avg[i].shape) if st["exp_avg"].shape != self.exp_avg[i].shape else st["exp_avg"])
             self.exp_avg_sq[i].copy_(st["exp_avg_sq"].reshape(self.exp_avg_sq[i].shape) if st["exp_avg_sq"].shape != self.exp_avg_sq[i].shape else st["exp_avg_sq"])
             steps.append(int(float(st["step"])))
+        self._recompute_hot()
         if steps and min(steps) != max(steps):
             raise ValueError("FusedClipAdamWEMA.load_state_dict: parameters with different step counts (the fused tail keeps one counter)")
         raw = np.zeros(1, dtype=_STATE_DT)
diff --git a/toist_amd/parallel.py b/toist_amd/parallel.py
--- a/toist_amd/parallel.py
+++ b/toist_amd/parallel.py
@@ -1,7 +1,7 @@
 import torch
 import torch.distributed as dist
 
-from . import functions
+from . import engine, functions
 
 
 class GradSync:
@@ -33,6 +33,7 @@
         work = dist.all_reduce(flat, op=op, group=self.group, async_op=True)
         self.pending.append((work, flat, op))
         self.ranges.append((flat.data_ptr(), flat.data_ptr() + flat.numel() * flat.element_size()))
+        self.pending.extend((w, None, dist.ReduceOp.MAX) for w in _touched_works([flat], self.group))
 
     def _local_states(self, params):
         state = []
@@ -88,6 +89,17 @@
         self.pending, self.ranges = [], []
 
 
+def _touched_works(tensors, group=None):
+    works = []
+    for t in tensors:
+        for tb in engine.touched_in(t):
+            try:
+                works.append(dist.all_reduce(tb, op=dist.ReduceOp.MAX, group=group, async_op=True))
+            except (RuntimeError, TypeError, ValueError):
+                tb.fill_(1)
+    return works
+
+
 def _mean_op(group=None):
     return dist.ReduceOp.AVG if dist.get_backend(group) == "nccl" else dist.ReduceOp.SUM
 
@@ -111,6 +123,7 @@
     op = _mean_op(group)
     wire = [f.to(torch.bfloat16) for f in flats] if bf16 else None
     works = [dist.all_reduce(t, op=op, group=group, async_op=True) for t in (wire if bf16 else flats)]
+    works += _touched_works(flats, group)
     return _MeanHandle(works, list(flats), op, dist.get_world_size(group), wire)
 
 
diff --git a/toist_amd/transformer.py b/toist_amd/transformer.py
--- a/toist_amd/transformer.py
+++ b/toist_amd/transformer.py
@@ -394,7 +394,11 @@
                 g = emb.take_grad()
                 if g is None or wv.g is None:
                     return
-                k.embed_bwd(g, ids_flat, pos_ids.view(-1), cfg.pad_token_id, wv.g, pv.g, tv.g[0] if tv.g is not None else None)
+                if wv.touched is not None or pv.touched is not None:
+                    k.embed_bwd_sparse(g, ids_flat, pos_ids.view(-1), cfg.pad_token_id, wv.g, pv.g, tv.g[0] if tv.g is not None else None,
+                                       wv.touched, pv.touched, engine.opt_chunk())
+                else:
+                    k.embed_bwd(g, ids_flat, pos_ids.view(-1), cfg.pad_token_id, wv.g, pv.g, tv.g[0] if tv.g is not None else None)
 
             tape.record(emb_bwd)
             x = engine.layernorm(tape, emb, P("embeddings.LayerNorm.weight"), P("embeddings.LayerNorm.bias"), cfg.layer_norm_eps)
@@ -423,7 +427,8 @@
 
         (out,) = functions.run_program(prog, named, [], cache=self._cache_text, training=self.training, drop_p=cfg.hidden_dropout_prob,
                                        seed=self._next_seed(), group_wgrads=True, transforms=transforms,
-                                       store_once=lambda n, t: t.dim() == 2 and "embeddings" not in n)
+                                       store_once=lambda n, t: t.dim() == 2 and "embeddings" not in n,
+                                       row_sparse=("text_encoder.embeddings.word_embeddings.weight", "text_encoder.embeddings.position_embeddings.weight"))
         return out, key_pad
 
     def encode_tokens(self, tokens, pos, key_pad, B, S):
```

Result: faster. 725.1 images/s (median of 6 runs) (+1.5%).
